# tp7/Sushi

Hardware: AMD Instinct MI355X
Metric: subtitle events/sec (matchTemplate+argmax) + max |shift err| vs cv2, 1/2/4/8 GPU (higher is better)
Workload: dtype f32; 1 GPU; BASELINE configs[2] (the north_star target's configuration): 3000 events, 120-min 12000 Hz float32 src/dst, +-120 s window (P=2880001 positions, patterns U[1,5] s), explicit centres; the whole job every step; global_events=3000, sample_type=float32, hard_events=0, events_with_a_planted_answer=3000, method=TM_SQDIFF_NORMED+argmin (what wav.py:185-186 does; see SURVEY F1), kernel_variant=2

## Files before the change

include/sushi_hip.h:

```cpp
#ifndef SUSHI_HIP_H
#define SUSHI_HIP_H

#include <stddef.h>
#include <stdint.h>

#ifdef __cplusplus
extern "C" {
#endif

#define SUSHI_HIP_ABI_VERSION 13

#if defined(__GNUC__)
#define SUSHI_HIP_API __attribute__((visibility("default")))
#else
#define SUSHI_HIP_API
#endif

#define SUSHI_HIP_OK 0
#define SUSHI_HIP_EINVAL (-1)
#define SUSHI_HIP_EALIGN (-2)
#define SUSHI_HIP_ELAUNCH (-3)
#define SUSHI_HIP_ENOSPACE (-4)
#define SUSHI_HIP_ENODEV (-5)
#define SUSHI_HIP_ENOMEM (-6)
#define SUSHI_HIP_EINTERNAL (-7)

#define SUSHI_HIP_U8 0
#define SUSHI_HIP_F32 1

#define SUSHI_HIP_PATH_FFT 0
#define SUSHI_HIP_PATH_DIRECT 1

#define SUSHI_HIP_METHOD_SQDIFF_NORMED 0
#define SUSHI_HIP_METHOD_CCOEFF_NORMED 1

SUSHI_HIP_API int sushi_hip_abi_version(void);
SUSHI_HIP_API const char* sushi_hip_strerror(int code);

SUSHI_HIP_API int sushi_hip_device_ok(void);
SUSHI_HIP_API int sushi_hip_device_prepare(void);

typedef struct SushiHipStream SushiHipStream;

SUSHI_HIP_API int sushi_hip_fft_size(void);
SUSHI_HIP_API int sushi_hip_fft_block(void);
SUSHI_HIP_API int sushi_hip_fft_slot_of_bin(int bin);
SUSHI_HIP_API int sushi_hip_fft_low_slot_of_bin(int bin);
SUSHI_HIP_API double sushi_hip_centre(int dtype);
SUSHI_HIP_API size_t sushi_hip_stream_bytes(int64_t n, int dtype, int searchable);
SUSHI_HIP_API size_t sushi_hip_stream_spectra_bytes(int64_t n);
SUSHI_HIP_API int sushi_hip_stream_create(const void* raw_dev, int dtype, int64_t n, int searchable,
                                          void* mem_dev, size_t mem_bytes, void* hip_stream, SushiHipStream** out);
SUSHI_HIP_API int sushi_hip_stream_add_spectra(SushiHipStream* stream, void* mem_dev, size_t mem_bytes, void* hip_stream);
#define SUSHI_HIP_VIEW_XC 0
#define SUSHI_HIP_VIEW_S1 1
#define SUSHI_HIP_VIEW_S2 2
#define SUSHI_HIP_VIEW_UREL 3
#define SUSHI_HIP_VIEW_BASE 4
#define SUSHI_HIP_VIEW_SPECTRA 5
#define SUSHI_HIP_VIEW_USREL 6
#define SUSHI_HIP_VIEW_BASE1 7
#define SUSHI_HIP_VIEW_COARSE 8
#define SUSHI_HIP_VIEW_SPECTRA_LOW 9
#define SUSHI_HIP_VIEW_ZNORM_REST 10
SUSHI_HIP_API int sushi_hip_stream_view(const SushiHipStream* stream, int which, const void** ptr_dev, size_t* bytes);
SUSHI_HIP_API void sushi_hip_stream_destroy(SushiHipStream* stream);

typedef struct SushiHipRequest {
    int64_t tmpl_off;
    int64_t win_start;
    int32_t tmpl_len;
    int32_t n_pos;
} SushiHipRequest;

typedef struct SushiHipBatchInfo {
    int32_t n_search;
    int32_t path;
    int32_t variant;
    int32_t sub_batches;
    int64_t direct_tiles;
    int64_t fft_pairs;
    int64_t fft_segments;
    uint64_t workspace_bytes;
    uint64_t mem_bytes;
    double flops;
    double algorithmic_bytes;
    int32_t lanes;
    int32_t reserved;
} SushiHipBatchInfo;

typedef struct SushiHipBatchDiag {
    int32_t flagged;
    int32_t all_positions;
    int64_t tiles_dense;
    int64_t tiles_sparse;
    int64_t candidates;
    float max_bound_ratio;
    float max_bound_ratio_noncandidate;
    int64_t audited;
    int64_t pairs_transformed;
    int64_t excluded_audited;
    float max_slb_ratio_excluded;
    int32_t slb_violations;
    int32_t band;
    int32_t suspended;
    int32_t band_votes[2];
    int64_t second_look_audited;
} SushiHipBatchDiag;

typedef struct SushiHipBatch SushiHipBatch;

SUSHI_HIP_API size_t sushi_hip_batch_bytes(const SushiHipRequest* req_host, int n, int path, int variant,
                                           size_t workspace_cap_bytes);
SUSHI_HIP_API int sushi_hip_batch_create(const SushiHipStream* dst, const SushiHipStream* src,
                                         const SushiHipRequest* req_host, int n, int path, int variant,
                                         size_t workspace_cap_bytes, void* mem_dev, size_t mem_bytes,
                                         void* hip_stream, SushiHipBatch** out);
SUSHI_HIP_API int sushi_hip_batch_reset(SushiHipBatch* batch, const SushiHipRequest* req_host, int n, void* hip_stream);
SUSHI_HIP_API int sushi_hip_batch_info(const SushiHipBatch* batch, SushiHipBatchInfo* info);
SUSHI_HIP_API int sushi_hip_batch_set_method(SushiHipBatch* batch, int method);
#define SUSHI_HIP_EXCLUDE_AUTO 0
#define SUSHI_HIP_EXCLUDE_ALWAYS 1
#define SUSHI_HIP_EXCLUDE_NEVER 2
#define SUSHI_HIP_EXCLUDE_BAND 3
#define SUSHI_HIP_EXCLUDE_WHOLE 4
SUSHI_HIP_API int sushi_hip_batch_set_exclusion(SushiHipBatch* batch, int mode);
#define SUSHI_HIP_BOUND_WORST_CASE 0
#define SUSHI_HIP_BOUND_STATISTICAL 1
SUSHI_HIP_API int sushi_hip_batch_set_bound_model(SushiHipBatch* batch, int model);
SUSHI_HIP_API int sushi_hip_batch_set_packed_output(SushiHipBatch* batch, int32_t* out_packed_dev);
SUSHI_HIP_API int sushi_hip_batch_set_early_output(SushiHipBatch* batch, int32_t* early);
SUSHI_HIP_API int sushi_hip_batch_run(SushiHipBatch* batch, double delta, int32_t* out_idx_dev, float* out_score_dev,
                                      void* hip_stream);
SUSHI_HIP_API int sushi_hip_batch_diagnostics(SushiHipBatch* batch, SushiHipBatchDiag* diag, float* ranking_err_host,
                                              int32_t* flagged_host);
SUSHI_HIP_API int sushi_hip_batch_pair_bounds(SushiHipBatch* batch, float* slb_host, float* acc_host, int64_t* n_pairs);
#define SUSHI_HIP_WS_TSPEC 0
#define SUSHI_HIP_WS_Y 1
#define SUSHI_HIP_WS_TSPEC_LOW 2
#define SUSHI_HIP_WS_Y_LOW 3
#define SUSHI_HIP_WS_TNORM_REST 4
#define SUSHI_HIP_WS_TSPEC_HALF 5
SUSHI_HIP_API int sushi_hip_batch_workspace_view(SushiHipBatch* batch, int which, void** ptr_dev, size_t* bytes);
SUSHI_HIP_API void sushi_hip_batch_destroy(SushiHipBatch* batch);

typedef struct SushiHipHit {
    int32_t index;
    float score;
} SushiHipHit;
SUSHI_HIP_API int sushi_hip_batch_run_threshold(SushiHipBatch* batch, double threshold, int32_t capacity,
                                                SushiHipHit* out_hits_dev, int64_t* out_counts_dev, void* hip_stream);

#define SUSHI_HIP_BEST_MAX_K 32
SUSHI_HIP_API int sushi_hip_batch_run_best(SushiHipBatch* batch, int32_t k, int32_t min_separation, const double* threshold,
                                           SushiHipHit* out_hits_dev, int32_t* out_counts_dev, void* hip_stream);

SUSHI_HIP_API int sushi_hip_fft_layout(int64_t win_start, int32_t n_pos, int32_t tmpl_len,
                                       int32_t* n_pairs, int32_t* n_seg);

SUSHI_HIP_API size_t sushi_hip_curve_bytes(const SushiHipRequest* req_host, int n);
SUSHI_HIP_API int sushi_hip_match_curves(const SushiHipStream* dst, const SushiHipStream* src,
                                         const SushiHipRequest* req_host, int n, int method,
                                         void* mem_dev, size_t mem_bytes, float* out_dev, void* hip_stream);

typedef struct SushiHipRetimeSegment {
    int64_t in_start;
    int64_t out_off;
    int64_t out_len;
    int32_t num, den;
} SushiHipRetimeSegment;
SUSHI_HIP_API size_t sushi_hip_retime_bytes(int n_seg);
SUSHI_HIP_API int sushi_hip_retime(const void* in_dev, int dtype, int64_t n_in,
                                   const SushiHipRetimeSegment* seg_host, int n_seg,
                                   void* out_dev, int64_t n_out,
                                   void* mem_dev, size_t mem_bytes, void* hip_stream);

SUSHI_HIP_API int sushi_hip_envelope(const void* in_dev, int dtype, int64_t n_in, int64_t in_start,
                                     int32_t hop, int32_t span, void* out_dev, int64_t out_len, void* hip_stream);

SUSHI_HIP_API int sushi_hip_filter(const void* in_dev, int dtype, int64_t n_in, int64_t in_start,
                                   const double* taps_dev, int32_t n_taps, void* out_dev, int64_t out_len, void* hip_stream);

SUSHI_HIP_API int sushi_hip_level(const void* in_dev, int dtype, int64_t n_in, int64_t in_start,
                                  int32_t window, double floor, double peak, void* out_dev, int64_t out_len, void* hip_stream);

typedef struct SushiHipJointRow {
    int64_t curve_off;
    double weight;
} SushiHipJointRow;
typedef struct SushiHipJointGroup {
    int32_t first_row;
    int32_t n_rows;
    int32_t n_shift;
    int32_t reserved;
} SushiHipJointGroup;
SUSHI_HIP_API size_t sushi_hip_joint_bytes(int n_groups, int n_rows);
SUSHI_HIP_API int sushi_hip_joint_reduce(const float* curves_dev, int64_t n_curve,
                                         const SushiHipJointRow* rows_host, int n_rows,
                                         const SushiHipJointGroup* groups_host, int n_groups, int method,
                                         void* mem_dev, size_t mem_bytes,
                                         int32_t* out_idx_dev, float* out_score_dev,
                                         float* out_row_score_dev, int32_t* out_row_idx_dev, float* out_row_best_dev,
                                         float* out_joint_dev, void* hip_stream);

SUSHI_HIP_API size_t sushi_hip_path_bytes(int n_rows, int32_t n_shift);
SUSHI_HIP_API int64_t sushi_hip_path_stay_words(int32_t n_shift);
SUSHI_HIP_API int sushi_hip_path_forward(const float* curves_dev, int64_t n_curve,
                                         const SushiHipJointRow* rows_host, int n_rows, int32_t n_shift,
                                         int method, double penalty, int row0, int n_total,
                                         double* D_dev, unsigned long long* stay_dev,
                                         double* row_min_dev, int32_t* row_arg_dev,
                                         int32_t* row_own_index_dev, float* row_own_score_dev,
                                         void* mem_dev, size_t mem_bytes, void* hip_stream);
SUSHI_HIP_API int sushi_hip_path_backtrack(const unsigned long long* stay_dev, const int32_t* row_arg_dev, int n_total,
                                           int32_t n_shift, int32_t* out_shift_dev, void* hip_stream);

SUSHI_HIP_API size_t sushi_hip_drift_bytes(int n_rows, int n_drifts);
SUSHI_HIP_API int sushi_hip_drift_reduce(const float* curves_dev, int64_t n_curve,
                                         const SushiHipJointRow* rows_host, int n_rows, int32_t n_shift,
                                         const int32_t* offsets_host, int n_drifts, int method,
                                         void* mem_dev, size_t mem_bytes,
                                         int32_t* out_best_dev, float* out_score_dev, float* out_row_score_dev,
                                         int32_t* out_drift_idx_dev, float* out_drift_score_dev,
                                         float* out_lines_dev, void* hip_stream);

#define SUSHI_HIP_TRACK_MAX_REACH 1024
#define SUSHI_HIP_TRACK_JUMP (-32768)
SUSHI_HIP_API size_t sushi_hip_track_bytes(int n_rows, int32_t n_shift);
SUSHI_HIP_API int sushi_hip_track_forward(const float* curves_dev, int64_t n_curve,
                                          const SushiHipJointRow* rows_host, const int32_t* reach_host, int n_rows, int32_t n_shift,
                                          int method, double penalty, double step_cost, int row0, int n_total,
                                          double* D_dev, int16_t* move_dev,
                                          double* row_min_dev, int32_t* row_arg_dev,
                                          int32_t* row_own_index_dev, float* row_own_score_dev,
                                          void* mem_dev, size_t mem_bytes, void* hip_stream);
SUSHI_HIP_API int sushi_hip_track_backtrack(const int16_t* move_dev, const int32_t* row_arg_dev, int n_total,
                                            int32_t n_shift, int32_t* out_shift_dev, void* hip_stream);

SUSHI_HIP_API int sushi_hip_track_forward_keep(const float* curves_dev, int64_t n_curve,
                                               const SushiHipJointRow* rows_host, const int32_t* reach_host, int n_rows, int32_t n_shift,
                                               int method, double penalty, double step_cost, int row0, int n_total,
                                               double* D_all_dev, int16_t* move_dev,
                                               double* row_min_dev, int32_t* row_arg_dev,
                                               int32_t* row_own_index_dev, float* row_own_score_dev,
                                               void* mem_dev, size_t mem_bytes, void* hip_stream);
SUSHI_HIP_API size_t sushi_hip_track_margins_bytes(int n_rows, int32_t n_shift);
SUSHI_HIP_API int sushi_hip_track_margins(const float* curves_dev, int64_t n_curve,
                                          const SushiHipJointRow* rows_host, const int32_t* reach_host, const int32_t* guard_host,
                                          int n_rows, int32_t n_shift, int method, double penalty, double step_cost,
                                          int row0, int n_total,
                                          const double* D_all_dev, const int32_t* shift_dev, double* C_dev, double* c_min_dev,
                                          double* through_dev, double* best_dev, int32_t* best_arg_dev,
                                          double* alt_dev, int32_t* alt_arg_dev, double* M_dev,
                                          void* mem_dev, size_t mem_bytes, void* hip_stream);

#define SUSHI_HIP_TRACK_BACK_ANY (-1)
SUSHI_HIP_API size_t sushi_hip_track_order_bytes(int n_rows, int32_t n_shift);
SUSHI_HIP_API int sushi_hip_track_forward_ordered(const float* curves_dev, int64_t n_curve,
                                                  const SushiHipJointRow* rows_host, const int32_t* reach_host,
                                                  const int32_t* back_host, int n_rows, int32_t n_shift,
                                                  int method, const double* penalty_host, double step_cost, int row0, int n_total,
                                                  double* D_dev, int16_t* move_dev,
                                                  double* P_dev, int32_t* from_dev, int32_t* back_dev,
                                                  double* row_min_dev, int32_t* row_arg_dev,
                                                  int32_t* row_own_index_dev, float* row_own_score_dev,
                                                  void* mem_dev, size_t mem_bytes, void* hip_stream);
SUSHI_HIP_API int sushi_hip_track_backtrack_ordered(const int16_t* move_dev, const int32_t* from_dev, const int32_t* back_dev,
                                                    const int32_t* row_arg_dev, int n_total, int32_t n_shift,
                                                    int32_t* out_shift_dev, void* hip_stream);

SUSHI_HIP_API int sushi_hip_track_forward_ordered_keep(const float* curves_dev, int64_t n_curve,
                                                       const SushiHipJointRow* rows_host, const int32_t* reach_host,
                                                       const int32_t* back_host, int n_rows, int32_t n_shift,
                                                       int method, const double* penalty_host, double step_cost, int row0, int n_total,
                                                       double* D_all_dev, int16_t* move_dev,
                                                       double* P_dev, int32_t* from_dev, int32_t* back_dev,
                                                       double* row_min_dev, int32_t* row_arg_dev,
                                                       int32_t* row_own_index_dev, float* row_own_score_dev,
                                                       void* mem_dev, size_t mem_bytes, void* hip_stream);
SUSHI_HIP_API size_t sushi_hip_track_order_margins_bytes(int n_rows, int32_t n_shift);
SUSHI_HIP_API int sushi_hip_track_order_margins(const float* curves_dev, int64_t n_curve,
                                                const SushiHipJointRow* rows_host, const int32_t* reach_host,
                                                const int32_t* back_host, const int32_t* guard_host,
                                                int n_rows, int32_t n_shift, int method, const double* penalty_host, double step_cost,
                                                int row0, int n_total,
                                                const double* D_all_dev, const int32_t* shift_dev, double* C_dev, double* S_dev,
                                                double* c_min_dev, double* through_dev, double* best_dev, int32_t* best_arg_dev,
                                                double* alt_dev, int32_t* alt_arg_dev, double* M_dev,
                                                void* mem_dev, size_t mem_bytes, void* hip_stream);

#define SUSHI_HIP_TRACK_WIDE_MAX_REACH 32767
SUSHI_HIP_API size_t sushi_hip_track_wide_bytes(int n_rows, int32_t n_shift);
SUSHI_HIP_API size_t sushi_hip_track_margins_wide_bytes(int n_rows, int32_t n_shift);
SUSHI_HIP_API int sushi_hip_track_forward_wide(const float* curves_dev, int64_t n_curve,
                                               const SushiHipJointRow* rows_host, const int32_t* reach_host, int n_rows, int32_t n_shift,
// ... 109 lines not shown
```

sushi_amd/_native.py:

```python
import ctypes
import os
import re

import numpy as np

from .common import SushiError

_HERE = os.path.dirname(os.path.abspath(__file__))
LIB_PATH = os.environ.get("SUSHI_HIP_LIB") or os.path.join(_HERE, "lib", "libsushi_hip.so")
HEADER_PATH = os.path.join(os.path.dirname(_HERE), "include", "sushi_hip.h")

U8, F32 = 0, 1
PATH_FFT, PATH_DIRECT = 0, 1
METHOD_SQDIFF_NORMED, METHOD_CCOEFF_NORMED = 0, 1
MIX_MAX_CHANNELS, MIX_MAX_OUTPUTS = 32, 8
PCM_FORMATS = {"u8": 1, "s16": 2, "s24": 3, "s32": 4, "f32": 5, "f64": 6}
PCM_WIDTHS = {"u8": 1, "s16": 2, "s24": 3, "s32": 4, "f32": 4, "f64": 8}
BEST_MAX_K = 32
TRACK_MAX_REACH, TRACK_JUMP = 1024, -32768
TRACK_WIDE_MAX_REACH = 32767
TRACK_BACK_ANY = -1
METHODS = {"sqdiff_normed": METHOD_SQDIFF_NORMED, "ccoeff_normed": METHOD_CCOEFF_NORMED}
VIEW_XC, VIEW_S1, VIEW_S2, VIEW_UREL, VIEW_BASE, VIEW_SPECTRA, VIEW_USREL, VIEW_BASE1, VIEW_COARSE, VIEW_SPECTRA_LOW, \
    VIEW_ZNORM_REST = range(11)

ABI_VERSION = 13
ENOSPACE = -4
NSTAGES = 6
STAGE_NAMES = ("tspec", "mac", "ifft", "refine", "finish", "bound")
STAGE_KERNELS = {"tspec": "tspec_real_kernel|tspec_kernel", "mac": "mac_kernel", "ifft": "mac_list_kernel+mac_rows_kernel+ifft_kernel", "refine": "refine_kernel",
                 "finish": "collect_kernel+exact_tiles_kernel+unpack_keys_kernel", "bound": "bound_low_kernel|bound_kernel"}
EXCLUSION = {"auto": 0, "always": 1, "never": 2, "band": 3, "whole": 4}
WS_TSPEC, WS_Y, WS_TSPEC_LOW, WS_Y_LOW, WS_TNORM_REST, WS_TSPEC_HALF = range(6)
BOUND_MODEL = {"worst_case": 0, "statistical": 1}
STAGE_KERNEL_SETS = {"tspec": ("tspec_real_kernel", "tspec_kernel"), "mac": ("mac_kernel", "mac_long_kernel"),
                     "ifft": ("ifft_kernel", "ifft_list_kernel", "pilot_kernel", "survivor_kernel", "mac_list_kernel", "mac_rows_kernel",
                              "bound_low_exact_kernel", "slb_list_kernel", "survivor2_kernel"),
                     "refine": ("refine_kernel",),
                     "finish": ("collect_kernel", "exact_tiles_kernel"), "bound": ("bound_kernel", "bound_low_kernel", "slb_kernel")}

REQUEST_DTYPE = np.dtype([("tmpl_off", "<i8"), ("win_start", "<i8"), ("tmpl_len", "<i4"), ("n_pos", "<i4")], align=True)
assert REQUEST_DTYPE.itemsize == 24
HIT_DTYPE = np.dtype([("index", "<i4"), ("score", "<f4")], align=True)
assert HIT_DTYPE.itemsize == 8
RETIME_SEGMENT_DTYPE = np.dtype([("in_start", "<i8"), ("out_off", "<i8"), ("out_len", "<i8"), ("num", "<i4"), ("den", "<i4")], align=True)
assert RETIME_SEGMENT_DTYPE.itemsize == 32
JOINT_ROW_DTYPE = np.dtype([("curve_off", "<i8"), ("weight", "<f8")], align=True)
assert JOINT_ROW_DTYPE.itemsize == 16
JOINT_GROUP_DTYPE = np.dtype([("first_row", "<i4"), ("n_rows", "<i4"), ("n_shift", "<i4"), ("reserved", "<i4")], align=True)
assert JOINT_GROUP_DTYPE.itemsize == 16
ROWS_ROW_DTYPE = np.dtype([("out_off", "<i8"), ("in_off", "<i8"), ("n_pos", "<i4"), ("reserved", "<i4")], align=True)
assert ROWS_ROW_DTYPE.itemsize == 24
ROWS_OVERFLOW, ROWS_BAD_HITS = 1, 2


class BatchInfo(ctypes.Structure):
    _fields_ = [("n_search", ctypes.c_int32), ("path", ctypes.c_int32), ("variant", ctypes.c_int32),
                ("sub_batches", ctypes.c_int32), ("direct_tiles", ctypes.c_int64), ("fft_pairs", ctypes.c_int64),
                ("fft_segments", ctypes.c_int64), ("workspace_bytes", ctypes.c_uint64), ("mem_bytes", ctypes.c_uint64),
                ("flops", ctypes.c_double), ("algorithmic_bytes", ctypes.c_double), ("lanes", ctypes.c_int32),
                ("reserved", ctypes.c_int32)]


class BatchDiag(ctypes.Structure):
    _fields_ = [("flagged", ctypes.c_int32), ("all_positions", ctypes.c_int32), ("tiles_dense", ctypes.c_int64),
                ("tiles_sparse", ctypes.c_int64), ("candidates", ctypes.c_int64), ("max_bound_ratio", ctypes.c_float),
                ("max_bound_ratio_noncandidate", ctypes.c_float), ("audited", ctypes.c_int64),
                ("pairs_transformed", ctypes.c_int64), ("excluded_audited", ctypes.c_int64),
                ("max_slb_ratio_excluded", ctypes.c_float), ("slb_violations", ctypes.c_int32), ("band", ctypes.c_int32),
                ("suspended", ctypes.c_int32), ("band_votes", ctypes.c_int32 * 2), ("second_look_audited", ctypes.c_int64)]


_lib = None


class NativeError(SushiError):
    pass


def declared_symbols():
    with open(HEADER_PATH) as f:
        text = f.read()
    return sorted(set(re.findall(r"SUSHI_HIP_API\s+[\w\s\*]+?\b(sushi_hip_\w+)\s*\(", text)))


def lib():
    global _lib
    if _lib is not None:
        return _lib
    if not os.path.exists(LIB_PATH):
        raise NativeError("libsushi_hip.so is not built (%s); run `python -m sushi_amd.build` -- "
                          "there is no CPU fallback for the matching path" % LIB_PATH)
    import torch
    L = ctypes.CDLL(LIB_PATH)
    vp, i64, ci, dbl, sz = ctypes.c_void_p, ctypes.c_int64, ctypes.c_int, ctypes.c_double, ctypes.c_size_t
    i32, u32, cf = ctypes.c_int32, ctypes.c_uint32, ctypes.c_float
    pvp = ctypes.POINTER(vp)
    L.sushi_hip_abi_version.restype = ci
    L.sushi_hip_strerror.restype = ctypes.c_char_p
    L.sushi_hip_strerror.argtypes = [ci]
    L.sushi_hip_device_ok.restype = ci
    L.sushi_hip_device_prepare.restype = ci
    L.sushi_hip_fft_size.restype = ci
    L.sushi_hip_fft_block.restype = ci
    L.sushi_hip_fft_slot_of_bin.restype = ci
    L.sushi_hip_fft_slot_of_bin.argtypes = [ci]
    L.sushi_hip_fft_low_slot_of_bin.restype = ci
    L.sushi_hip_fft_low_slot_of_bin.argtypes = [ci]
    L.sushi_hip_centre.restype = dbl
    L.sushi_hip_centre.argtypes = [ci]
    L.sushi_hip_stream_bytes.restype = sz
    L.sushi_hip_stream_bytes.argtypes = [i64, ci, ci]
    L.sushi_hip_stream_spectra_bytes.restype = sz
    L.sushi_hip_stream_spectra_bytes.argtypes = [i64]
    L.sushi_hip_stream_create.restype = ci
    L.sushi_hip_stream_create.argtypes = [vp, ci, i64, ci, vp, sz, vp, pvp]
    L.sushi_hip_stream_add_spectra.restype = ci
    L.sushi_hip_stream_add_spectra.argtypes = [vp, vp, sz, vp]
    L.sushi_hip_stream_view.restype = ci
    L.sushi_hip_stream_view.argtypes = [vp, ci, pvp, ctypes.POINTER(sz)]
    L.sushi_hip_stream_destroy.restype = None
    L.sushi_hip_stream_destroy.argtypes = [vp]
    L.sushi_hip_batch_bytes.restype = sz
    L.sushi_hip_batch_bytes.argtypes = [vp, ci, ci, ci, sz]
    L.sushi_hip_batch_create.restype = ci
    L.sushi_hip_batch_create.argtypes = [vp, vp, vp, ci, ci, ci, sz, vp, sz, vp, pvp]
    L.sushi_hip_batch_reset.restype = ci
    L.sushi_hip_batch_reset.argtypes = [vp, vp, ci, vp]
    L.sushi_hip_batch_info.restype = ci
    L.sushi_hip_batch_info.argtypes = [vp, ctypes.POINTER(BatchInfo)]
    L.sushi_hip_batch_set_method.restype = ci
    L.sushi_hip_batch_set_method.argtypes = [vp, ci]
    L.sushi_hip_batch_run.restype = ci
    L.sushi_hip_batch_run.argtypes = [vp, dbl, vp, vp, vp]
    L.sushi_hip_batch_run_threshold.restype = ci
    L.sushi_hip_batch_run_threshold.argtypes = [vp, dbl, i32, vp, vp, vp]
    L.sushi_hip_batch_run_best.restype = ci
    L.sushi_hip_batch_run_best.argtypes = [vp, i32, i32, ctypes.POINTER(dbl), vp, vp, vp]
    L.sushi_hip_batch_diagnostics.restype = ci
    L.sushi_hip_batch_diagnostics.argtypes = [vp, ctypes.POINTER(BatchDiag), vp, vp]
    L.sushi_hip_batch_set_packed_output.restype = ci
    L.sushi_hip_batch_set_packed_output.argtypes = [vp, vp]
    L.sushi_hip_batch_set_early_output.restype = ci
    L.sushi_hip_batch_set_early_output.argtypes = [vp, vp]
    L.sushi_hip_batch_set_exclusion.restype = ci
    L.sushi_hip_batch_set_exclusion.argtypes = [vp, ci]
    L.sushi_hip_batch_set_bound_model.restype = ci
    L.sushi_hip_batch_set_bound_model.argtypes = [vp, ci]
    L.sushi_hip_batch_pair_bounds.restype = ci
    L.sushi_hip_batch_pair_bounds.argtypes = [vp, vp, vp, ctypes.POINTER(i64)]
    L.sushi_hip_batch_workspace_view.restype = ci
    L.sushi_hip_batch_workspace_view.argtypes = [vp, ci, pvp, ctypes.POINTER(sz)]
    L.sushi_hip_batch_destroy.restype = None
    L.sushi_hip_batch_destroy.argtypes = [vp]
    L.sushi_hip_fft_layout.restype = ci
    L.sushi_hip_fft_layout.argtypes = [i64, i32, i32, ctypes.POINTER(i32), ctypes.POINTER(i32)]
    L.sushi_hip_curve_bytes.restype = sz
    L.sushi_hip_curve_bytes.argtypes = [vp, ci]
    L.sushi_hip_match_curves.restype = ci
    L.sushi_hip_match_curves.argtypes = [vp, vp, vp, ci, ci, vp, sz, vp, vp]
    L.sushi_hip_retime_bytes.restype = sz
    L.sushi_hip_retime_bytes.argtypes = [ci]
    L.sushi_hip_retime.restype = ci
    L.sushi_hip_retime.argtypes = [vp, ci, i64, vp, ci, vp, i64, vp, sz, vp]
    L.sushi_hip_envelope.restype = ci
    L.sushi_hip_envelope.argtypes = [vp, ci, i64, i64, i32, i32, vp, i64, vp]
    L.sushi_hip_filter.restype = ci
    L.sushi_hip_filter.argtypes = [vp, ci, i64, i64, vp, i32, vp, i64, vp]
    L.sushi_hip_level.restype = ci
    L.sushi_hip_level.argtypes = [vp, ci, i64, i64, i32, dbl, dbl, vp, i64, vp]
    L.sushi_hip_joint_bytes.restype = sz
    L.sushi_hip_joint_bytes.argtypes = [ci, ci]
    L.sushi_hip_joint_reduce.restype = ci
    L.sushi_hip_joint_reduce.argtypes = [vp, i64, vp, ci, vp, ci, ci, vp, sz, vp, vp, vp, vp, vp, vp, vp]
    L.sushi_hip_drift_bytes.restype = sz
    L.sushi_hip_drift_bytes.argtypes = [ci, ci]
    L.sushi_hip_drift_reduce.restype = ci
    L.sushi_hip_drift_reduce.argtypes = [vp, i64, vp, ci, i32, vp, ci, ci, vp, sz, vp, vp, vp, vp, vp, vp, vp]
    L.sushi_hip_path_bytes.restype = sz
    L.sushi_hip_path_bytes.argtypes = [ci, i32]
    L.sushi_hip_path_stay_words.restype = i64
    L.sushi_hip_path_stay_words.argtypes = [i32]
    L.sushi_hip_path_forward.restype = ci
    L.sushi_hip_path_forward.argtypes = [vp, i64, vp, ci, i32, ci, dbl, ci, ci, vp, vp, vp, vp, vp, vp, vp, sz, vp]
    L.sushi_hip_path_backtrack.restype = ci
    L.sushi_hip_path_backtrack.argtypes = [vp, vp, ci, i32, vp, vp]
    L.sushi_hip_track_bytes.restype = sz
    L.sushi_hip_track_bytes.argtypes = [ci, i32]
    L.sushi_hip_track_forward.restype = ci
    L.sushi_hip_track_forward.argtypes = [vp, i64, vp, vp, ci, i32, ci, dbl, dbl, ci, ci, vp, vp, vp, vp, vp, vp, vp, sz, vp]
    L.sushi_hip_track_backtrack.restype = ci
    L.sushi_hip_track_backtrack.argtypes = [vp, vp, ci, i32, vp, vp]
    L.sushi_hip_track_forward_keep.restype = ci
    L.sushi_hip_track_forward_keep.argtypes = L.sushi_hip_track_forward.argtypes
    L.sushi_hip_track_margins_bytes.restype = sz
    L.sushi_hip_track_margins_bytes.argtypes = [ci, i32]
    L.sushi_hip_track_margins.restype = ci
    L.sushi_hip_track_margins.argtypes = [vp, i64, vp, vp, vp, ci, i32, ci, dbl, dbl, ci, ci, vp, vp, vp, vp, vp, vp, vp, vp, vp, vp, vp,
                                          sz, vp]
    L.sushi_hip_track_wide_bytes.restype = sz
    L.sushi_hip_track_wide_bytes.argtypes = [ci, i32]
    L.sushi_hip_track_margins_wide_bytes.restype = sz
    L.sushi_hip_track_margins_wide_bytes.argtypes = [ci, i32]
    L.sushi_hip_track_forward_wide.restype = ci
    L.sushi_hip_track_forward_wide.argtypes = L.sushi_hip_track_forward.argtypes
    L.sushi_hip_track_forward_wide_keep.restype = ci
    L.sushi_hip_track_forward_wide_keep.argtypes = L.sushi_hip_track_forward.argtypes
    L.sushi_hip_track_margins_wide.restype = ci
    L.sushi_hip_track_margins_wide.argtypes = L.sushi_hip_track_margins.argtypes
    L.sushi_hip_track_order_bytes.restype = sz
    L.sushi_hip_track_order_bytes.argtypes = [ci, i32]
    L.sushi_hip_track_forward_ordered.restype = ci
    L.sushi_hip_track_forward_ordered.argtypes = [vp, i64, vp, vp, vp, ci, i32, ci, vp, dbl, ci, ci, vp, vp, vp, vp, vp, vp, vp, vp, vp,
                                                  vp, sz, vp]
    L.sushi_hip_track_backtrack_ordered.restype = ci
    L.sushi_hip_track_backtrack_ordered.argtypes = [vp, vp, vp, vp, ci, i32, vp, vp]
    L.sushi_hip_track_forward_ordered_keep.restype = ci
    L.sushi_hip_track_forward_ordered_keep.argtypes = L.sushi_hip_track_forward_ordered.argtypes
    L.sushi_hip_track_order_margins_bytes.restype = sz
    L.sushi_hip_track_order_margins_bytes.argtypes = [ci, i32]
    L.sushi_hip_track_order_margins.restype = ci
    L.sushi_hip_track_order_margins.argtypes = [vp, i64, vp, vp, vp, vp, ci, i32, ci, vp, dbl, ci, ci, vp, vp, vp, vp, vp, vp, vp, vp, vp,
                                                vp, vp, vp, sz, vp]
    L.sushi_hip_track_order_wide_bytes.restype = sz
    L.sushi_hip_track_order_wide_bytes.argtypes = [ci, i32]
    L.sushi_hip_track_order_margins_wide_bytes.restype = sz
    L.sushi_hip_track_order_margins_wide_bytes.argtypes = [ci, i32]
    L.sushi_hip_track_forward_ordered_wide.restype = ci
    L.sushi_hip_track_forward_ordered_wide.argtypes = L.sushi_hip_track_forward_ordered.argtypes
    L.sushi_hip_track_forward_ordered_wide_keep.restype = ci
    L.sushi_hip_track_forward_ordered_wide_keep.argtypes = L.sushi_hip_track_forward_ordered.argtypes
    L.sushi_hip_track_order_margins_wide.restype = ci
    L.sushi_hip_track_order_margins_wide.argtypes = L.sushi_hip_track_order_margins.argtypes
    L.sushi_hip_rows_tile.restype = ci
    L.sushi_hip_rows_bytes.restype = sz
    L.sushi_hip_rows_bytes.argtypes = [ci]
    L.sushi_hip_rows_from_hits.restype = ci
    L.sushi_hip_rows_from_hits.argtypes = [vp, vp, ci, i32, vp, cf, vp, i64, vp, vp, sz, vp]
    L.sushi_hip_rows_clamp.restype = ci
    L.sushi_hip_rows_clamp.argtypes = [vp, i64, vp, i64, vp, ci, ci, cf, vp, sz, vp]
    L.sushi_hip_load_decode.restype = ci
    L.sushi_hip_load_decode.argtypes = [vp, i64, i32, i32, vp, vp]
    L.sushi_hip_load_decode_mix.restype = ci
    L.sushi_hip_load_decode_mix.argtypes = [vp, i64, i32, i32, vp, i32, vp, i64, vp]
    L.sushi_hip_load_decode_format.restype = ci
    L.sushi_hip_load_decode_format.argtypes = [vp, i64, i32, i32, vp, vp]
    L.sushi_hip_load_decode_mix_format.restype = ci
    L.sushi_hip_load_decode_mix_format.argtypes = [vp, i64, i32, i32, vp, i32, vp, i64, vp]
    L.sushi_hip_load_resample.restype = ci
    L.sushi_hip_load_resample.argtypes = [vp, i64, i32, i32, dbl, i64, i32, i32, dbl, i64, i64, vp, vp]
    L.sushi_hip_load_resample_fir.restype = ci
    L.sushi_hip_load_resample_fir.argtypes = [vp, i64, i32, i32, vp, i32, i64, i64, i64, vp, vp]
    L.sushi_hip_load_histogram.restype = ci
    L.sushi_hip_load_histogram.argtypes = [vp, i64, ci, u32, u32, ci, vp, vp]
    L.sushi_hip_load_normalise.restype = ci
    L.sushi_hip_load_normalise.argtypes = [vp, i64, cf, cf, cf, vp, vp]
    L.sushi_hip_profile_begin.restype = ci
    L.sushi_hip_profile_end.restype = ci
    L.sushi_hip_profile_end.argtypes = [vp, ci, ctypes.POINTER(ci)]
    if L.sushi_hip_abi_version() != ABI_VERSION:
        raise NativeError("libsushi_hip.so ABI version mismatch")
    _lib = L
    return L


def check(rc, what):
    if rc != 0:
        msg = lib().sushi_hip_strerror(rc).decode()
        raise NativeError("%s failed: %s (%d)" % (what, msg, rc))


def fft_layout(win_start, n_pos, tmpl_len):
    a, b = ctypes.c_int32(0), ctypes.c_int32(0)
    check(lib().sushi_hip_fft_layout(int(win_start), int(n_pos), int(tmpl_len), ctypes.byref(a), ctypes.byref(b)),
          "sushi_hip_fft_layout")
    return a.value, b.value


def profile_begin():
    check(lib().sushi_hip_profile_begin(), "sushi_hip_profile_begin")


def profile_end(max_calls):
    buf = np.zeros((max(1, max_calls), NSTAGES), np.float32)
    n = ctypes.c_int(0)
    check(lib().sushi_hip_profile_end(buf.ctypes.data, int(max_calls), ctypes.byref(n)), "sushi_hip_profile_end")
    return buf[:n.value]
```

sushi_amd/csrc/fft_core.hpp:

```cpp
#ifndef SUSHI_FFT_CORE_HPP
#define SUSHI_FFT_CORE_HPP

#ifdef __HIPCC__
#define SUSHI_HD __device__ __forceinline__
#define SUSHI_HHD __host__ __device__ inline
#else
#define SUSHI_HD inline
#define SUSHI_HHD inline
#endif

namespace sushi_fft {

constexpr int PER = 16;
constexpr int TWIDDLE_N = 16384;

template <int LOGN> struct Plan;
template <> struct Plan<13> {
    static constexpr int N = 8192, NT = 512, R3 = 8;
};
template <> struct Plan<14> {
    static constexpr int N = 16384, NT = 1024, R3 = 16;
};
constexpr int R1 = 8, R2 = 8, R4 = 16;

// ... 491 lines not shown
}
typedef _Float16 h2 __attribute__((ext_vector_type(2)));
__device__ __forceinline__ h2 h_rot(const h2 a) { return h2{-a.y, a.x}; }
__device__ __forceinline__ h2 h_cmul(const h2 a, const h2 w) { return a * w.xx + h_rot(a) * w.yy; }
__device__ __forceinline__ h2 h_splat(const float c) { return h2{(_Float16)c, (_Float16)c}; }
__device__ __forceinline__ void h_bfly_root32(const h2 e, const h2 o, const int q, h2& lo, h2& hi) {
    const float C[9] = {1.0f, 0.98078528040323044913f, 0.92387953251128673848f, 0.83146961230254523708f, 0.70710678118654752440f,
                        0.55557023301960222474f, 0.38268343236508978178f, 0.19509032201612826785f, 0.0f};
    switch (q) {
        case 0: lo = e + o; hi = e - o; return;
        case 8: lo = e + h_rot(o); hi = e - h_rot(o); return;
        case 4: { const h2 p = o + h_rot(o); lo = p * h_splat(C[4]) + e; hi = e - p * h_splat(C[4]); return; }
        case 12: { const h2 p = h_rot(o) - o; lo = p * h_splat(C[4]) + e; hi = e - p * h_splat(C[4]); return; }
        default: {
            const float c = q <= 8 ? C[q] : -C[16 - q], sn = q <= 8 ? C[8 - q] : C[q - 8];
            lo = h_rot(o) * h_splat(sn) + (o * h_splat(c) + e);
            hi = e * h_splat(2.0f) - lo;
        }
    }
}
template <int R>
struct DftH {
    static __device__ __forceinline__ void run(h2* v) {
        h2 e[R / 2], o[R / 2];
#pragma unroll
        for (int u = 0; u < R / 2; ++u) { e[u] = v[2 * u]; o[u] = v[2 * u + 1]; }
        DftH<R / 2>::run(e);
        DftH<R / 2>::run(o);
#pragma unroll
        for (int t = 0; t < R / 2; ++t) h_bfly_root32(e[t], o[t], t * (32 / R), v[t], v[t + R / 2]);
    }
};
template <>
struct DftH<1> {
    static __device__ __forceinline__ void run(h2*) {}
};
struct HTwiddles { h2 p2[16]; h2 z1[4], z2[4], z3[4]; };
__device__ __forceinline__ h2 h_round(const cpx c) { return h2{(_Float16)c.x, (_Float16)c.y}; }
__device__ __forceinline__ HTwiddles load_htwiddles(const int lane, const cpx* __restrict__ tw) {
    HTwiddles t;
    const int e1 = lane & 15;
#pragma unroll
    for (int d = 0; d < 16; ++d) t.p2[d] = h_round(cconj(tw[((e1 * d) & 255) * (TWIDDLE_N / 256)]));
    const cpx q3 = cconj(tw[((lane & 15) + 64 * (lane >> 4)) * (TWIDDLE_N / 1024)]);
#pragma unroll
    for (int e = 0; e < 4; ++e) {
        const cpx z = cmul(q3, cconj(tw[e * (TWIDDLE_N / 64)]));
        const cpx z2 = cmul(z, z);
        t.z1[e] = h_round(z); t.z2[e] = h_round(z2); t.z3[e] = h_round(cmul(z2, z));
    }
    return t;
}
__device__ __forceinline__ unsigned h_abs2(const h2 a) {
    return __builtin_bit_cast(unsigned, __builtin_amdgcn_fdot2(a, a, 0.f, false));
}
__device__ __forceinline__ unsigned h_max_bits(const unsigned a, const unsigned b) { return a > b ? a : b; }
struct MfmaBh { half8 r, i; };
__device__ __forceinline__ MfmaBh load_mfma_bh(const int lane, const uint4v* __restrict__ table) {
    MfmaBh b;
    b.r = __builtin_bit_cast(half8, table[lane]);
    b.i = __builtin_bit_cast(half8, table[64 + lane]);
    return b;
}
__device__ __forceinline__ void fft_wave_half_front(const uint4v (&yl)[4], h2* v, const HTwiddles& tw, const MfmaBh& b, unsigned& max_in2,
                                                    h2* pass1_out = nullptr, h2* pass2_out = nullptr, h2* swapped_out = nullptr) {
    unsigned mi = 0u;
#pragma unroll
    for (int g = 0; g < 4; ++g) {
        unsigned rr01 = __builtin_amdgcn_perm(yl[g][1], yl[g][0], 0x05040100u), rr23 = __builtin_amdgcn_perm(yl[g][3], yl[g][2], 0x05040100u);
        unsigned ii01 = __builtin_amdgcn_perm(yl[g][1], yl[g][0], 0x07060302u), ii23 = __builtin_amdgcn_perm(yl[g][3], yl[g][2], 0x07060302u);
        { const auto r = __builtin_amdgcn_permlane32_swap(rr01, ii01, false, false); rr01 = r[0]; ii01 = r[1]; }
        { const auto r = __builtin_amdgcn_permlane32_swap(rr23, ii23, false, false); rr23 = r[0]; ii23 = r[1]; }
        const uint4v aw = {rr01, rr23, ii01, ii23};
        const half8 a = __builtin_bit_cast(half8, aw);
        const float4v z = {0.f, 0.f, 0.f, 0.f};
        const float4v dr = __builtin_amdgcn_mfma_f32_16x16x32_f16(a, b.r, z, 0, 0, 0);
        const float4v di = __builtin_amdgcn_mfma_f32_16x16x32_f16(a, b.i, z, 0, 0, 0);
#pragma unroll
        for (int i = 0; i < 4; ++i) {
            unsigned packed = __builtin_bit_cast(unsigned, h2{(_Float16)dr[i], (_Float16)di[i]});
            asm volatile("" : "+v"(packed));
            v[4 * g + i] = __builtin_bit_cast(h2, packed);
            mi = h_max_bits(mi, h_abs2(v[4 * g + i]));
        }
    }
    max_in2 = mi;
    if (pass1_out) {
#pragma unroll
        for (int t = 0; t < 16; ++t) pass1_out[t] = v[t];
    }
#pragma unroll
    for (int t = 1; t < 16; ++t) v[t] = h_cmul(v[t], tw.p2[t]);
    DftH<16>::run(v);
    if (pass2_out) {
#pragma unroll
        for (int t = 0; t < 16; ++t) pass2_out[t] = v[t];
    }
    auto swap32 = [](h2& x, h2& y) {
        const auto r = __builtin_amdgcn_permlane32_swap(__builtin_bit_cast(unsigned, x), __builtin_bit_cast(unsigned, y), false, false);
        unsigned ra = r[0], rb = r[1];
        asm volatile("" : "+v"(ra), "+v"(rb));
        x = __builtin_bit_cast(h2, ra); y = __builtin_bit_cast(h2, rb);
    };
    auto swap16 = [](h2& x, h2& y) {
        const auto r = __builtin_amdgcn_permlane16_swap(__builtin_bit_cast(unsigned, x), __builtin_bit_cast(unsigned, y), false, false);
        unsigned ra = r[0], rb = r[1];
        asm volatile("" : "+v"(ra), "+v"(rb));
        x = __builtin_bit_cast(h2, ra); y = __builtin_bit_cast(h2, rb);
    };
#pragma unroll
    for (int r = 0; r < 8; ++r) swap32(v[r], v[r + 8]);
#pragma unroll
    for (int r = 0; r < 16; ++r)
        if ((r & 4) == 0) swap16(v[r], v[r + 4]);
    if (swapped_out) {
#pragma unroll
        for (int t = 0; t < 16; ++t) swapped_out[t] = v[t];
    }
#pragma unroll
    for (int e = 0; e < 4; ++e) {
        h2 q[4] = {v[e], h_cmul(v[4 + e], tw.z1[e]), h_cmul(v[8 + e], tw.z2[e]), h_cmul(v[12 + e], tw.z3[e])};
        DftH<4>::run(q);
        v[e] = q[0]; v[4 + e] = q[1]; v[8 + e] = q[2]; v[12 + e] = q[3];
    }
}
#endif

constexpr int LB_HW = WN / 8;
constexpr int LB_BINS = 2 * LB_HW;
constexpr int LB_ENTRIES = LB_BINS / 4;
constexpr int LB_GROUPS = 8;
SUSHI_HHD int lslot_of_thread(int tid) {
    const int g = tid & 7, t = tid >> 3;
    const int kq = t >> 6, g4 = (t >> 4) & 3, mm = ((t & 3) << 2) | ((t >> 2) & 3);
    return (g * 4 + g4) * 32 + 16 * kq + mm;
}
SUSHI_HHD int lb_d1(int kq, int j) { return kq + (j == 0 ? 0 : (j == 1 ? 2 : (j == 2 ? 12 : 14))); }
SUSHI_HHD int lb_bin_of(int entry, int j) {
    const int g = entry >> 7, g4 = (entry >> 5) & 3, l = entry & 31, kq = l >> 4, mm = l & 15;
    const int d2 = 4 * g4 + (mm & 3), d3 = mm >> 2;
    const int m = 64 * lb_d1(kq, j) + 4 * d2 + d3;
    const int k = g + 8 * m;
    return k < WN / 8 ? k : k + WN / 2;
}
SUSHI_HHD int lslot_of_bin(int f) {
    if (f < 0 || f >= WN || (f >= LB_HW && f < WN - LB_HW)) return -1;
    const int k = f < LB_HW ? f : f - WN / 2;
    const int g = k & 7, m = k >> 3;
    const int d1 = m >> 6, d2 = (m >> 2) & 15, d3 = m & 3;
    const int kq = d1 & 1, b = d1 - kq;
    const int j = b == 0 ? 0 : (b == 2 ? 1 : (b == 12 ? 2 : 3));
    return (((g * 4 + (d2 >> 2)) * 32 + 16 * kq + ((d3 << 2) | (d2 & 3))) << 2) + j;
}
SUSHI_HHD double dft16_low_operand(int form, int l, int j) {
    const int kq = l >> 4, n = l & 15, part = kq >> 1, d1 = lb_d1(kq & 1, j);
    const double PI = 3.14159265358979323846;
    const double wr = __builtin_cos(2.0 * PI * (double)((n * d1) & 15) / 16.0), wi = __builtin_sin(2.0 * PI * (double)((n * d1) & 15) / 16.0);
    return form == 0 ? (part == 0 ? wr : -wi) : (part == 0 ? wi : wr);
}

#ifdef __HIPCC__
typedef _Float16 half4 __attribute__((ext_vector_type(4)));
typedef unsigned uint2v __attribute__((ext_vector_type(2)));
struct MfmaBl { half4 r, i; };
__device__ __forceinline__ MfmaBl load_mfma_bl(const int lane, const uint2v* __restrict__ table) {
    MfmaBl b;
    b.r = __builtin_bit_cast(half4, table[lane]);
    b.i = __builtin_bit_cast(half4, table[64 + lane]);
    return b;
}
__device__ __forceinline__ void fft_wave_half_tail(h2* v, const HTwiddles& tw) {
#pragma unroll
    for (int t = 1; t < 16; ++t) v[t] = h_cmul(v[t], tw.p2[t]);
    DftH<16>::run(v);
    auto swap32 = [](h2& x, h2& y) {
        const auto r = __builtin_amdgcn_permlane32_swap(__builtin_bit_cast(unsigned, x), __builtin_bit_cast(unsigned, y), false, false);
        unsigned ra = r[0], rb = r[1];
        asm volatile("" : "+v"(ra), "+v"(rb));
        x = __builtin_bit_cast(h2, ra); y = __builtin_bit_cast(h2, rb);
    };
    auto swap16 = [](h2& x, h2& y) {
        const auto r = __builtin_amdgcn_permlane16_swap(__builtin_bit_cast(unsigned, x), __builtin_bit_cast(unsigned, y), false, false);
        unsigned ra = r[0], rb = r[1];
        asm volatile("" : "+v"(ra), "+v"(rb));
        x = __builtin_bit_cast(h2, ra); y = __builtin_bit_cast(h2, rb);
    };
#pragma unroll
    for (int r = 0; r < 8; ++r) swap32(v[r], v[r + 8]);
#pragma unroll
    for (int r = 0; r < 16; ++r)
        if ((r & 4) == 0) swap16(v[r], v[r + 4]);
#pragma unroll
    for (int e = 0; e < 4; ++e) {
        h2 q[4] = {v[e], h_cmul(v[4 + e], tw.z1[e]), h_cmul(v[8 + e], tw.z2[e]), h_cmul(v[12 + e], tw.z3[e])};
        DftH<4>::run(q);
        v[e] = q[0]; v[4 + e] = q[1]; v[8 + e] = q[2]; v[12 + e] = q[3];
    }
}
__device__ __forceinline__ void fft_wave_half_front_low(const uint4v (&yl)[4], h2* v, const HTwiddles& tw, const MfmaBl& b, unsigned& max_in2,
                                                        h2* pass1_out = nullptr) {
    unsigned mi = 0u;
#pragma unroll
    for (int g = 0; g < 4; ++g) {
        unsigned rr01 = __builtin_amdgcn_perm(yl[g][1], yl[g][0], 0x05040100u), rr23 = __builtin_amdgcn_perm(yl[g][3], yl[g][2], 0x05040100u);
        unsigned ii01 = __builtin_amdgcn_perm(yl[g][1], yl[g][0], 0x07060302u), ii23 = __builtin_amdgcn_perm(yl[g][3], yl[g][2], 0x07060302u);
        { const auto r = __builtin_amdgcn_permlane32_swap(rr01, ii01, false, false); rr01 = r[0]; ii01 = r[1]; }
        { const auto r = __builtin_amdgcn_permlane32_swap(rr23, ii23, false, false); rr23 = r[0]; ii23 = r[1]; }
        const uint2v aw = {rr01, rr23};
        const half4 a = __builtin_bit_cast(half4, aw);
        const float4v z = {0.f, 0.f, 0.f, 0.f};
        const float4v dr = __builtin_amdgcn_mfma_f32_16x16x16f16(a, b.r, z, 0, 0, 0);
        const float4v di = __builtin_amdgcn_mfma_f32_16x16x16f16(a, b.i, z, 0, 0, 0);
#pragma unroll
        for (int i = 0; i < 4; ++i) {
            unsigned packed = __builtin_bit_cast(unsigned, h2{(_Float16)dr[i], (_Float16)di[i]});
            asm volatile("" : "+v"(packed));
            v[4 * g + i] = __builtin_bit_cast(h2, packed);
            mi = h_max_bits(mi, h_abs2(v[4 * g + i]));
        }
    }
    max_in2 = mi;
    if (pass1_out) {
#pragma unroll
        for (int t = 0; t < 16; ++t) pass1_out[t] = v[t];
    }
    fft_wave_half_tail(v, tw);
}
#endif

}
#endif
```

sushi_amd/csrc/run_policy.hpp:

```cpp
#ifndef SUSHI_RUN_POLICY_HPP
#define SUSHI_RUN_POLICY_HPP

#include <stdint.h>
#include <string.h>

#include <algorithm>

#include "sushi_geometry.hpp"

#ifndef SUSHI_HHD
#ifdef __HIPCC__
#define SUSHI_HHD __host__ __device__ inline
#else
#define SUSHI_HHD inline
#endif
#endif

namespace sushi {

enum RunKind { RUN_ARGMIN, RUN_THRESHOLD, RUN_BEST };

struct Learnt {
    int band = -1;
    int band_decided_method = -1;
    int band_votes[2] = {0, 0};
    int suspended = 0;
    unsigned suspended_at = 0;
    unsigned long long last_transformed = 0;
    void forget() { *this = Learnt(); }
};

struct LastRun {
    RunKind kind = RUN_ARGMIN;
    int band = -1;
    bool whole_cut = false;
    bool suspended = false;
    int64_t direct_pairs = 0;
    bool ran = false;
};

constexpr double SUSPEND_LEFT_SHARE = 0.75;
constexpr unsigned LOOK_AGAIN_MASK = 63u;
constexpr int64_t EXCLUDE_FROM_PAIRS = 3000, EXCLUDE_PAIRS_PER_SEARCH = 2;
constexpr double BAND_VOTE_SHARE = 0.75;
constexpr int64_t DIRECT_SLOTS_MIN = 4096, DIRECT_USUAL_PART = 8;
constexpr int64_t DIRECT_FIRST_RUN_PART = 2;

inline void absorb_counts(Learnt& l, int exclusion, unsigned run_seq, unsigned long long transformed, unsigned long long audited,
                          int64_t plan_pairs) {
    const unsigned long long left = transformed - audited;
    l.last_transformed = transformed;
    if (exclusion == SUSHI_HIP_EXCLUDE_AUTO) {
        if ((double)left > SUSPEND_LEFT_SHARE * (double)plan_pairs) { if (!l.suspended) l.suspended_at = run_seq; l.suspended = 1; }
        else l.suspended = 0;
    }
}

inline bool run_suspended(const Learnt& l, int exclusion, unsigned run_seq) {
    return exclusion == SUSHI_HIP_EXCLUDE_AUTO && l.suspended && ((run_seq - l.suspended_at) & LOOK_AGAIN_MASK) != LOOK_AGAIN_MASK;
}

inline bool whole_rows_throughout(const Learnt& l, int exclusion, int method, bool suspended) {
    return suspended || exclusion == SUSHI_HIP_EXCLUDE_NEVER || exclusion == SUSHI_HIP_EXCLUDE_WHOLE ||
           ((exclusion == SUSHI_HIP_EXCLUDE_AUTO || exclusion == SUSHI_HIP_EXCLUDE_ALWAYS) && l.band == 0 && l.band_decided_method == method);
}
inline bool takes_whole_cut(bool whole_rows, bool whole_cut_exists) { return whole_rows && whole_cut_exists; }
inline int run_lanes(bool whole_rows, int plan_lanes) { return whole_rows ? 1 : plan_lanes; }

inline bool sub_excludes(int exclusion, bool suspended, int64_t pairs, int n_sub) {
    return exclusion == SUSHI_HIP_EXCLUDE_ALWAYS || exclusion == SUSHI_HIP_EXCLUDE_BAND || exclusion == SUSHI_HIP_EXCLUDE_WHOLE ||
           (exclusion == SUSHI_HIP_EXCLUDE_AUTO && !suspended && pairs > EXCLUDE_FROM_PAIRS + EXCLUDE_PAIRS_PER_SEARCH * (int64_t)n_sub);
}

inline bool listed_run_excludes(int exclusion) { return exclusion != SUSHI_HIP_EXCLUDE_NEVER; }

inline bool form_chosen(int exclusion) { return exclusion == SUSHI_HIP_EXCLUDE_BAND || exclusion == SUSHI_HIP_EXCLUDE_WHOLE; }
inline bool vote_due(const Learnt& l, int exclusion, int method) {
    return !form_chosen(exclusion) && (l.band < 0 || l.band_decided_method != method);
}
inline void decide_form(Learnt& l, int method, int looked_at, int with_room) {
    l.band_votes[0] = looked_at; l.band_votes[1] = with_room;
    l.band = l.band_votes[0] > 0 && (double)l.band_votes[1] >= BAND_VOTE_SHARE * (double)l.band_votes[0] ? 1 : 0;
    l.band_decided_method = method;
}
inline int exclusion_form(const Learnt& l, int exclusion) {
    return !form_chosen(exclusion) ? l.band : exclusion == SUSHI_HIP_EXCLUDE_BAND ? 1 : 0;
}

inline int64_t direct_slots(unsigned long long last_transformed, int64_t pairs, int64_t plan_pairs) {
    int64_t direct64 = std::min<int64_t>(pairs, std::max<int64_t>(DIRECT_SLOTS_MIN, pairs / DIRECT_USUAL_PART));
    if ((double)last_transformed * (double)pairs > (double)direct64 * (double)plan_pairs) direct64 = pairs;
    else if (last_transformed == 0) direct64 = std::min<int64_t>(pairs, std::max<int64_t>(DIRECT_SLOTS_MIN, pairs / DIRECT_FIRST_RUN_PART));
    return direct64;
}

enum { PILOT_ROWS_BY_SEARCH = 0, PILOT_ROWS_LIST = 1 };
inline int pilot_rows_route(const char* setting) {
    if (!setting || !*setting || !strcmp(setting, "search")) return PILOT_ROWS_BY_SEARCH;
    return !strcmp(setting, "list") ? PILOT_ROWS_LIST : -1;
}
inline bool pilot_rows_by_search(int route) { return route != PILOT_ROWS_LIST; }

enum { REST_ROWS_BY_ITEM = 0, REST_ROWS_BY_SEARCH = 1 };
inline int rest_rows_route(const char* setting) {
    if (!setting || !*setting || !strcmp(setting, "items")) return REST_ROWS_BY_ITEM;
    return !strcmp(setting, "search") ? REST_ROWS_BY_SEARCH : -1;
}
inline bool rest_rows_by_item(int route) { return route != REST_ROWS_BY_SEARCH; }

#ifndef SUSHI_REST_ITEM_PAIRS
#define SUSHI_REST_ITEM_PAIRS 4
#endif
constexpr int REST_ITEM_PAIRS = SUSHI_REST_ITEM_PAIRS;
static_assert(REST_ITEM_PAIRS >= 1, "an item holds a pair");
SUSHI_HHD bool rest_pair_to_form(int listed, int i, int audit) { return listed != 0 && i != audit; }
SUSHI_HHD unsigned long long rest_item_starts(unsigned long long form, int before, int per_item) {
    unsigned long long starts = 0;
    int rank = before;
    for (unsigned long long m = form; m; m &= m - 1, ++rank)
        if (rank % per_item == 0) starts |= m & (~m + 1);
    return starts;
}
SUSHI_HHD unsigned long long rest_item_take(unsigned long long form, int room) {
    unsigned long long take = 0;
    for (unsigned long long m = form; m && room > 0; m &= m - 1, --room) take |= m & (~m + 1);
    return take;
}

enum { TSPEC_REAL = 0, TSPEC_COMPLEX = 1 };
inline int tspec_route(const char* setting) {
    if (!setting || !*setting || !strcmp(setting, "real")) return TSPEC_REAL;
    return !strcmp(setting, "complex") ? TSPEC_COMPLEX : -1;
}
inline bool tspec_real(int route) { return route != TSPEC_COMPLEX; }
inline bool tspec_half_rows(int route) { return tspec_real(route); }

inline void begin_run(LastRun& last, RunKind kind) {
    last = LastRun();
    last.kind = kind; last.ran = true;
}

inline void report_last_run(const LastRun& last, const Learnt& l, const RunCounters& c, SushiHipBatchDiag* diag) {
    const bool argmin = last.kind == RUN_ARGMIN;
    diag->pairs_transformed = (int64_t)c.pairs_transformed + last.direct_pairs;
    diag->band = last.band;
    diag->suspended = argmin && last.suspended ? 1 : 0;
    diag->band_votes[0] = argmin ? l.band_votes[0] : 0; diag->band_votes[1] = argmin ? l.band_votes[1] : 0;
    diag->second_look_audited = argmin ? (int64_t)c.second_look_audited : 0;
}

}
#endif
```

sushi_amd/csrc/sushi_fft.hip:

```cpp

#include <hip/hip_runtime.h>
#include <stdint.h>
#include <float.h>
#include <limits.h>
#include <stdio.h>
#include <stdlib.h>
#include <string.h>

#include <algorithm>
#include <cmath>
#include <memory>
#include <mutex>
#include <new>
#include <string>
#include <type_traits>
#include <vector>

#include "../../include/sushi_hip.h"
#include "sushi_common.hpp"
#include "sushi_internal.hpp"
#include "fft_core.hpp"
#include "mac_core.hpp"
#include "plan_core.hpp"
#include "batch_core.hpp"
#include "run_policy.hpp"

namespace {

using namespace sushi;
using sushi_fft::cpx;

constexpr int FN = FFT_N;
constexpr int FT = sushi_fft::Plan<FFT_LOGN>::NT;
constexpr int FH = FFT_H;
constexpr int HPT = FH / FT;
constexpr int RPB = FFT_SEG / FT;
static_assert(FH % FT == 0 && FFT_SEG % FT == 0 && HPT == FFT_VB * RPB, "position layout");
static_assert(HPT <= sushi_fft::PER, "a thread's valid outputs are a prefix of its transform outputs");
constexpr int LDS_FLOATS = sushi_fft::lds_floats<FFT_LOGN>();

#include "sushi_fft_store.inc"
#include "sushi_fft_spectra.inc"
#include "sushi_fft_mac.inc"
#include "sushi_fft_ifft.inc"
#include "sushi_fft_bound.inc"
#include "sushi_fft_collect.inc"
#include "sushi_fft_threshold.inc"
#include "sushi_fft_best.inc"
#include "sushi_fft_plan.inc"

}

struct HostSlots {
    static constexpr int SLOTS = 1024, WORDS = 2;
    std::mutex mu;
    unsigned long long* base = nullptr;
    std::vector<int> free_list;
    unsigned long long* take() {
        std::lock_guard<std::mutex> g(mu);
        if (!base) {
            if (hipHostMalloc((void**)&base, (size_t)SLOTS * WORDS * sizeof(unsigned long long), hipHostMallocPortable) != hipSuccess) { base = nullptr; return nullptr; }
            for (int k = SLOTS - 1; k >= 0; --k) free_list.push_back(k);
        }
        if (free_list.empty()) return nullptr;
        const int k = free_list.back(); free_list.pop_back();
        return base + (size_t)k * WORDS;
    }
    void give(unsigned long long* p) {
        if (!p) return;
        std::lock_guard<std::mutex> g(mu);
        free_list.push_back((int)((p - base) / WORDS));
    }
};
static HostSlots g_host_slots;

struct LanePool {
    static constexpr int MAX_DEVICES = 16;
    std::mutex mu;
    hipStream_t st[MAX_DEVICES][MAX_LANES] = {};
    hipStream_t get(int lane) {
        int dev = 0;
        if (hipGetDevice(&dev) != hipSuccess || dev < 0 || dev >= MAX_DEVICES) return nullptr;
        std::lock_guard<std::mutex> g(mu);
        if (!st[dev][lane] && hipStreamCreateWithFlags(&st[dev][lane], hipStreamNonBlocking) != hipSuccess) st[dev][lane] = nullptr;
        return st[dev][lane];
    }
};
static LanePool g_lane_pool;

struct SushiHipBatch {
    const SushiHipStream* dst = nullptr;
    const SushiHipStream* src = nullptr;
    int n = 0, path = 0, variant = 0, method = SUSHI_HIP_METHOD_SQDIFF_NORMED, exclusion = SUSHI_HIP_EXCLUDE_AUTO;
    Learnt learnt;
    LastRun last;
    unsigned run_seq = 0;
    int audit_every = 2;
    int pilot_rows = PILOT_ROWS_BY_SEARCH;
    int rest_rows = REST_ROWS_BY_ITEM;
    int tspec = TSPEC_REAL;
    int bound_model = SUSHI_HIP_BOUND_WORST_CASE;
    BoundFault fault;
    unsigned long long* host_stats = nullptr;
    hipEvent_t stats_ready = nullptr;
    bool stats_pending = false;
    int32_t* packed_out = nullptr;
    int32_t* early_out = nullptr;
    BatchPlanState states[2];
    BatchPlanState *now = &states[0], *spare = &states[1];
    bool planned = false;
    size_t mem_bytes = 0, ws_cap = 0;
    char* mem = nullptr;
    hipStream_t last_stream = nullptr;
    hipEvent_t uploaded = nullptr;
    hipStream_t lane_stream[MAX_LANES] = {};
    hipEvent_t lane_done[MAX_LANES] = {};
    hipEvent_t fork = nullptr;
    void* tspec_whole = nullptr;
    size_t tspec_whole_bytes = 0;
    void forget_learnt() { learnt.forget(); last = LastRun(); }
    ~SushiHipBatch() {
        for (int l = 1; l < MAX_LANES; ++l) {
            if (lane_stream[l]) (void)hipStreamSynchronize(lane_stream[l]);
            if (lane_done[l]) (void)hipEventDestroy(lane_done[l]);
        }
        if (fork) (void)hipEventDestroy(fork);
        if (uploaded) { (void)hipEventSynchronize(uploaded); (void)hipEventDestroy(uploaded); }
        if (stats_pending && stats_ready) (void)hipEventSynchronize(stats_ready);
        if (stats_ready) (void)hipEventDestroy(stats_ready);
        g_host_slots.give(host_stats);
        if (tspec_whole) (void)hipFree(tspec_whole);
    }
};

static SubView last_sub(const SushiHipBatch* b) {
    const std::vector<SubBatch>& subs = b->last.whole_cut ? b->now->plan.subs_whole : b->now->plan.subs;
    return SubView(b->mem, b->now->lay, b->now->plan.ws_lane, subs.back(), subs.size() - 1);
}

struct RunCtx {
    SushiHipBatch* b;
    const SushiHipStream *dst, *src;
    StreamRefs r;
    const SearchDesc* searches;
    unsigned long long *keys, *gkeys;
    int *flags, *flag_list, *viol;
    RunCounters* counters;
    double delta;
    int method, lanes = 1;
    unsigned run_seq = 0;
    ProfCall* pc = nullptr;
    bool suspended = false, cand_filled = false, excluded_any = false;
    RunCtx(SushiHipBatch* bb, double d) : b(bb), dst(bb->dst), src(bb->src), delta(d), method(bb->method) {
        r = StreamRefs{dst->xc, dst->s1, dst->s2, dst->n, src->xc, src->s1, src->s2, src->n, sushi_hip_centre(dst->dtype), dst->raw, src->raw,
                       dst->dtype};
        searches = (const SearchDesc*)(b->mem + b->now->lay.desc); keys = (unsigned long long*)(b->mem + b->now->lay.keys); gkeys = keys + b->n;
        flags = (int*)(b->mem + b->now->lay.flags); flag_list = (int*)(b->mem + b->now->lay.flag_list); viol = (int*)(b->mem + b->now->lay.viol);
        counters = (RunCounters*)(b->mem + b->now->lay.counters);
    }
};

struct Lanes {
    SushiHipBatch* b;
    hipStream_t st[MAX_LANES];
    int forked = 1;
    Lanes(SushiHipBatch* bb, hipStream_t st0) : b(bb) { for (hipStream_t& s : st) s = st0; }
    ~Lanes() { (void)join(); }
    int fork(int lanes) {
        if (lanes < 2) return SUSHI_HIP_OK;
        if ((!b->fork && hipEventCreateWithFlags(&b->fork, hipEventDisableTiming) != hipSuccess) || hipEventRecord(b->fork, st[0]) != hipSuccess)
            return SUSHI_HIP_ELAUNCH;
        for (int l = 1; l < lanes; ++l) {
            if (!b->lane_stream[l] && !(b->lane_stream[l] = g_lane_pool.get(l))) return SUSHI_HIP_ELAUNCH;
            if (!b->lane_done[l] && hipEventCreateWithFlags(&b->lane_done[l], hipEventDisableTiming) != hipSuccess) return SUSHI_HIP_ELAUNCH;
            if (hipStreamWaitEvent(b->lane_stream[l], b->fork, 0) != hipSuccess) return SUSHI_HIP_ELAUNCH;
            st[l] = b->lane_stream[l];
            forked = l + 1;
        }
        return SUSHI_HIP_OK;
    }
    int join() {
        int rc = SUSHI_HIP_OK;
        for (int l = 1; l < forked; ++l)
            if (hipEventRecord(b->lane_done[l], st[l]) != hipSuccess || hipStreamWaitEvent(st[0], b->lane_done[l], 0) != hipSuccess) rc = SUSHI_HIP_ELAUNCH;
        forked = 1;
        return rc;
    }
};

struct RunForm { bool suspended; const std::vector<SubBatch>* subs; int lanes; };
static int run_form(SushiHipBatch* b, unsigned run_seq, hipStream_t st0, RunForm* f) {
    if (b->stats_pending && hipEventQuery(b->stats_ready) == hipSuccess) {
        b->stats_pending = false;
        absorb_counts(b->learnt, b->exclusion, run_seq, b->host_stats[0], b->host_stats[1], b->now->plan.pairs);
    }
    f->suspended = run_suspended(b->learnt, b->exclusion, run_seq);
    const bool whole_rows = whole_rows_throughout(b->learnt, b->exclusion, b->method, f->suspended);
    if (whole_rows && b->now->plan.whole_pending) {
        if (complete_whole_cut(b->now->descs, b->now->plan)) {
            for (const UploadSpan& u : whole_cut_upload(b->now->plan, b->now->lay))
                if (hipMemcpyAsync(b->mem + u.dev_off, u.host, u.bytes, hipMemcpyHostToDevice, st0) != hipSuccess) return SUSHI_HIP_ELAUNCH;
            if (hipEventRecord(b->uploaded, st0) != hipSuccess) return SUSHI_HIP_ELAUNCH;
        } else {
            b->now->plan.whole_pending = false;
        }
    }
    const bool whole_cut = takes_whole_cut(whole_rows, !b->now->plan.subs_whole.empty());
    f->subs = whole_cut ? &b->now->plan.subs_whole : &b->now->plan.subs;
    f->lanes = run_lanes(whole_rows, b->now->plan.lanes);
    b->last.suspended = f->suspended; b->last.whole_cut = whole_cut;
    return SUSHI_HIP_OK;
}

static void fill_add(FillArgs& fa, void* p, size_t bytes, uint32_t v) { fa.p[fa.n] = (uint32_t*)p; fa.words[fa.n] = (uint32_t)(bytes / 4); fa.value[fa.n] = v; ++fa.n; }
static int begin_run(SushiHipBatch* b, const hipStream_t st0, const RunKind kind) {
    b->last_stream = st0;
    begin_run(b->last, kind);
    return hipStreamWaitEvent(st0, b->uploaded, 0) == hipSuccess ? SUSHI_HIP_OK : SUSHI_HIP_ELAUNCH;
}
template <class PerSub>
static int run_sub_batches(RunCtx& c, const hipStream_t st0, const RunKind kind, FillArgs fa, PerSub&& per_sub) {
    SushiHipBatch* b = c.b;
    int rc = begin_run(b, st0, kind);
    if (rc != SUSHI_HIP_OK) return rc;
    const MemSpan zeros = run_fill_span(b->now->lay);
    fill_add(fa, b->mem + zeros.off, zeros.bytes, 0u);
    if (launch_fill(fa, st0) != SUSHI_HIP_OK) return SUSHI_HIP_ELAUNCH;
    c.run_seq = b->run_seq++;
    RunForm form{false, &b->now->plan.subs, b->now->plan.lanes};
    if (kind == RUN_ARGMIN && (rc = run_form(b, c.run_seq, st0, &form)) != SUSHI_HIP_OK) return rc;
    c.suspended = form.suspended; c.lanes = form.lanes;
    Lanes lanes(b, st0);
    if ((rc = lanes.fork(form.lanes)) != SUSHI_HIP_OK) return rc;
    for (size_t si = 0; si < form.subs->size(); ++si) {
        const SubBatch& sb = (*form.subs)[si];
        if ((rc = per_sub(SubView(b->mem, b->now->lay, b->now->plan.ws_lane, sb, si), lanes.st[sb.lane])) != SUSHI_HIP_OK) return rc;
    }
    return lanes.join();
}

static int stage_tspec(const RunCtx& c, const SubView& v, hipStream_t st) {
    hipEvent_t t0 = prof_begin(c.pc, st);
    TspecArgs ta;
    ta.src_raw = c.src->raw; ta.searches = c.searches + v.sb.a0; ta.n_sub = v.n_sub; ta.sub_first_seg = v.sb.first_seg;
    ta.tspec = v.tspec; ta.sub_first_pair = v.sb.first_pair; ta.pairmap = v.pairmap; ta.tconst = v.tconst;
    ta.src_s1 = c.src->s1; ta.src_s2 = c.src->s2; ta.centre = c.r.centre; ta.dst_stats = c.dst->stats; ta.method = c.method;
    ta.tspec_low = v.tspec_low; ta.tnorm_rest = v.tnorm_rest;
    const bool real = tspec_real(c.b->tspec);
    if (launch_dtype(c.src->dtype, [&](auto t) {
            typedef std::remove_pointer_t<decltype(t)> S;
            if (real) hipLaunchKernelGGL(tspec_real_kernel<S>, dim3((unsigned)v.sb.segs), dim3(RT), 0, st, ta);
            else hipLaunchKernelGGL(tspec_kernel<S>, dim3((unsigned)v.sb.segs), dim3(FT), 0, st, ta); }) != SUSHI_HIP_OK)
        return SUSHI_HIP_ELAUNCH;
    prof_end(c.pc, t0, SUSHI_HIP_STAGE_TSPEC, st);
    return SUSHI_HIP_OK;
}

static BoundArgs bound_args(const RunCtx& c, const SubView& v) {
    const SushiHipStream* dst = c.dst;
    BoundArgs ba;
    memset(&ba, 0, sizeof(ba));
    ba.dst_stats = dst->stats; ba.searches = c.searches + v.sb.a0; ba.sub_first_pair = v.sb.first_pair; ba.first_search = v.sb.a0; ba.dst_len = dst->n;
    ba.pairmap = v.pairmap; ba.tconst = v.tconst; ba.ubase = dst->base; ba.sbase = dst->base1; ba.nb = dst->blocks;
    ba.coarse = dst->coarse; ba.nc = dst->nc; ba.slb = v.slb; ba.n_sub = v.n_sub; ba.n_pairs = (int)v.sb.pairs; ba.plist = v.plist;
    ba.slist = v.slist; ba.scount = v.n_slist; ba.order = v.order; ba.gkeys = c.gkeys; ba.pair_lb = v.pair_lb; ba.counters = c.counters; ba.acc = v.acc;
    ba.sub_first_seg = v.sb.first_seg; ba.tnorm_rest = v.tnorm_rest; ba.znorm_rest = dst->znorm_rest; ba.norm_stride = dst->norm_stride;
    ba.band_votes = v.votes; ba.audit_mark = v.audit_mark; ba.audit_seq = c.run_seq; ba.audit_every = c.b->audit_every;
    ba.worst_case = c.b->bound_model == SUSHI_HIP_BOUND_WORST_CASE ? 1 : 0;
    ba.half_err = ba.worst_case ? 0.6f : 0.29f;
    return ba;
}

static int launch_slb(const RunCtx& c, const SubView& v, const BoundArgs& x, hipStream_t st) {
    return launch_method(c.method, [&](auto m) {
        hipLaunchKernelGGL(slb_kernel<decltype(m)::value>, dim3((unsigned)((v.sb.pairs + 3) / 4)), dim3(256), 0, st, x); });
}

static int launch_bound_fault(const RunCtx& c, const SubView& v, hipStream_t st) {
    BoundFaultArgs fa;
    fa.searches = c.searches + v.sb.a0; fa.pairmap = v.pairmap; fa.slb = v.slb; fa.first_search = v.sb.a0;
    fa.sub_first_pair = v.sb.first_pair; fa.n_pairs = (int)v.sb.pairs; fa.f = c.b->fault;
    hipLaunchKernelGGL(bound_fault_kernel, dim3((unsigned)((v.sb.pairs + 255) / 256)), dim3(256), 0, st, fa);
    return launch_ok();
}

static int decide_band(const RunCtx& c, const SubView& v, hipStream_t st, int* band) {
    SushiHipBatch* b = c.b;
    if (vote_due(b->learnt, b->exclusion, b->method)) {
        int slots[VOTE_SLOTS * VOTE_STRIDE];
        if (hipMemsetAsync(v.votes, 0, sizeof(slots), st) != hipSuccess) return SUSHI_HIP_ELAUNCH;
        BoundArgs bp = bound_args(c, v);
        bp.band = 2;
        if (launch_slb(c, v, bp, st) != SUSHI_HIP_OK) return SUSHI_HIP_ELAUNCH;
        if (hipMemcpyAsync(slots, v.votes, sizeof(slots), hipMemcpyDeviceToHost, st) != hipSuccess || hipStreamSynchronize(st) != hipSuccess)
            return SUSHI_HIP_ELAUNCH;
        int looked_at = 0, with_room = 0;
        for (int k = 0; k < VOTE_SLOTS; ++k) { looked_at += slots[k * VOTE_STRIDE]; with_room += slots[k * VOTE_STRIDE + 1]; }
        decide_form(b->learnt, b->method, looked_at, with_room);
    }
    *band = b->last.band = exclusion_form(b->learnt, b->exclusion);
    return SUSHI_HIP_OK;
}

static int launch_mac(const RunCtx& c, const SubView& v, hipStream_t st, const bool low, const int* enable, const int32_t* items_of_the_launch) {
    const SubBatch& sb = v.sb;
    MacArgs ma;
    ma.spec_blocks = c.dst->blocks; ma.searches = c.searches + sb.a0; ma.tconst = v.tconst; ma.sub_first_seg = sb.first_seg;
    ma.sub_first_pair = sb.first_pair; ma.dummy = v.dummy; ma.enable = enable;
    if (low) { ma.spec = (const uint4*)c.dst->spec_low; ma.tspec = v.tspec_low; ma.y = v.ylow; }
    else { ma.spec = (const uint4*)c.dst->spec; ma.tspec = (const uint4*)v.tspec; ma.y = v.y; }
    ma.tspec_half = !low && tspec_half_rows(c.b->tspec) ? 1 : 0;
    for (int kern = 0; kern < 2; ++kern) {
        if (sb.item_count[kern] == 0) continue;
        ma.items = items_of_the_launch + (size_t)(sb.item_first[kern] - sb.item_first[0]) * (1 + MAC_SPW);
        ma.n_items = sb.item_count[kern];
        const int chunks = (low ? LROWE : ROWE) / MAC_BW;
        ma.chunk_group = std::min(sb.chunk_group[kern], chunks / 8);
        const dim3 grid((unsigned)chunks * (unsigned)ma.n_items);
        auto go = [&](auto row) {
            if (kern == 0) hipLaunchKernelGGL(mac_kernel<decltype(row)::value>, grid, dim3(MAC_THREADS), 0, st, ma);
            else hipLaunchKernelGGL(mac_long_kernel<decltype(row)::value>, grid, dim3(MAC_THREADS), 0, st, ma);
        };
        if (low) go(std::integral_constant<int, LROWE>()); else go(std::integral_constant<int, ROWE>());
        if (launch_ok() != SUSHI_HIP_OK) return SUSHI_HIP_ELAUNCH;
    }
    return SUSHI_HIP_OK;
}

static int launch_mac_list(const RunCtx& c, const SubView& v, hipStream_t st, const int* list, const int* count, int n_list,
                           const int* dense_search, int long_only) {
    MacListArgs la;
    la.dense_search = dense_search; la.long_only = long_only;
    la.spec = (const uint4*)c.dst->spec; la.spec_blocks = c.dst->blocks; la.tspec = (const uint4*)v.tspec; la.tspec_half = tspec_half_rows(c.b->tspec) ? 1 : 0; la.y = v.y;
    la.searches = c.searches + v.sb.a0; la.tconst = v.tconst; la.pairmap = v.pairmap; la.list = list; la.count = count;
    la.n_list = n_list; la.sub_first_seg = v.sb.first_seg; la.sub_first_pair = v.sb.first_pair;
    const int64_t want = (int64_t)n_list * MACL_PARTS;
    hipLaunchKernelGGL(mac_list_kernel, dim3((unsigned)std::min<int64_t>(want, 256 * 32)), dim3(MACL_THREADS), 0, st, la);
    return launch_ok();
}

static int launch_mac_rows(const RunCtx& c, const SubView& v, hipStream_t st, const BoundArgs& ba, const int mode) {
    const SubBatch& sb = v.sb;
    MacRowsArgs ra;
    ra.spec = (const uint4*)c.dst->spec; ra.spec_blocks = c.dst->blocks; ra.tspec = (const uint4*)v.tspec; ra.tspec_half = tspec_half_rows(c.b->tspec) ? 1 : 0; ra.y = v.y;
    ra.searches = c.searches + sb.a0; ra.tconst = v.tconst; ra.mark = ba.audit_mark; ra.n_sub = v.n_sub;
    ra.sub_first_seg = sb.first_seg; ra.sub_first_pair = sb.first_pair; ra.dense_search = v.dense_search;
    ra.plist = ba.plist; ra.first_search = ba.first_search; ra.audit_seq = ba.audit_seq; ra.audit_every = ba.audit_every;
    ra.items = v.slist; ra.item_count = v.n_rest_items; ra.pairmap = v.pairmap; ra.n_pairs = (int)sb.pairs;
    const int64_t rows_want = (int64_t)(mode == ROWS_ITEMS ? sb.pairs : v.n_sub) * (mode == ROWS_FIRST && ra.tspec_half ? MACL_PARTS / 2 : MACL_PARTS);
    const dim3 grid0((unsigned)std::min<int64_t>(rows_want, 256 * 32)), grid1((unsigned)std::min<int64_t>(rows_want, 256 * 16));
    auto go = [&](auto m) {
        if (sb.item_count[0] > 0) hipLaunchKernelGGL((mac_rows_kernel<0, decltype(m)::value>), grid0, dim3(MACL_THREADS), 0, st, ra);
        if (sb.item_count[1] > 0) hipLaunchKernelGGL((mac_rows_kernel<1, decltype(m)::value>), grid1, dim3(MACL_THREADS), 0, st, ra);
    };
    if (mode == ROWS_FIRST) go(std::integral_constant<int, ROWS_FIRST>());
    else if (mode == ROWS_REST) go(std::integral_constant<int, ROWS_REST>());
    else if (mode == ROWS_ITEMS) go(std::integral_constant<int, ROWS_ITEMS>());
    else go(std::integral_constant<int, ROWS_MARKED>());
    return launch_ok();
}

static int launch_ifft(const RunCtx& c, const IfftArgs& x, unsigned grid, hipStream_t st) {
    const bool strided = x.count && !x.list_direct;
    return launch_method(c.method, [&](auto m) {
        if (strided) hipLaunchKernelGGL(ifft_list_kernel<decltype(m)::value>, dim3(grid), dim3(FT), 0, st, x);
        else hipLaunchKernelGGL(ifft_kernel<decltype(m)::value>, dim3(grid), dim3(FT), 0, st, x);
    });
}

static int bound_pairs(const RunCtx& c, const SubView& v, hipStream_t st, const int band, BoundArgs& ba) {
    const SubBatch& sb = v.sb;
    ba = bound_args(c, v);
    ba.band = band;
    ba.y = band ? (const uint2*)v.ylow : (const uint2*)v.y;
    if (!band && hipMemsetAsync(ba.acc, 0, (size_t)sb.pairs * 2 * sizeof(float), st) != hipSuccess) return SUSHI_HIP_ELAUNCH;
    const int per_pair = band ? 1 : 16;
    const int64_t want = (sb.pairs * per_pair + BOUND_THREADS / 64 - 1) / (BOUND_THREADS / 64);
    const unsigned grid = (unsigned)std::min<int64_t>(want, 256 * (band ? 3 * (c.lanes > 1 ? 2 : 4) : 4));
    auto go = [&](auto energies) {
        if (band) hipLaunchKernelGGL(bound_low_kernel<decltype(energies)::value>, dim3(grid), dim3(BOUND_THREADS), 0, st, ba);
        else hipLaunchKernelGGL(bound_kernel<decltype(energies)::value>, dim3(grid), dim3(BOUND_THREADS), 0, st, ba);
    };
    if (ba.worst_case) go(std::false_type()); else go(std::true_type());
    if (launch_ok() != SUSHI_HIP_OK || launch_slb(c, v, ba, st) != SUSHI_HIP_OK) return SUSHI_HIP_ELAUNCH;
    if (c.b->fault.period > 0) return launch_bound_fault(c, v, st);
    return SUSHI_HIP_OK;
}

static int second_look(const RunCtx& c, const SubView& v, hipStream_t st, BoundArgs& ba) {
    ba.list = ba.slist; ba.list_count = ba.scount;
    ba.list2 = v.slist2; ba.list2_count = v.n_slist2;
    hipLaunchKernelGGL(bound_low_exact_kernel, dim3(256 * 4), dim3(BLE_T), 0, st, ba);
    if (launch_ok() != SUSHI_HIP_OK) return SUSHI_HIP_ELAUNCH;
    if (launch_method(c.method, [&](auto m) { hipLaunchKernelGGL(slb_list_kernel<decltype(m)::value>, dim3(256 * 2), dim3(256), 0, st, ba); }) !=
        SUSHI_HIP_OK)
        return SUSHI_HIP_ELAUNCH;
    if (c.b->fault.period > 0 && launch_bound_fault(c, v, st) != SUSHI_HIP_OK) return SUSHI_HIP_ELAUNCH;
    hipLaunchKernelGGL(survivor2_kernel, dim3(256), dim3(256), 0, st, ba);
    return launch_ok();
}

static int exclude_pairs(const RunCtx& c, const SubView& v, hipStream_t st, const int band, IfftArgs& ip, hipEvent_t& t0) {
    const SubBatch& sb = v.sb;
    BoundArgs ba;
    if (bound_pairs(c, v, st, band, ba) != SUSHI_HIP_OK) return SUSHI_HIP_ELAUNCH;
    prof_end(c.pc, t0, SUSHI_HIP_STAGE_BOUND, st);
    t0 = prof_begin(c.pc, st);
    hipLaunchKernelGGL(pilot_kernel, dim3((unsigned)v.n_sub), dim3(64), 0, st, ba);
    if (launch_ok() != SUSHI_HIP_OK) return SUSHI_HIP_ELAUNCH;
    ip.slb = ba.slb; ip.audit_mark = nullptr;
    ip.order = ba.plist; ip.count = nullptr;
    const bool by_search = pilot_rows_by_search(c.b->pilot_rows);
    if (band && by_search && launch_mac_rows(c, v, st, ba, ROWS_FIRST) != SUSHI_HIP_OK) return SUSHI_HIP_ELAUNCH;
    if (band && launch_mac_list(c, v, st, ba.plist, nullptr, v.n_sub, nullptr, by_search ? 1 : 0) != SUSHI_HIP_OK) return SUSHI_HIP_ELAUNCH;
    if (launch_ifft(c, ip, (unsigned)v.n_sub, st) != SUSHI_HIP_OK) return SUSHI_HIP_ELAUNCH;
    hipLaunchKernelGGL(survivor_kernel, dim3((unsigned)((sb.pairs + 255) / 256)), dim3(256), 0, st, ba);
    if (launch_ok() != SUSHI_HIP_OK) return SUSHI_HIP_ELAUNCH;
    ip.order = ba.slist; ip.count = ba.scount; ip.audit_mark = ba.audit_mark;
    if (!band) return SUSHI_HIP_OK;
    if (second_look(c, v, st, ba) != SUSHI_HIP_OK) return SUSHI_HIP_ELAUNCH;
    ip.order = ba.list2; ip.count = ba.list2_count;
    const bool by_item = by_search && rest_rows_by_item(c.b->rest_rows);
    hipLaunchKernelGGL(dense_search_kernel, dim3((unsigned)v.n_sub), dim3(64), 0, st, ba, v.dense_search, v.n_dense_listed,
                       by_item ? v.slist : nullptr, v.n_rest_items);
    const size_t second = (size_t)(sb.item_first[1] - sb.item_first[0]) * (1 + MAC_SPW);
    hipLaunchKernelGGL(dense_repack_kernel, dim3(2), dim3(REPACK_THREADS), 0, st, v.items, sb.item_count[0], v.items + second,
                       sb.item_count[1], v.dense_search, v.n_sub, v.ditems, v.ditems + second, v.n_dense_listed, (int)(sb.pairs / 8),
                       v.any_dense);
    if (launch_ok() != SUSHI_HIP_OK) return SUSHI_HIP_ELAUNCH;
    if (launch_mac_rows(c, v, st, ba, by_item ? ROWS_ITEMS : by_search ? ROWS_REST : ROWS_MARKED) != SUSHI_HIP_OK) return SUSHI_HIP_ELAUNCH;
    if (sb.long_patterns && launch_mac_list(c, v, st, ba.list2, ba.list2_count, (int)sb.pairs, v.dense_search, 1) != SUSHI_HIP_OK) return SUSHI_HIP_ELAUNCH;
    return launch_mac(c, v, st, false, v.any_dense, v.ditems);
}

static int transform_listed(const RunCtx& c, const SubView& v, hipStream_t st, IfftArgs ip) {
    const SubBatch& sb = v.sb;
    const SushiHipBatch* b = c.b;
    const unsigned direct = (unsigned)direct_slots(b->learnt.last_transformed, sb.pairs, b->now->plan.pairs);
    ip.list_first = 0; ip.list_direct = 1;
    if (launch_ifft(c, ip, direct, st) != SUSHI_HIP_OK) return SUSHI_HIP_ELAUNCH;
    if ((int64_t)direct >= sb.pairs) return SUSHI_HIP_OK;
    ip.list_first = (int)direct; ip.list_direct = 0;
    return launch_ifft(c, ip, (unsigned)std::min<int64_t>(sb.pairs - direct, 1024), st);
}

static int stage_refine(const RunCtx& c, const SubView& v, hipStream_t st) {
    hipEvent_t t0 = prof_begin(c.pc, st);
    RefineParams rp;
    rp.r = c.r; rp.searches = c.searches; rp.first_search = v.sb.a0; rp.n_sub = v.n_sub; rp.sub_first_pair = v.sb.first_pair;
    rp.cand = v.cand; rp.pair_lb = v.pair_lb; rp.gkeys = c.gkeys; rp.keys = c.keys; rp.flags = c.flags; rp.flag_list = c.flag_list + v.sb.a0;
    rp.sub = v.sub; rp.counters = c.counters; rp.delta = (float)c.delta; rp.method = c.method; rp.citems = v.citems; rp.n_citems = v.n_citems;
    rp.viol = c.viol; rp.early = reinterpret_cast<int4*>(c.b->early_out);
    const int rc = launch_refine(rp, st);
    if (rc == SUSHI_HIP_OK) prof_end(c.pc, t0, SUSHI_HIP_STAGE_REFINE, st);
    return rc;
}

static int stage_collect(const RunCtx& c, const SubView& v, hipStream_t st, IfftArgs ia) {
    hipEvent_t t0 = prof_begin(c.pc, st);
    ia.citems = v.citems; ia.n_citems = v.n_citems;
    if (launch_method(c.method, [&](auto m) { hipLaunchKernelGGL(collect_kernel<decltype(m)::value>, dim3(COLLECT_GRID), dim3(FT), 0, st, ia); }) !=
        SUSHI_HIP_OK)
        return SUSHI_HIP_ELAUNCH;
    TileParams tp;
    tp.r = c.r; tp.searches = c.searches; tp.tiles = v.tiles; tp.cand = v.candbuf; tp.keys = c.keys; tp.counters = c.counters; tp.sub = v.sub; tp.method = c.method;
    const int rc = launch_tiles(tp, st);
    if (rc == SUSHI_HIP_OK) prof_end(c.pc, t0, SUSHI_HIP_STAGE_FINISH, st);
    return rc;
}

static int run_sub(RunCtx& c, const SubView& v, hipStream_t st) {
    SushiHipBatch* b = c.b;
    const SubBatch& sb = v.sb;
    int rc = stage_tspec(c, v, st);
    if (rc != SUSHI_HIP_OK) return rc;
    const bool exclude = sub_excludes(b->exclusion, c.suspended, sb.pairs, v.n_sub);
    c.excluded_any = c.excluded_any || exclude;
    int band = 0;
    if (exclude && (rc = decide_band(c, v, st, &band)) != SUSHI_HIP_OK) return rc;
    hipEvent_t t0 = prof_begin(c.pc, st);
    if (launch_mac(c, v, st, band != 0, nullptr, v.items) != SUSHI_HIP_OK) return SUSHI_HIP_ELAUNCH;
    prof_end(c.pc, t0, SUSHI_HIP_STAGE_MAC, st);
    t0 = prof_begin(c.pc, st);
    if (!c.cand_filled && hipMemsetAsync(v.cand, 0xff, cand_rows_bytes(sb.pairs), st) != hipSuccess)
        return SUSHI_HIP_ELAUNCH;
    IfftArgs ia;
    memset(&ia, 0, sizeof(ia));
    ia.y = (const uint2*)v.y; ia.dst_stats = c.dst->stats; ia.searches = c.searches + sb.a0; ia.n_sub = v.n_sub; ia.first_search = sb.a0;
    ia.sub_first_pair = sb.first_pair; ia.dst_len = c.dst->n; ia.delta = (float)c.delta; ia.cand = v.cand; ia.pair_lb = v.pair_lb; ia.gkeys = c.gkeys;
    ia.pairmap = v.pairmap; ia.tconst = v.tconst; ia.order = v.order; ia.urel = c.dst->urel; ia.nb = c.dst->blocks; ia.ubase = c.dst->base;
    ia.usrel = c.dst->usrel; ia.sbase = c.dst->base1; ia.flags = c.flags; ia.flag_list = c.flag_list + sb.a0; ia.sub = v.sub;
    ia.tiles = v.tiles; ia.candbuf = v.candbuf; ia.cand_cap = (int)cand_capacity(sb.pairs); ia.counters = c.counters; ia.viol = c.viol;
    if (!exclude) {
        if (launch_ifft(c, ia, (unsigned)sb.pairs, st) != SUSHI_HIP_OK) return SUSHI_HIP_ELAUNCH;
        b->last.direct_pairs += sb.pairs;
    } else {
        IfftArgs ip = ia;
        if ((rc = exclude_pairs(c, v, st, band, ip, t0)) != SUSHI_HIP_OK || (rc = transform_listed(c, v, st, ip)) != SUSHI_HIP_OK) return rc;
    }
    prof_end(c.pc, t0, SUSHI_HIP_STAGE_IFFT, st);
    if ((rc = stage_refine(c, v, st)) != SUSHI_HIP_OK) return rc;
    return stage_collect(c, v, st, ia);
}

static ListedPairs listed_pairs(const RunCtx& c, const SubView& v) {
    ListedPairs lp;
    lp.r = c.r; lp.searches = c.searches + v.sb.a0; lp.pairmap = v.pairmap; lp.sub_first_pair = v.sb.first_pair; lp.first_search = v.sb.a0;
    lp.list = v.order; lp.list_count = nullptr; lp.list_max = (int)v.sb.pairs; lp.rows = (uint32_t*)v.y; lp.method = c.method;
    return lp;
}

static void pair_run_args(const RunCtx& c, const SubView& v, PairRunArgs& a) {
    a.searches = c.searches + v.sb.a0; a.first_search = v.sb.a0; a.sub_first_pair = v.sb.first_pair; a.n_sub = v.n_sub; a.n_pairs = (int)v.sb.pairs;
    a.pairmap = v.pairmap; a.rows = (const uint32_t*)v.y; a.slb = v.slb; a.audit_mark = v.audit_mark; a.viol = c.viol;
    a.counters = c.counters; a.method = c.method;
}

static int mac_and_bound(const RunCtx& c, const SubView& v, hipStream_t st, int* band, BoundArgs& ba) {
    const int rc = decide_band(c, v, st, band);
    if (rc != SUSHI_HIP_OK) return rc;
    if (launch_mac(c, v, st, *band != 0, nullptr, v.items) != SUSHI_HIP_OK) return SUSHI_HIP_ELAUNCH;
    return bound_pairs(c, v, st, *band, ba);
}

struct ThresholdRun { double threshold; unsigned long long ukey; int32_t capacity; SushiHipHit* hits; int64_t* counts; };

static int run_sub_threshold(RunCtx& c, const SubView& v, hipStream_t st, const ThresholdRun& tr) {
    SushiHipBatch* b = c.b;
    const SubBatch& sb = v.sb;
    const bool exclude = listed_run_excludes(b->exclusion);
    ThresholdTileParams tp;
    tp.lp = listed_pairs(c, v);
    tp.threshold = tr.threshold; tp.pass = 0; tp.hits = tr.hits; tp.capacity = tr.capacity;
    ThrArgs ta;
    memset(&ta, 0, sizeof(ta));
    pair_run_args(c, v, ta);
    ta.rows_w = (uint32_t*)v.y; ta.counts_out = tr.counts;
    if (!exclude) ta.audit_mark = nullptr;
    int rc = stage_tspec(c, v, st);
    if (rc != SUSHI_HIP_OK) return rc;
    if (exclude) {
        hipLaunchKernelGGL(thr_seed_kernel, dim3((unsigned)((v.n_sub + 255) / 256)), dim3(256), 0, st, c.gkeys + sb.a0, v.n_sub, tr.ukey, v.plist);
        if (launch_ok() != SUSHI_HIP_OK) return SUSHI_HIP_ELAUNCH;
        int band = 0;
        BoundArgs ba;
        if ((rc = mac_and_bound(c, v, st, &band, ba)) != SUSHI_HIP_OK) return rc;
        hipLaunchKernelGGL(survivor_kernel, dim3((unsigned)((sb.pairs + 255) / 256)), dim3(256), 0, st, ba);
        if (launch_ok() != SUSHI_HIP_OK) return SUSHI_HIP_ELAUNCH;
        tp.lp.list = ba.slist; tp.lp.list_count = ba.scount;
        if (band) {
            if (second_look(c, v, st, ba) != SUSHI_HIP_OK) return SUSHI_HIP_ELAUNCH;
            tp.lp.list = ba.list2; tp.lp.list_count = ba.list2_count;
        }
        ta.list = tp.lp.list; ta.list_count = tp.lp.list_count;
        ta.list3 = band ? v.slist : v.slist2; ta.list3_count = v.n_list3;
    } else {
        b->last.direct_pairs += sb.pairs;
    }
    if (launch_threshold_tiles(tp, st) != SUSHI_HIP_OK) return SUSHI_HIP_ELAUNCH;
    ThresholdTileParams t3 = tp;
    if (exclude) {
        hipLaunchKernelGGL(thr_check_kernel, dim3((unsigned)std::min<int64_t>((sb.pairs + 255) / 256, 256)), dim3(256), 0, st, ta);
        hipLaunchKernelGGL(thr_extend_kernel, dim3((unsigned)((sb.pairs + 255) / 256)), dim3(256), 0, st, ta);
        if (launch_ok() != SUSHI_HIP_OK) return SUSHI_HIP_ELAUNCH;
        t3.lp.list = ta.list3; t3.lp.list_count = ta.list3_count;
        if (launch_threshold_tiles(t3, st) != SUSHI_HIP_OK) return SUSHI_HIP_ELAUNCH;
    }
    hipLaunchKernelGGL(thr_scan_kernel, dim3((unsigned)v.n_sub), dim3(256), 0, st, ta);
    if (launch_ok() != SUSHI_HIP_OK) return SUSHI_HIP_ELAUNCH;
    if (tr.capacity == 0) return SUSHI_HIP_OK;
    tp.pass = 1; t3.pass = 1;
    if (launch_threshold_tiles(tp, st) != SUSHI_HIP_OK) return SUSHI_HIP_ELAUNCH;
    if (exclude && launch_threshold_tiles(t3, st) != SUSHI_HIP_OK) return SUSHI_HIP_ELAUNCH;
    return SUSHI_HIP_OK;
}

struct BestRun { int k, min_separation, has_threshold; double threshold; unsigned long long tkey; SushiHipHit* hits; int32_t* counts; };

static int run_sub_best(RunCtx& c, const SubView& v, hipStream_t st, const BestRun& br) {
    SushiHipBatch* b = c.b;
    const SubBatch& sb = v.sb;
    const bool exclude = listed_run_excludes(b->exclusion);
    BestParams bp;
    memset(&bp, 0, sizeof(bp));
    bp.lp = listed_pairs(c, v);
    bp.n_sub = v.n_sub; bp.has_threshold = br.has_threshold; bp.threshold = br.threshold; bp.tkey = br.tkey; bp.k = br.k;
    bp.min_separation = br.min_separation; bp.gkeys = c.gkeys; bp.hits = br.hits; bp.counts = br.counts;
    int rc = stage_tspec(c, v, st);
    if (rc != SUSHI_HIP_OK) return rc;
    if (!exclude) {
        b->last.direct_pairs += sb.pairs;
        if (launch_best_tiles(bp, st) != SUSHI_HIP_OK) return SUSHI_HIP_ELAUNCH;
        return launch_best_select(bp, st);
    }
    int band = 0;
    BoundArgs ba;
    if ((rc = mac_and_bound(c, v, st, &band, ba)) != SUSHI_HIP_OK) return rc;
    BestArgs a;
    memset(&a, 0, sizeof(a));
    pair_run_args(c, v, a);
    a.k = br.k; a.order = v.order; a.gkeys = c.gkeys; a.tkey = br.tkey; a.list = v.slist; a.list_count = v.n_slist; a.flags = c.flags;
    a.need = c.flag_list; a.audit_seq = c.run_seq; a.audit_every = b->audit_every;
    bp.audit_mark = v.audit_mark; bp.stamp_flags = c.flags; bp.reset0 = v.n_slist; bp.reset1 = v.n_slist2;
    const unsigned per_pair = (unsigned)((sb.pairs + 255) / 256);
    auto evaluate = [&](const int* list, const int* count) {
        bp.lp.list = list; bp.lp.list_count = count;
        return launch_best_tiles(bp, st);
    };
    int stamp = 1;
    a.stamp = bp.stamp = stamp;
    hipLaunchKernelGGL(best_seed_kernel, dim3((unsigned)v.n_sub), dim3(256), 0, st, a);
    if (launch_ok() != SUSHI_HIP_OK) return SUSHI_HIP_ELAUNCH;
    const bool seed_look = band && br.has_threshold;
    if (seed_look && second_look(c, v, st, ba) != SUSHI_HIP_OK) return SUSHI_HIP_ELAUNCH;
    if (evaluate(seed_look ? v.slist2 : v.slist, seed_look ? v.n_slist2 : v.n_slist) != SUSHI_HIP_OK || launch_best_select(bp, st) != SUSHI_HIP_OK) return SUSHI_HIP_ELAUNCH;
    for (int round = 0; round < BEST_ROUNDS; ++round) {
        a.stamp = bp.stamp = ++stamp;
        hipLaunchKernelGGL(best_survivor_kernel, dim3(per_pair), dim3(256), 0, st, a);
        if (launch_ok() != SUSHI_HIP_OK) return SUSHI_HIP_ELAUNCH;
        if (band && second_look(c, v, st, ba) != SUSHI_HIP_OK) return SUSHI_HIP_ELAUNCH;
        if (evaluate(band ? v.slist2 : v.slist, band ? v.n_slist2 : v.n_slist) != SUSHI_HIP_OK || launch_best_select(bp, st) != SUSHI_HIP_OK) return SUSHI_HIP_ELAUNCH;
    }
    a.stamp = bp.stamp = ++stamp;
    hipLaunchKernelGGL(best_final_kernel, dim3(per_pair), dim3(256), 0, st, a);
    if (launch_ok() != SUSHI_HIP_OK || evaluate(v.slist, v.n_slist) != SUSHI_HIP_OK) return SUSHI_HIP_ELAUNCH;
    hipLaunchKernelGGL(best_check_kernel, dim3(per_pair), dim3(256), 0, st, a);
    a.list = v.slist2; a.list_count = v.n_slist2;
    hipLaunchKernelGGL(best_extend_kernel, dim3(per_pair), dim3(256), 0, st, a);
    if (launch_ok() != SUSHI_HIP_OK || evaluate(v.slist2, v.n_slist2) != SUSHI_HIP_OK) return SUSHI_HIP_ELAUNCH;
    return launch_best_select(bp, st);
}

static thread_local PlanCache g_plan_cache;

static int variant_of(int path, int variant, const SushiHipRequest* req, int n) {
    int tiles[DIRECT_CHOICES];
    for (int v = 0; v < DIRECT_CHOICES; ++v) tiles[v] = direct_variant_tile(v);
    return resolve_variant(path, variant, req, n, direct_variant_count(), tiles);
}

extern "C" {

int sushi_hip_device_prepare(void) {
    for (int l = 1; l < MAX_LANES; ++l)
        if (!g_lane_pool.get(l)) return SUSHI_HIP_ELAUNCH;
    unsigned long long* p = g_host_slots.take();
    if (!p) return SUSHI_HIP_ENOMEM;
    g_host_slots.give(p);
    return SUSHI_HIP_OK;
}

int sushi_hip_fft_size(void) { return FN; }

int sushi_hip_fft_block(void) { return FFT_SEG; }

int sushi_hip_fft_slot_of_bin(int bin) { return (bin < 0 || bin >= FN) ? -1 : sushi_fft::mslot_of_bin(bin); }

int sushi_hip_fft_low_slot_of_bin(int bin) { return sushi_fft::lslot_of_bin(bin); }

size_t sushi_hip_stream_spectra_bytes(int64_t n) { return n <= 0 ? 0 : spectra_layout(n).total; }

int sushi_hip_fft_layout(int64_t win_start, int32_t n_pos, int32_t tmpl_len, int32_t* n_pairs, int32_t* n_seg) {
    if (win_start < 0 || n_pos < 1 || tmpl_len < 1 || !n_pairs || !n_seg) return SUSHI_HIP_EINVAL;
    const FftLayout l = fft_layout(win_start, n_pos, tmpl_len);
    *n_pairs = l.n_pairs;
    *n_seg = l.n_seg;
    return SUSHI_HIP_OK;
}

int sushi_hip_stream_add_spectra(SushiHipStream* s, void* mem_dev, size_t mem_bytes, void* hip_stream) {
    if (!s || !mem_dev) return SUSHI_HIP_EINVAL;
    if ((uintptr_t)mem_dev & 255) return SUSHI_HIP_EALIGN;
    const size_t need = sushi_hip_stream_spectra_bytes(s->n);
    if (mem_bytes < need) return SUSHI_HIP_ENOSPACE;
    if (s->blocks >= 0x7fffffff) return SUSHI_HIP_EINVAL;
    SushiHipStream with = *s;
    fill_spectra(with, mem_dev, stream_layout(s->n, 0));
    if (launch_dtype(s->dtype, [&](auto t) {
            using T = std::remove_pointer_t<decltype(t)>;
            hipLaunchKernelGGL(spectra_kernel<T>, dim3((unsigned)s->blocks + 1), dim3(FT), 0, (hipStream_t)hip_stream, (const T*)s->raw, s->n,
                               (uint32_t*)with.spec, (const double*)s->stats, (uint4*)with.spec_low, with.znorm_rest, with.norm_stride); }) != SUSHI_HIP_OK)
        return SUSHI_HIP_ELAUNCH;
    *s = with;
    return SUSHI_HIP_OK;
}

size_t sushi_hip_batch_bytes(const SushiHipRequest* req_host, int n, int path, int variant, size_t workspace_cap_bytes) { return c_boundary([&]() -> size_t {
    if (!req_host || n <= 0 || (path != SUSHI_HIP_PATH_FFT && path != SUSHI_HIP_PATH_DIRECT)) return 0;
    if ((variant = variant_of(path, variant, req_host, n)) < 0) return 0;
    std::vector<SearchDesc> descs;
    int64_t tiles;
    if (make_descs(req_host, n, direct_variant_tile(variant), descs, &tiles) != SUSHI_HIP_OK) return 0;
    if (path == SUSHI_HIP_PATH_DIRECT) return batch_layout(n, path, 0, 0, 0, 0, 0).total;
    Plan plan;
    const char* lanes = getenv("SUSHI_HIP_LANES");
    if (make_plan(descs, workspace_cap_bytes, lanes, plan) != SUSHI_HIP_OK) return 0;
    const size_t total = batch_layout(n, path, plan.order.size(), plan.items.size(), plan.ws_bytes, plan.subs.size(), plan.segs).total;
    g_plan_cache.remember(req_host, n, workspace_cap_bytes, lanes, std::move(plan));
    return total;
}, 0, 0); }

static int plan_and_upload(SushiHipBatch* b, const SushiHipRequest* req_host, int n, hipStream_t st) {
    const BatchSpec spec{b->path, direct_variant_tile(b->variant), b->ws_cap, b->mem_bytes, b->dst->n, b->src->n, b->dst->dtype == SUSHI_HIP_F32 ? 4.0 : 1.0};
    const int rc = stage_batch(req_host, n, spec, getenv("SUSHI_HIP_LANES"), g_plan_cache, *b->spare);
    if (rc != SUSHI_HIP_OK) return rc;
    if (b->uploaded ? hipEventSynchronize(b->uploaded) != hipSuccess : hipEventCreateWithFlags(&b->uploaded, hipEventDisableTiming) != hipSuccess)
        return SUSHI_HIP_ELAUNCH;
    std::swap(b->now, b->spare);
    b->forget_learnt();
    b->planned = hipMemcpyAsync(b->mem + b->now->lay.desc, b->now->upload.data(), b->now->upload.size(), hipMemcpyHostToDevice, st) == hipSuccess &&
                 hipEventRecord(b->uploaded, st) == hipSuccess;
    return b->planned ? SUSHI_HIP_OK : SUSHI_HIP_ELAUNCH;
}

int sushi_hip_batch_create(const SushiHipStream* dst, const SushiHipStream* src, const SushiHipRequest* req_host, int n,
                           int path, int variant, size_t workspace_cap_bytes, void* mem_dev, size_t mem_bytes,
                           void* hip_stream, SushiHipBatch** out) { return c_boundary([&]() -> int {
    if (!dst || !src || !req_host || !mem_dev || !out || n <= 0) return SUSHI_HIP_EINVAL;
    if (path != SUSHI_HIP_PATH_FFT && path != SUSHI_HIP_PATH_DIRECT) return SUSHI_HIP_EINVAL;
    if (dst->dtype != src->dtype) return SUSHI_HIP_EINVAL;
    if ((uintptr_t)mem_dev & 255) return SUSHI_HIP_EALIGN;
    if (path == SUSHI_HIP_PATH_FFT && !dst->spec) return SUSHI_HIP_EINVAL;
    if ((variant = variant_of(path, variant, req_host, n)) < 0) return SUSHI_HIP_EINVAL;
    SushiHipBatch* b = new (std::nothrow) SushiHipBatch();
    if (!b) return SUSHI_HIP_ENOMEM;
    std::unique_ptr<SushiHipBatch> guard(b);
    b->dst = dst; b->src = src; b->n = n; b->path = path; b->variant = variant;
    b->mem = (char*)mem_dev; b->mem_bytes = mem_bytes; b->ws_cap = workspace_cap_bytes;
    const char* e = getenv("SUSHI_HIP_AUDIT_EVERY");
    if (e && *e) { const int v = atoi(e); b->audit_every = v < 0 ? 0 : v; }
    if ((b->pilot_rows = pilot_rows_route(getenv("SUSHI_HIP_PILOT_ROWS"))) < 0) return SUSHI_HIP_EINVAL;
    if ((b->rest_rows = rest_rows_route(getenv("SUSHI_HIP_REST_ROWS"))) < 0) return SUSHI_HIP_EINVAL;
    if ((b->tspec = tspec_route(getenv("SUSHI_HIP_TSPEC"))) < 0) return SUSHI_HIP_EINVAL;
    const char* m = getenv("SUSHI_HIP_BOUND_MODEL");
    if (m && !strcmp(m, "statistical")) b->bound_model = SUSHI_HIP_BOUND_STATISTICAL;
    const char* f = getenv("SUSHI_HIP_TEST_BOUND_FAULT");
    if (f && *f && !parse_bound_fault(f, &b->fault)) return SUSHI_HIP_EINVAL;
    const int rc = plan_and_upload(b, req_host, n, (hipStream_t)hip_stream);
    if (rc != SUSHI_HIP_OK) return rc;
    *out = guard.release();
    return SUSHI_HIP_OK;
}); }

int sushi_hip_batch_reset(SushiHipBatch* b, const SushiHipRequest* req_host, int n, void* hip_stream) { return c_boundary([&]() -> int {
    if (!b || !req_host || n != b->n) return SUSHI_HIP_EINVAL;
    if (b->stats_pending && b->stats_ready) { (void)hipEventSynchronize(b->stats_ready); b->stats_pending = false; }
    return plan_and_upload(b, req_host, n, (hipStream_t)hip_stream);
}); }

int sushi_hip_batch_info(const SushiHipBatch* b, SushiHipBatchInfo* info) {
    if (!b || !info) return SUSHI_HIP_EINVAL;
    memset(info, 0, sizeof(*info));
    info->n_search = b->n; info->path = b->path; info->variant = b->variant;
    info->sub_batches = b->path == SUSHI_HIP_PATH_FFT ? (int32_t)b->now->plan.subs.size() : 1;
    info->direct_tiles = b->now->n_tiles;
    info->fft_pairs = b->now->plan.pairs; info->fft_segments = b->now->plan.segs;
    info->workspace_bytes = b->now->plan.ws_bytes; info->mem_bytes = b->now->lay.total;
    info->flops = b->now->flops; info->algorithmic_bytes = b->now->algorithmic_bytes;
    info->lanes = b->path == SUSHI_HIP_PATH_FFT ? b->now->plan.lanes : 1;
    return SUSHI_HIP_OK;
}

void sushi_hip_batch_destroy(SushiHipBatch* b) { delete b; }

int sushi_hip_batch_set_method(SushiHipBatch* b, int method) {
    if (!b) return SUSHI_HIP_EINVAL;
    if (!method_known(method)) return SUSHI_HIP_EINVAL;
    b->method = method;
    return SUSHI_HIP_OK;
}

int sushi_hip_batch_set_packed_output(SushiHipBatch* b, int32_t* out_packed_dev) {
    if (!b) return SUSHI_HIP_EINVAL;
    if ((uintptr_t)out_packed_dev & 7) return SUSHI_HIP_EALIGN;
    b->packed_out = out_packed_dev;
    return SUSHI_HIP_OK;
}

int sushi_hip_batch_set_early_output(SushiHipBatch* b, int32_t* early) {
    if (!b) return SUSHI_HIP_EINVAL;
    if ((uintptr_t)early & 15) return SUSHI_HIP_EALIGN;
    b->early_out = early;
    return SUSHI_HIP_OK;
}

int sushi_hip_batch_set_exclusion(SushiHipBatch* b, int mode) {
    if (!b || mode < SUSHI_HIP_EXCLUDE_AUTO || mode > SUSHI_HIP_EXCLUDE_WHOLE) return SUSHI_HIP_EINVAL;
    b->exclusion = mode;
    return SUSHI_HIP_OK;
}

int sushi_hip_batch_set_bound_model(SushiHipBatch* b, int model) {
    if (!b || (model != SUSHI_HIP_BOUND_WORST_CASE && model != SUSHI_HIP_BOUND_STATISTICAL)) return SUSHI_HIP_EINVAL;
    b->bound_model = model;
    return SUSHI_HIP_OK;
}

int sushi_hip_batch_run(SushiHipBatch* b, double delta, int32_t* out_idx_dev, float* out_score_dev, void* hip_stream) { return c_boundary([&]() -> int {
    if (!b || !out_idx_dev || !out_score_dev || !b->planned) return SUSHI_HIP_EINVAL;
    const hipStream_t st0 = (hipStream_t)hip_stream;
    RunCtx c(b, delta);
    if (b->path == SUSHI_HIP_PATH_DIRECT) {
        if (begin_run(b, st0, RUN_ARGMIN) != SUSHI_HIP_OK) return SUSHI_HIP_ELAUNCH;
        return launch_direct(c.r, c.searches, b->n, (int)b->now->n_tiles, b->variant, b->method, c.keys, out_idx_dev, out_score_dev, b->packed_out, st0);
    }
    if (!(delta >= 3.8e-6) || delta > 1.0) return SUSHI_HIP_EINVAL;
    if (g_prof_on) { g_prof.emplace_back(); c.pc = &g_prof.back(); }
    FillArgs fa{};
    fill_add(fa, c.keys, (size_t)2 * b->n * sizeof(uint64_t), 0xffffffffu);
    if ((c.cand_filled = fills_candidate_rows(b->now->plan))) {
        const SubView v0(b->mem, b->now->lay, b->now->plan.ws_lane, b->now->plan.subs[0], 0);
        fill_add(fa, v0.cand, cand_rows_bytes(v0.sb.pairs), 0xffffffffu);
    }
    int rc = run_sub_batches(c, st0, RUN_ARGMIN, fa, [&](const SubView& v, hipStream_t st) { return run_sub(c, v, st); });
    if (rc != SUSHI_HIP_OK) return rc;
    hipEvent_t t0 = prof_begin(c.pc, st0);
    rc = launch_unpack(c.keys, b->n, b->method, out_idx_dev, out_score_dev, b->packed_out, st0);
    prof_end(c.pc, t0, SUSHI_HIP_STAGE_FINISH, st0);
    if (rc == SUSHI_HIP_OK && c.excluded_any && !b->stats_pending) {
        if (!b->host_stats) b->host_stats = g_host_slots.take();
        if (b->host_stats && !b->stats_ready && hipEventCreateWithFlags(&b->stats_ready, hipEventDisableTiming) != hipSuccess) b->stats_ready = nullptr;
        if (b->host_stats && b->stats_ready &&
            hipMemcpyAsync(b->host_stats, &c.counters->pairs_transformed, 2 * sizeof(unsigned long long), hipMemcpyDeviceToHost, st0) == hipSuccess &&
            hipEventRecord(b->stats_ready, st0) == hipSuccess)
            b->stats_pending = true;
    }
    return rc;
}); }

int sushi_hip_batch_run_threshold(SushiHipBatch* b, double threshold, int32_t capacity, SushiHipHit* out_hits_dev, int64_t* out_counts_dev,
                                  void* hip_stream) { return c_boundary([&]() -> int {
    if (!b || !out_hits_dev || !out_counts_dev || capacity < 0 || !std::isfinite(threshold) || b->path != SUSHI_HIP_PATH_FFT || !b->planned)
        return SUSHI_HIP_EINVAL;
    if (((uintptr_t)out_hits_dev & 3) || ((uintptr_t)out_counts_dev & 7)) return SUSHI_HIP_EALIGN;
    const ThresholdRun tr{threshold, ranking_key(b->method, threshold, false), capacity, out_hits_dev, out_counts_dev};
    RunCtx c(b, 0.0);
    return run_sub_batches(c, (hipStream_t)hip_stream, RUN_THRESHOLD, FillArgs{},
                           [&](const SubView& v, hipStream_t st) { return run_sub_threshold(c, v, st, tr); });
}); }

int sushi_hip_batch_run_best(SushiHipBatch* b, int32_t k, int32_t min_separation, const double* threshold, SushiHipHit* out_hits_dev,
                             int32_t* out_counts_dev, void* hip_stream) { return c_boundary([&]() -> int {
    if (!b || !out_hits_dev || !out_counts_dev || k < 1 || k > SUSHI_HIP_BEST_MAX_K || min_separation < 0 ||
        (threshold && !std::isfinite(*threshold)) || b->path != SUSHI_HIP_PATH_FFT || !b->planned)
        return SUSHI_HIP_EINVAL;
    if (((uintptr_t)out_hits_dev & 3) || ((uintptr_t)out_counts_dev & 3)) return SUSHI_HIP_EALIGN;
    const BestRun br{k, min_separation, threshold ? 1 : 0, threshold ? *threshold : 0.0,
                     threshold ? ranking_key(b->method, *threshold, true) : NO_KEY, out_hits_dev, out_counts_dev};
    RunCtx c(b, 0.0);
    return run_sub_batches(c, (hipStream_t)hip_stream, RUN_BEST, FillArgs{},
                           [&](const SubView& v, hipStream_t st) { return run_sub_best(c, v, st, br); });
}); }

int sushi_hip_batch_diagnostics(SushiHipBatch* b, SushiHipBatchDiag* diag, float* ranking_err_host, int32_t* flagged_host) { return c_boundary([&]() -> int {
    if (!b || !diag) return SUSHI_HIP_EINVAL;
    memset(diag, 0, sizeof(*diag));
    if (!b->last.ran || b->path != SUSHI_HIP_PATH_FFT) {
        if (ranking_err_host) memset(ranking_err_host, 0, (size_t)b->n * sizeof(float));
        if (flagged_host) memset(flagged_host, 0, (size_t)b->n * sizeof(int32_t));
        return SUSHI_HIP_OK;
    }
    if (hipStreamSynchronize(b->last_stream) != hipSuccess) return SUSHI_HIP_ELAUNCH;
    RunCounters c;
    if (hipMemcpy(&c, b->mem + b->now->lay.counters, sizeof(c), hipMemcpyDeviceToHost) != hipSuccess) return SUSHI_HIP_ELAUNCH;
    diag->flagged = c.n_flagged; diag->all_positions = c.n_all_positions;
    diag->tiles_dense = (int64_t)c.tiles_dense; diag->tiles_sparse = (int64_t)c.tiles_sparse;
    diag->candidates = (int64_t)c.candidates;
    memcpy(&diag->max_bound_ratio, &c.max_ratio_bits, sizeof(float));
    memcpy(&diag->max_bound_ratio_noncandidate, &c.max_ratio_audit_bits, sizeof(float));
    diag->audited = (int64_t)c.audited;
    diag->excluded_audited = (int64_t)c.excluded_audited;
    memcpy(&diag->max_slb_ratio_excluded, &c.max_slb_ratio_bits, sizeof(float));
    diag->slb_violations = c.slb_violations;
    report_last_run(b->last, b->learnt, c, diag);
    if (b->last.kind != RUN_ARGMIN) {
        if (ranking_err_host) memset(ranking_err_host, 0, (size_t)b->n * sizeof(float));
        if (flagged_host) memset(flagged_host, 0, (size_t)b->n * sizeof(int32_t));
        if (b->last.kind == RUN_BEST && flagged_host &&
            hipMemcpy(flagged_host, b->mem + b->now->lay.flags, (size_t)b->n * sizeof(int32_t), hipMemcpyDeviceToHost) != hipSuccess)
            return SUSHI_HIP_ELAUNCH;
        return SUSHI_HIP_OK;
    }
    std::vector<int32_t> fl((size_t)b->n);
    if (hipMemcpy(fl.data(), b->mem + b->now->lay.flags, (size_t)b->n * sizeof(int32_t), hipMemcpyDeviceToHost) != hipSuccess)
        return SUSHI_HIP_ELAUNCH;
    if (flagged_host) memcpy(flagged_host, fl.data(), (size_t)b->n * sizeof(int32_t));
    if (ranking_err_host) {
        std::vector<unsigned long long> g((size_t)b->n);
        if (hipMemcpy(g.data(), b->mem + b->now->lay.keys + (size_t)b->n * sizeof(unsigned long long),
                      (size_t)b->n * sizeof(unsigned long long), hipMemcpyDeviceToHost) != hipSuccess)
            return SUSHI_HIP_ELAUNCH;
        for (int k = 0; k < b->n; ++k) {
            const uint32_t bits = fl[k] ? 0u : (uint32_t)(g[k] & 0xffffffffull);
            memcpy(&ranking_err_host[k], &bits, sizeof(float));
        }
    }
    return SUSHI_HIP_OK;
}); }

int sushi_hip_batch_pair_bounds(SushiHipBatch* b, float* slb_host, float* acc_host, int64_t* n_pairs) { return c_boundary([&]() -> int {
    if (!b || !n_pairs) return SUSHI_HIP_EINVAL;
    if (!b->last.ran || b->path != SUSHI_HIP_PATH_FFT || b->now->plan.subs.empty()) { *n_pairs = 0; return SUSHI_HIP_OK; }
    if (hipStreamSynchronize(b->last_stream) != hipSuccess) return SUSHI_HIP_ELAUNCH;
    const SubView v = last_sub(b);
    const int64_t cap = *n_pairs;
    *n_pairs = v.sb.pairs;
    if (cap < v.sb.pairs) return SUSHI_HIP_ENOSPACE;
    if (slb_host && hipMemcpy(slb_host, v.slb, (size_t)v.sb.pairs * sizeof(float), hipMemcpyDeviceToHost) != hipSuccess) return SUSHI_HIP_ELAUNCH;
    if (acc_host && hipMemcpy(acc_host, v.acc, (size_t)v.sb.pairs * 2 * sizeof(float), hipMemcpyDeviceToHost) != hipSuccess) return SUSHI_HIP_ELAUNCH;
    return SUSHI_HIP_OK;
}); }

int sushi_hip_batch_workspace_view(SushiHipBatch* b, int which, void** ptr_dev, size_t* bytes) {
    if (!b || !ptr_dev || !bytes) return SUSHI_HIP_EINVAL;
    *ptr_dev = nullptr; *bytes = 0;
    if (!b->last.ran || b->path != SUSHI_HIP_PATH_FFT || b->now->plan.subs.empty()) return SUSHI_HIP_OK;
    if (hipStreamSynchronize(b->last_stream) != hipSuccess) return SUSHI_HIP_ELAUNCH;
    const SubView v = last_sub(b);
    switch (which) {
        case SUSHI_HIP_WS_TSPEC: {
            const size_t need = (size_t)v.sb.segs * ROW_BYTES;
            if (!tspec_half_rows(b->tspec)) { *ptr_dev = v.tspec; *bytes = need; break; }
            if (b->tspec_whole_bytes < need) {
                if (b->tspec_whole) (void)hipFree(b->tspec_whole);
                b->tspec_whole = nullptr; b->tspec_whole_bytes = 0;
                if (hipMalloc(&b->tspec_whole, need) != hipSuccess) { b->tspec_whole = nullptr; return SUSHI_HIP_ENOMEM; }
                b->tspec_whole_bytes = need;
            }
            const long long n_entries = (long long)v.sb.segs * ROWE;
            hipLaunchKernelGGL(tspec_expand_kernel, dim3((unsigned)std::min<long long>((n_entries + 255) / 256, 256 * 32)), dim3(256), 0, b->last_stream,
                               (const uint4*)v.tspec, (uint4*)b->tspec_whole, n_entries);
            if (launch_ok() != SUSHI_HIP_OK || hipStreamSynchronize(b->last_stream) != hipSuccess) return SUSHI_HIP_ELAUNCH;
            *ptr_dev = b->tspec_whole; *bytes = need;
            break;
        }
        case SUSHI_HIP_WS_TSPEC_HALF:
            if (!tspec_half_rows(b->tspec)) return SUSHI_HIP_EINVAL;
            *ptr_dev = v.tspec; *bytes = (size_t)v.sb.segs * HROW_BYTES;
            break;
        case SUSHI_HIP_WS_Y: *ptr_dev = v.y; *bytes = (size_t)v.sb.pairs * ROW_BYTES; break;
        case SUSHI_HIP_WS_TSPEC_LOW: *ptr_dev = v.tspec_low; *bytes = (size_t)v.sb.segs * LROW_BYTES; break;
        case SUSHI_HIP_WS_Y_LOW: *ptr_dev = v.ylow; *bytes = (size_t)v.sb.pairs * LROW_BYTES; break;
        case SUSHI_HIP_WS_TNORM_REST: *ptr_dev = v.tnorm_rest; *bytes = (size_t)v.sb.segs * sizeof(float); break;
        default: return SUSHI_HIP_EINVAL;
    }
    return SUSHI_HIP_OK;
}

int sushi_hip_profile_begin(void) {
    for (ProfCall& c : g_prof)
        for (ProfSpan& sp : c.spans) { (void)hipEventDestroy(sp.t0); (void)hipEventDestroy(sp.t1); }
    g_prof.clear();
    g_prof_on = true;
    return SUSHI_HIP_OK;
}

int sushi_hip_profile_end(float* stage_ms, int max_calls, int* n_calls) { return c_boundary([&]() -> int {
    g_prof_on = false;
    if (!stage_ms || !n_calls || max_calls < 0) return SUSHI_HIP_EINVAL;
    int out = 0;
    int rc = SUSHI_HIP_OK;
    for (ProfCall& c : g_prof) {
        if (out < max_calls && !c.spans.empty()) {
            float* row = stage_ms + (size_t)out * SUSHI_HIP_NSTAGES;
            for (int k = 0; k < SUSHI_HIP_NSTAGES; ++k) row[k] = 0.f;
            for (ProfSpan& sp : c.spans) {
                float ms = 0.f;
                if (hipEventSynchronize(sp.t1) != hipSuccess || hipEventElapsedTime(&ms, sp.t0, sp.t1) != hipSuccess) {
                    rc = SUSHI_HIP_ELAUNCH;
                    break;
                }
                if (sp.stage >= 0 && sp.stage < SUSHI_HIP_NSTAGES) row[sp.stage] += ms;
            }
            ++out;
        }
        for (ProfSpan& sp : c.spans) { (void)hipEventDestroy(sp.t0); (void)hipEventDestroy(sp.t1); }
    }
    g_prof.clear();
    *n_calls = out;
    return rc;
}); }

}
```

sushi_amd/csrc/sushi_fft_bound.inc:

```

struct BoundArgs {
    const uint2* y;
    const double* dst_stats;
    const SearchDesc* searches;
    int sub_first_pair;
    int first_search;
    int64_t dst_len;
    const int* pairmap;
    const TemplConsts* tconst;
    const double* ubase;
    const double* sbase;
    int64_t nb;
    const double* coarse;
    int64_t nc;
    float* slb;
    float* acc;
    int n_sub;
    int n_pairs;
    int* plist;
    int* slist;
    int* scount;
    const int* order;
    const unsigned long long* gkeys;
    float* pair_lb;
    RunCounters* counters;
    int band;
    int sub_first_seg;
    const float* tnorm_rest;
    const float* znorm_rest;
    int64_t norm_stride;
    int* band_votes;
    unsigned char* audit_mark;
    unsigned audit_seq;
    int audit_every;
    int worst_case;
    float half_err;
    const int* list;
    const int* list_count;
    int* list2;
    int* list2_count;
};

template <bool NEED_Q>
__global__ __launch_bounds__(256, 3)
void bound_low_kernel(BoundArgs a) {
    const int lane = threadIdx.x & 63;
    const int waves = gridDim.x * 4;
    const int gw = blockIdx.x * 4 + (threadIdx.x >> 6);
    const int64_t n_items = (int64_t)a.n_pairs * sushi_fft::LB_GROUPS;
    const sushi_fft::MfmaBl mb = sushi_fft::load_mfma_bl(lane, reinterpret_cast<const sushi_fft::uint2v*>(g_dft16_bl));
    const sushi_fft::HTwiddles tw = sushi_fft::load_htwiddles(lane, twiddles());
    const sushi_fft::uint4v* __restrict__ yh = reinterpret_cast<const sushi_fft::uint4v*>(a.y);
    auto load_item = [&](const int64_t it, sushi_fft::uint4v (&yl)[4]) {
#pragma unroll
        for (int u = 0; u < 4; ++u) yl[u] = yh[(size_t)it * (LROWE / sushi_fft::LB_GROUPS) + u * 32 + (lane & 31)];
    };
    if (gw >= a.n_pairs) return;
    sushi_fft::uint4v yl[4], yn[4];
    load_item((int64_t)gw * sushi_fft::LB_GROUPS, yl);
    for (int64_t pr = gw; pr < a.n_pairs; pr += waves) {
        float msum[sushi_fft::PER];
#pragma unroll
        for (int r = 0; r < sushi_fft::PER; ++r) msum[r] = 0.f;
        float q2 = 0.f, d2 = 0.f, dc_re = 0.f, dc_im = 0.f;
        for (int g = 0; g < sushi_fft::LB_GROUPS; ++g) {
            int64_t nx = pr * sushi_fft::LB_GROUPS + g + 1;
            if (g == sushi_fft::LB_GROUPS - 1) nx = pr + waves < a.n_pairs ? (pr + waves) * sushi_fft::LB_GROUPS : nx - 1;
            nx = nx < n_items ? nx : n_items - 1;
            load_item(nx, yn);
            __builtin_amdgcn_sched_barrier(0);
            typedef _Float16 h2 __attribute__((ext_vector_type(2)));
            if (NEED_Q) {
                float q = 0.f;
#pragma unroll
                for (int u = 0; u < 4; ++u) q = add_abs2_entry(yl[u], q);
                q2 += lane < 32 ? q : 0.f;
            }
            if (g == 0) {
                const h2 y0 = __builtin_bit_cast(h2, (unsigned)__builtin_amdgcn_readfirstlane((int)yl[0][0]));
                dc_re = (float)y0.x; dc_im = (float)y0.y;
                if ((lane & 31) == 0) yl[0][0] = 0u;
            }
            sushi_fft::h2 v[sushi_fft::PER];
            unsigned in2;
            sushi_fft::fft_wave_half_front_low(yl, v, tw, mb, in2);
            d2 += a.half_err * a.half_err * __uint_as_float(wave_max_u32(in2));
#pragma unroll
            for (int r = 0; r < sushi_fft::PER; ++r) msum[r] = __builtin_amdgcn_fdot2(v[r], v[r], msum[r], false);
#pragma unroll
            for (int u = 0; u < 4; ++u) yl[u] = yn[u];
        }
        unsigned m2 = 0u;
#pragma unroll
        for (int r = 0; r < sushi_fft::PER; ++r) m2 = sushi_fft::h_max_bits(m2, __float_as_uint(msum[r]));
        const unsigned wm = wave_max_u32(m2);
        const float qw = NEED_Q ? wave_sum_f32(q2) : 0.f;
        if (lane == 0) {
            float bw = 1.4142137f * 2.8284272f * (sqrtf(__uint_as_float(wm)) * 1.002f + sqrtf(d2)) * 1024.0f + fmaxf(dc_re, dc_im);
            if (wm >= 0x7f800000u || !(d2 < __builtin_inff())) bw = __builtin_inff();
            a.acc[2 * (size_t)pr] = bw;
            a.acc[2 * (size_t)pr + 1] = qw * 1.000001f;
        }
    }
}

constexpr int BOUND_THREADS = 256;
template <bool NEED_Q>
__global__ __launch_bounds__(BOUND_THREADS, 4)
void bound_kernel(BoundArgs a) {
    const int lane = threadIdx.x & 63;
    const int waves = gridDim.x * (BOUND_THREADS / 64);
    const int gw = blockIdx.x * (BOUND_THREADS / 64) + (threadIdx.x >> 6);
    const int64_t n_items = (int64_t)a.n_pairs * 16;
    const sushi_fft::MfmaBh mb = sushi_fft::load_mfma_bh(lane, reinterpret_cast<const sushi_fft::uint4v*>(g_dft16_bh));
    const sushi_fft::HTwiddles tw = sushi_fft::load_htwiddles(lane, twiddles());
    const sushi_fft::uint4v* __restrict__ yh = reinterpret_cast<const sushi_fft::uint4v*>(a.y);
    auto load_item = [&](const int64_t it, sushi_fft::uint4v (&yl)[4]) {
        const size_t pr = (size_t)(it >> 4);
        const int n1 = (int)(it & 15);
#pragma unroll
        for (int u = 0; u < 4; ++u) yl[u] = yh[pr * (FN / 4) + sushi_fft::wslot_uint4(n1 * 64 + lane, u)];
    };
    int64_t it = gw;
    if (it >= n_items) return;
    sushi_fft::uint4v yl[4], yn[4];
    load_item(it, yl);
    for (; it < n_items; it += waves) {
        const int64_t nx = it + waves < n_items ? it + waves : it;
        load_item(nx, yn);
        __builtin_amdgcn_sched_barrier(0);
        float q2 = 0.f;
        if (NEED_Q) {
#pragma unroll
            for (int u = 0; u < 4; ++u) q2 = add_abs2_entry(yl[u], q2);
        }
        sushi_fft::h2 v[sushi_fft::PER];
        unsigned in2;
        sushi_fft::fft_wave_half_front(yl, v, tw, mb, in2);
        unsigned m2 = 0u;
#pragma unroll
        for (int r = 0; r < sushi_fft::PER; ++r) m2 = sushi_fft::h_max_bits(m2, sushi_fft::h_abs2(v[r]));
        const unsigned wm = wave_max_u32(m2), wi = wave_max_u32(in2);
        const float qw = NEED_Q ? wave_sum_f32(q2) : 0.f;
        if (lane == 0) {
            const size_t pr = (size_t)(it >> 4);
            float bw = (sqrtf(__uint_as_float(wm)) * 1.002f + a.half_err * sqrtf(__uint_as_float(wi))) * 1024.0f;
            if (wm >= 0x7f800000u || wi >= 0x7f800000u) bw = __builtin_inff();
            atomicAdd(a.acc + 2 * pr, bw);
            if (NEED_Q) atomicMax(reinterpret_cast<unsigned*>(a.acc + 2 * pr + 1), __float_as_uint(qw));
        }
#pragma unroll
        for (int u = 0; u < 4; ++u) yl[u] = yn[u];
    }
}

template <int METHOD>
__device__ __forceinline__ void slb_one(const BoundArgs& a, const int pr, const int lane) {
    constexpr bool CC = METHOD == SUSHI_HIP_METHOD_CCOEFF_NORMED;
    const int k = __builtin_amdgcn_readfirstlane(a.pairmap[pr]);
    const SearchDesc sd = a.searches[k];
    const FftLayout lay = fft_layout(sd.win_start, sd.n_pos, sd.tmpl_len);
    const int64_t pairI = absolute_pair(lay, a.sub_first_pair, pr, sd);
    const int64_t qbase = pairI * FFT_STEP * (int64_t)FFT_SEG;
    const int M = sd.tmpl_len;
    const TemplConsts tc = a.tconst[k];
    const int64_t kA = pairI * FFT_STEP;
    const int n_seg = lay.n_seg;
    const int64_t n = a.dst_len;
    const double c = a.dst_stats[1];
    const float acc0 = a.acc[2 * (size_t)pr], acc1 = a.acc[2 * (size_t)pr + 1];
    const int64_t iA = kA < a.nb ? kA : a.nb, iB = kA + n_seg + 2 * FFT_VB < a.nb ? kA + n_seg + 2 * FFT_VB : a.nb;
    const double u0 = a.ubase[iA], u1 = a.ubase[iB], s0 = a.sbase[iA], s1 = a.sbase[iB];
    const int sl = lane < n_seg ? lane : 0;
    const int64_t jl = kA + sl < a.nb ? kA + sl : a.nb;
    float tn0 = a.tnorm_rest[(sd.first_seg - a.sub_first_seg) + sl];
    const float zn0 = a.znorm_rest[jl], an0 = a.znorm_rest[a.norm_stride + jl], bn0 = a.znorm_rest[2 * a.norm_stride + jl];
    constexpr int NSB = 2 * FH / COARSE_G;
    static_assert(NSB <= 128 && (FFT_STEP * FFT_SEG) % COARSE_G == 0, "a lane looks up two stretches");
    const int64_t plo = sd.win_start - qbase, phi = (int64_t)sd.n_pos + (sd.win_start - qbase);
    const double* __restrict__ c2 = a.coarse;
    const double* __restrict__ c1 = a.coarse + a.nc;
    auto clampi = [&](int64_t x) { return x < a.nc - 1 ? x : a.nc - 1; };
    bool use[2];
    int64_t js[2], je[2], jo0[2], jo1[2];
    double c2e[2], c2s[2], c1e[2], c1s[2], c2o1[2], c2o0[2], c1o1[2], c1o0[2];
#pragma unroll
    for (int t = 0; t < 2; ++t) {
        const int sb = lane + 64 * t;
        const int64_t p0 = (int64_t)sb * COARSE_G;
        use[t] = sb < NSB && p0 + COARSE_G > plo && p0 < phi;
        const int64_t j = qbase / COARSE_G + sb;
        js[t] = clampi(j + 1); je[t] = clampi(j + M / COARSE_G);
        c2e[t] = c2[je[t]]; c2s[t] = c2[js[t]];
        if (CC) {
            jo0[t] = clampi(j); jo1[t] = clampi(j + M / COARSE_G + 2);
            c1e[t] = c1[je[t]]; c1s[t] = c1[js[t]];
            c2o1[t] = c2[jo1[t]]; c2o0[t] = c2[jo0[t]]; c1o1[t] = c1[jo1[t]]; c1o0[t] = c1[jo0[t]];
        }
    }
    __builtin_amdgcn_sched_barrier(0);
    float wl = __builtin_inff();
#pragma unroll
    for (int t = 0; t < 2; ++t) {
        if (use[t]) {
            double e = 0.0;
            if (je[t] > js[t]) {
                if (CC) {
                    auto len = [&](int64_t lo, int64_t hi) {
                        const int64_t x0 = lo * COARSE_G < n ? lo * COARSE_G : n, x1 = hi * COARSE_G < n ? hi * COARSE_G : n;
                        return (double)(x1 - x0);
                    };
                    const double d_in = (c1e[t] - c1s[t]) - c * len(js[t], je[t]);
                    const double e_in = (c2e[t] - c2s[t]) - 2.0 * c * (c1e[t] - c1s[t]) + c * c * len(js[t], je[t]);
                    const double e_out = (c2o1[t] - c2o0[t]) - 2.0 * c * (c1o1[t] - c1o0[t]) + c * c * len(jo0[t], jo1[t]);
                    const double d_ub = fabs(d_in) + sqrt(2.0 * COARSE_G * fmax(e_out - e_in, 0.0)) * 1.000001 + 1e-6 * (fabs(d_in) + 1.0);
                    e = e_in * 0.999999 - d_ub * d_ub / (double)M - 1e-9 * (c2e[t] - c2s[t]);
                } else {
                    e = c2e[t] - c2s[t];
                }
            }
            wl = fminf(wl, fmaxf((float)e * 0.9999995f, 0.f));
        }
    }
    const float wlb = wave_min_f32(wl);
    float b_rest = 0.f;
    if (a.band) {
        const float t0n = lane < n_seg ? sqrtf(tn0) * 1.000002f : 0.f;
        float pz = t0n * zn0, pa = t0n * an0, pb = t0n * bn0;
        for (int s = lane + 64; s < n_seg; s += 64) {
            const int64_t jj = kA + s < a.nb ? kA + s : a.nb;
            const float t = sqrtf(a.tnorm_rest[(sd.first_seg - a.sub_first_seg) + s]) * 1.000002f;
            pz += t * a.znorm_rest[jj]; pa += t * a.znorm_rest[a.norm_stride + jj]; pb += t * a.znorm_rest[2 * a.norm_stride + jj];
        }
        pz = wave_sum_f32(pz); pa = wave_sum_f32(pa); pb = wave_sum_f32(pb);
        const int passes = (n_seg + MAC_SMAX_LONG - 1) / MAC_SMAX_LONG;
        b_rest = (fmaxf(pa, pb) + 1.5e-3f * pz) * tc.mac_scale * (1.0006f + 0.0005f * (float)passes) + 1e-3f;
    }
    if (lane == 0) {
        float B = acc0, qmax = acc1;
        if (a.band) {
            B = (a.band == 2 ? 0.f : B) + b_rest;
            qmax = ((a.band == 2 ? 0.f : qmax) + b_rest * b_rest) * (1.0f / (float)(FT / 64));
        }
        const int64_t s_lo = qbase < n ? qbase : n;
        const int64_t s_hi64 = (kA + n_seg + 2 * FFT_VB) * (int64_t)FFT_SEG;
        const int64_t s_hi = s_hi64 < n ? s_hi64 : n;
        const double e2 = (u1 - u0) - 2.0 * c * (s1 - s0) + c * c * (double)(s_hi - s_lo);
        const double zn_c = sqrt(fmax(e2, 0.0)) * 1.0000005, zn = sqrt(fmax(u1 - u0, 0.0)) * 1.0000005;
        const int mac_passes = (n_seg + MAC_SMAX_LONG - 1) / MAC_SMAX_LONG;
        const double sigma_y = sqrt((double)((float)(FT / 64) * qmax) * (7.9472862e-8 * (double)(2 + mac_passes)) + (double)FN * 1.2e-15) *
                               (double)tc.inv_scale;
        const double tn = CC ? (tc.inv_tnorm_c > 0.f ? 1.0 / (double)tc.inv_tnorm_c : 0.0) : (double)tc.tnorm;
        double ymax = (double)B * (double)tc.inv_scale + fabs((double)B) * (double)tc.inv_scale * 2e-5;
        if (a.worst_case) {
            const double c_wc = (double)(mac_passes + 2) * 4.8829e-4 * 1.001 + 4e-5;
            const double zn_wc = CC ? fmax(zn, zn_c) : zn_c;
            ymax += c_wc * 2.8284272 * tn * zn_wc
                  + 3.3e-10 * sqrt((double)n_seg) * tn * sqrt(fmax(a.dst_stats[0], 0.0)) + 5e-4 * (double)tc.inv_scale;
        } else {
            ymax += 5.9604645e-8 * (double)FFT_KE * (CC ? fmax(zn, zn_c) : zn_c) * tn + (double)Y_KQ * sigma_y;
        }
        float slb = -__builtin_inff();
        bool room = false;
        if (CC) {
            if (wlb > 0.f && wlb < __builtin_inff() && !tc.flat && tn > 0.0) {
                slb = (float)(1.0 - ymax / (tn * sqrt((double)wlb)) * 1.000001);
                room = slb > 0.55f;
            }
        } else {
            const double t0 = tc.tU - 2.0 * (double)tc.c_sum_t;
            const double a0 = t0 - 2.0 * ymax;
            if (wlb > 0.f && wlb < __builtin_inff() && a0 < (double)wlb && tc.tU > 0.0) {
                slb = (float)((a0 + (double)wlb) / (sqrt((double)wlb) * (double)tc.tnorm) * 0.999999);
                room = a0 + (double)wlb >= 0.55 * (t0 + (double)wlb);
            }
        }
        a.slb[pr] = slb;
        if (a.band == 2) {
            int* __restrict__ v = a.band_votes + (size_t)(pr & (VOTE_SLOTS - 1)) * VOTE_STRIDE;
            atomicAdd(v, 1);
            if (room) atomicAdd(v + 1, 1);
        }
    }
}
template <int METHOD>
__global__ __launch_bounds__(256)
void slb_kernel(BoundArgs a) {
    const int pr = __builtin_amdgcn_readfirstlane(blockIdx.x * 4 + (threadIdx.x >> 6));
    if (pr >= a.n_pairs) return;
    slb_one<METHOD>(a, pr, threadIdx.x & 63);
}
template <int METHOD>
__global__ __launch_bounds__(256)
void slb_list_kernel(BoundArgs a) {
    const int n = *a.list_count;
    if (n > a.n_pairs / 5) return;
    const int waves = gridDim.x * 4;
    for (int slot = blockIdx.x * 4 + (threadIdx.x >> 6); slot < n; slot += waves)
        slb_one<METHOD>(a, __builtin_amdgcn_readfirstlane(a.list[slot]), threadIdx.x & 63);
}

struct BoundFaultArgs {
    const SearchDesc* searches;
    const int* pairmap;
    float* slb;
    int first_search, sub_first_pair, n_pairs;
    BoundFault f;
};
__global__ __launch_bounds__(256)
void bound_fault_kernel(BoundFaultArgs a) {
    const int pr = blockIdx.x * 256 + threadIdx.x;
    if (pr >= a.n_pairs) return;
    const int k = a.pairmap[pr];
    if ((unsigned)(a.first_search + k) % (unsigned)a.f.period != (unsigned)a.f.phase) return;
    if (a.f.pair >= 0 && pair_of_search(a.sub_first_pair, pr, a.searches[k]) != a.f.pair) return;
    a.slb[pr] = __builtin_inff();
}

__global__ __launch_bounds__(64)
void pilot_kernel(BoundArgs a) {
    const int k = blockIdx.x, lane = threadIdx.x;
    const SearchDesc sd = a.searches[k];
    const FftLayout lay = fft_layout(sd.win_start, sd.n_pos, sd.tmpl_len);
    const int p0 = first_pair_in_sub(a.sub_first_pair, sd);
    unsigned long long best = NO_KEY;
    for (int i = lane; i < lay.n_pairs; i += 64) {
        const float s = a.slb[p0 + i];
        const unsigned long long key = ((unsigned long long)ordered_bits(__float_as_uint(s)) << 32) | (unsigned)i;
        best = key < best ? key : best;
    }
    best = wave_min_u64(best);
    if (lane == 0) {
        a.plist[k] = p0 + (int)(best & 0xffffffffull);
        if (k == 0) *a.scount = 0;
        atomicAdd(&a.counters->pairs_transformed, 1ull);
    }
}

__device__ __forceinline__ bool bound_excludes(const float* slb, const int pr, const unsigned long long gkey) {
    const float U = gkey == NO_KEY ? __builtin_inff() : key_score(gkey);
    return U < 0.9999f && slb[pr] > U * 1.000001f + 1e-7f;
}

template <class Args>
__device__ __forceinline__ bool audited_search(const Args& a, const int k) {
    return a.audit_every > 0 && ((unsigned)(a.first_search + k) + a.audit_seq) % (unsigned)a.audit_every == 0u;
}
template <class Args>
__device__ __forceinline__ int audit_pair_of(const Args& a, const SearchDesc& sd, const int k) {
    const FftLayout lay = fft_layout(sd.win_start, sd.n_pos, sd.tmpl_len);
    const unsigned h = ((unsigned)(a.first_search + k) * 2654435761u + a.audit_seq * 40503u) >> 9;
    return (int)(h % (unsigned)lay.n_pairs);
}
template <class Args>
__device__ __forceinline__ bool is_audit_pair(const Args& a, const int pr, const int k) {
    if (!audited_search(a, k)) return false;
    const SearchDesc sd = a.searches[k];
    return audit_pair_of(a, sd, k) == pair_of_search(a.sub_first_pair, pr, sd);
}

__device__ __forceinline__ void append_pairs(int* list, int* count, RunCounters* counters, const bool add, const int pr) {
    const unsigned long long m = __ballot(add);
    const int lane = threadIdx.x & 63;
    int base = 0;
    if (lane == 0 && m) {
        base = atomicAdd(count, __popcll(m));
        atomicAdd(&counters->pairs_transformed, (unsigned long long)__popcll(m));
    }
    base = __shfl(base, 0, 64);
    if (add) list[base + __popcll(m & ((1ull << lane) - 1ull))] = pr;
}

__global__ __launch_bounds__(256)
void survivor_kernel(BoundArgs a) {
    const int b = blockIdx.x * 256 + threadIdx.x;
    bool keep = false;
    int pr = 0;
    if (b < a.n_pairs) {
        pr = a.order[b];
        const int k = a.pairmap[pr];
        bool audit = false;
        if (a.plist[k] != pr) {
            const bool excluded = bound_excludes(a.slb, pr, a.gkeys[a.first_search + k]);
            if (excluded && audited_search(a, k)) {
                const SearchDesc sd = a.searches[k];
                audit = audit_pair_of(a, sd, k) == a.sub_first_pair + pr - sd.first_pair;
            }
            if (excluded && !audit) a.pair_lb[pr] = __builtin_inff();
            keep = !excluded || audit;
        }
        if (a.audit_mark) a.audit_mark[pr] = (audit ? MARK_AUDITED : 0) | (keep ? MARK_LISTED : 0);
    }
    append_pairs(a.slist, a.scount, a.counters, keep, pr);
}

enum { ROWS_MARKED = 0, ROWS_FIRST = 1, ROWS_REST = 2, ROWS_ITEMS = 3 };
struct MacRowsArgs {
    const uint4* spec;
    int64_t spec_blocks;
    const uint4* tspec;
    int tspec_half;
    uint4* y;
    const SearchDesc* searches;
    const TemplConsts* tconst;
    const unsigned char* mark;
    int n_sub;
    int sub_first_seg;
    int sub_first_pair;
    const int* dense_search;
    const int* plist;
    int first_search;
    unsigned audit_seq;
    int audit_every;
    const int* items;
    const int* item_count;
    const int* pairmap;
    int n_pairs;
};
template <int SMAX>
__device__ __forceinline__ void mac_row_of_pair(const MacRowsArgs& a, const FftLayout& lay, const sushi_mac::h8 (&tt)[SMAX],
                                                const uint4* __restrict__ zsp, const int p0, const int ip, const float sy, const int e,
                                                const int z_zero) {
    typedef _Float16 h2 __attribute__((ext_vector_type(2)));
    const long long I = lay.pair0 + ip;
    sushi_mac::acc4 acc = sushi_mac::zero_acc();
#pragma unroll
    for (int s6 = 0; s6 < SMAX; s6 += 6) {
        sushi_mac::h8 z[6];
#pragma unroll
        for (int t = 0; t < 6; ++t) {
            const long long jj = s6 + t < lay.n_seg ? FFT_STEP * I + s6 + t : (long long)z_zero;
            z[t] = as_h8(zsp[(size_t)(jj < z_zero ? jj : z_zero) * ROWE]);
        }
#pragma unroll
        for (int t = 0; t < 6; ++t) {
            const sushi_mac::zrow zr = {z[t], sushi_mac::rot_mi(z[t])};
            sushi_mac::mac4(acc, tt[s6 + t], zr);
        }
    }
    unsigned o[sushi_mac::BINS];
#pragma unroll
    for (int q = 0; q < sushi_mac::BINS; ++q) {
        const h2 h = {(_Float16)(acc.re[q] * sy), (_Float16)(acc.im[q] * sy)};
        o[q] = __builtin_bit_cast(unsigned, h);
    }
    a.y[(size_t)(p0 + ip) * ROWE + e] = uint4{o[0], o[1], o[2], o[3]};
}
template <int SMAX>
__device__ __forceinline__ void mac_rows_first_paired(const MacRowsArgs& a, const SearchDesc& sd, const FftLayout& lay, const int k,
                                                      const float sy, const int h, const int z_zero) {
    const uint4* __restrict__ hrow = a.tspec + (size_t)(sd.first_seg - a.sub_first_seg) * HROWE;
    const int e_own = sushi_fft::half_to_full(h), e_mir = sushi_fft::half_mirror_of(h);
    const int p0 = first_pair_in_sub(a.sub_first_pair, sd);
    const int audit = audited_search(a, k) ? audit_pair_of(a, sd, k) : -1;
    const int pilot = a.plist[k] - p0;
    const bool two = audit >= 0 && audit < lay.n_pairs && audit != pilot;
    sushi_mac::h8 tt[SMAX];
#pragma unroll
    for (int s = 0; s < SMAX; ++s) tt[s] = s < lay.n_seg ? as_h8(hrow[(size_t)s * HROWE + h]) : sushi_mac::zero_h8();
    mac_row_of_pair<SMAX>(a, lay, tt, a.spec + e_own, p0, pilot, sy, e_own, z_zero);
    if (two) mac_row_of_pair<SMAX>(a, lay, tt, a.spec + e_own, p0, audit, sy, e_own, z_zero);
    if ((h & ~16) == 0) {
        const int hx = sushi_fft::half_entry(1024, h >> 4);
#pragma unroll
        for (int s = 0; s < SMAX; ++s) tt[s] = s < lay.n_seg ? as_h8(hrow[(size_t)s * HROWE + hx]) : sushi_mac::zero_h8();
    }
#pragma unroll
    for (int s = 0; s < SMAX; ++s) tt[s] = as_h8(sushi_fft::real_conjrev(as_uint4(tt[s])));
    mac_row_of_pair<SMAX>(a, lay, tt, a.spec + e_mir, p0, pilot, sy, e_mir, z_zero);
    if (two) mac_row_of_pair<SMAX>(a, lay, tt, a.spec + e_mir, p0, audit, sy, e_mir, z_zero);
}
template <int SMAX, int MODE>
__device__ __forceinline__ void mac_rows_of_search(const MacRowsArgs& a, const SearchDesc& sd, const FftLayout& lay, const int k,
                                                   const float sy, const int e, unsigned long long (*masks)[4], const int z_zero) {
    if (MODE == ROWS_FIRST && a.tspec_half) { mac_rows_first_paired<SMAX>(a, sd, lay, k, sy, e, z_zero); return; }
    const TspecLane tsp = tspec_lane(a.tspec, a.tspec_half, (size_t)(sd.first_seg - a.sub_first_seg), e);
    const uint4* __restrict__ zsp = a.spec + e;
    const int p0 = first_pair_in_sub(a.sub_first_pair, sd);
    const int tid = threadIdx.x;
    int audit = -1;
    if (MODE != ROWS_MARKED && audited_search(a, k)) audit = audit_pair_of(a, sd, k);
    if (MODE == ROWS_REST) {
        bool any = false;
        for (int i = tid; i < lay.n_pairs; i += MACL_THREADS) any = any || (i != audit && (a.mark[p0 + i] & MARK_LISTED));
        if (!__syncthreads_or(any)) return;
    }
    sushi_mac::h8 tt[SMAX];
#pragma unroll
    for (int s = 0; s < SMAX; ++s) tt[s] = s < lay.n_seg ? as_h8(tspec_entry(tsp, (size_t)s)) : sushi_mac::zero_h8();
    if (MODE == ROWS_FIRST) {
        const int pilot = a.plist[k] - p0;
        mac_row_of_pair<SMAX>(a, lay, tt, zsp, p0, pilot, sy, e, z_zero);
        if (audit >= 0 && audit < lay.n_pairs && audit != pilot) mac_row_of_pair<SMAX>(a, lay, tt, zsp, p0, audit, sy, e, z_zero);
        return;
    }
    for (int base = 0; base < lay.n_pairs; base += MACL_THREADS) {
        __syncthreads();
        const int i = base + tid;
        const bool on = i < lay.n_pairs && (MODE == ROWS_MARKED || i != audit) && (a.mark[p0 + i] & MARK_LISTED);
        const unsigned long long bm = __ballot(on);
        if ((tid & 63) == 0) (*masks)[tid >> 6] = bm;
        __syncthreads();
        for (int w = 0; w < 4; ++w) {
            unsigned long long m = (*masks)[w];
            while (m) {
                const int bit = __builtin_ctzll(m);
                m &= m - 1;
                mac_row_of_pair<SMAX>(a, lay, tt, zsp, p0, base + 64 * w + bit, sy, e, z_zero);
            }
        }
    }
}
template <int SMAX>
__device__ __forceinline__ void mac_rows_of_item(const MacRowsArgs& a, const SearchDesc& sd, const FftLayout& lay, const int k,
                                                 const float sy, const int e, const int z_zero, const int first) {
    const TspecLane tsp = tspec_lane(a.tspec, a.tspec_half, (size_t)(sd.first_seg - a.sub_first_seg), e);
    const uint4* __restrict__ zsp = a.spec + e;
    const int p0 = first_pair_in_sub(a.sub_first_pair, sd);
    const int audit = audited_search(a, k) ? audit_pair_of(a, sd, k) : -1;
    sushi_mac::h8 tt[SMAX];
#pragma unroll
    for (int s = 0; s < SMAX; ++s) tt[s] = s < lay.n_seg ? as_h8(tspec_entry(tsp, (size_t)s)) : sushi_mac::zero_h8();
    int room = REST_ITEM_PAIRS;
    for (int base = first; base < lay.n_pairs && room > 0; base += 64) {
        const int i = base + (threadIdx.x & 63);
        const bool on = i < lay.n_pairs && rest_pair_to_form(a.mark[p0 + i] & MARK_LISTED, i, audit);
        unsigned long long m = rest_item_take(__ballot(on), room);
        room -= __popcll(m);
        while (m) {
            const int bit = __builtin_ctzll(m);
            m &= m - 1;
            mac_row_of_pair<SMAX>(a, lay, tt, zsp, p0, base + bit, sy, e, z_zero);
        }
    }
}
template <int LONG, int MODE>
__global__ __launch_bounds__(MACL_THREADS)
void mac_rows_kernel(MacRowsArgs a) {
    __shared__ unsigned long long masks[4];
    const int z_zero = (int)(a.spec_blocks < 0x7fffffff ? a.spec_blocks : 0x7fffffff);
    if (MODE == ROWS_ITEMS) {
        const int listed = *a.item_count;
        const int n_items = listed < a.n_pairs ? listed : a.n_pairs;
        for (long long it = blockIdx.x; it < (long long)n_items * MACL_PARTS; it += gridDim.x) {
            const int first = __builtin_amdgcn_readfirstlane(a.items[it / MACL_PARTS]);
            if ((unsigned)first >= (unsigned)a.n_pairs) continue;
            const int k = __builtin_amdgcn_readfirstlane(a.pairmap[first]);
            if ((unsigned)k >= (unsigned)a.n_sub || a.dense_search[k]) continue;
            const int e = (int)(it % MACL_PARTS) * MACL_THREADS + threadIdx.x;
            const SearchDesc sd = a.searches[k];
            const FftLayout lay = fft_layout(sd.win_start, sd.n_pos, sd.tmpl_len);
            const float sy = a.tconst[k].mac_scale;
            const int i0 = first - first_pair_in_sub(a.sub_first_pair, sd);
            if ((unsigned)i0 >= (unsigned)lay.n_pairs) continue;
            if (LONG) {
                if (lay.n_seg > MAC_SMAX_SHORT && lay.n_seg <= MAC_SMAX_LONG) mac_rows_of_item<MAC_SMAX_LONG>(a, sd, lay, k, sy, e, z_zero, i0);
            } else {
                if (lay.n_seg <= 6) mac_rows_of_item<6>(a, sd, lay, k, sy, e, z_zero, i0);
                else if (lay.n_seg <= 12) mac_rows_of_item<12>(a, sd, lay, k, sy, e, z_zero, i0);
                else if (lay.n_seg <= MAC_SMAX_SHORT) mac_rows_of_item<MAC_SMAX_SHORT>(a, sd, lay, k, sy, e, z_zero, i0);
            }
        }
        return;
    }
    const int parts = MODE == ROWS_FIRST && a.tspec_half ? MACL_PARTS / 2 : MACL_PARTS;
    for (long long it = blockIdx.x; it < (long long)a.n_sub * parts; it += gridDim.x) {
        const int k = (int)(it / parts);
        if (MODE != ROWS_FIRST && a.dense_search[k]) continue;
        const int e = (int)(it % parts) * MACL_THREADS + threadIdx.x;
        const SearchDesc sd = a.searches[k];
        const FftLayout lay = fft_layout(sd.win_start, sd.n_pos, sd.tmpl_len);
        const float sy = a.tconst[k].mac_scale;
        if (LONG) {
            if (lay.n_seg > MAC_SMAX_SHORT && lay.n_seg <= MAC_SMAX_LONG) mac_rows_of_search<MAC_SMAX_LONG, MODE>(a, sd, lay, k, sy, e, &masks, z_zero);
        } else {
            if (lay.n_seg <= 6) mac_rows_of_search<6, MODE>(a, sd, lay, k, sy, e, &masks, z_zero);
            else if (lay.n_seg <= 12) mac_rows_of_search<12, MODE>(a, sd, lay, k, sy, e, &masks, z_zero);
            else if (lay.n_seg <= MAC_SMAX_SHORT) mac_rows_of_search<MAC_SMAX_SHORT, MODE>(a, sd, lay, k, sy, e, &masks, z_zero);
        }
    }
}

constexpr int BLE_LOGN = 13;
constexpr int BLE_N = sushi_fft::Plan<BLE_LOGN>::N, BLE_T = sushi_fft::Plan<BLE_LOGN>::NT;
static_assert(BLE_N == FN / 2, "the low band sampled at every second position");
__global__ __launch_bounds__(BLE_T)
void bound_low_exact_kernel(BoundArgs a) {
    __shared__ __attribute__((aligned(16))) float lds[sushi_fft::lds_floats<BLE_LOGN>()];
    __shared__ unsigned red[BLE_T / 64];
    typedef _Float16 h2 __attribute__((ext_vector_type(2)));
    const int n = *a.list_count;
    if (n > a.n_pairs / 5) return;
    for (int slot = blockIdx.x; slot < n; slot += gridDim.x) {
        int tid = threadIdx.x;
        asm volatile("" : "+v"(tid));
        const sushi_fft::Twiddles tw = sushi_fft::load_twiddles<BLE_LOGN, 1>(tid, twiddles());
        const int pr = a.list[slot];
        const uint32_t* __restrict__ row = reinterpret_cast<const uint32_t*>(a.y) + (size_t)pr * (LROWE * 4);
        cpx v[sushi_fft::PER];
        float dc_re = 0.f, dc_im = 0.f;
#pragma unroll
        for (int r = 0; r < sushi_fft::PER; ++r) {
            const int kin = sushi_fft::in_index<BLE_LOGN>(tid, r);
            const bool in_band = kin < FN / 8 || kin >= 3 * FN / 8;
            const int ls = sushi_fft::lslot_of_bin(kin < FN / 8 ? kin : (in_band ? kin + FN / 2 : 0));
            const h2 h = __builtin_bit_cast(h2, in_band ? row[ls] : 0u);
            v[r] = cpx{(float)h.x, (float)h.y};
            if (kin == 0) { dc_re = v[r].x; dc_im = v[r].y; v[r] = cpx{0.f, 0.f}; }
        }
        sushi_fft::fft_split<BLE_LOGN, 1>(v, tid, lds, tw);
        float m2 = 0.f;
#pragma unroll
        for (int r = 0; r < sushi_fft::PER; ++r) m2 = fmaxf(m2, v[r].x * v[r].x + v[r].y * v[r].y);
        const unsigned wm = wave_max_u32(__float_as_uint(m2));
        __syncthreads();
        if ((tid & 63) == 0) red[tid >> 6] = wm;
        __syncthreads();
        if (tid == 0) {
            unsigned mm = 0u;
#pragma unroll
            for (int i = 0; i < BLE_T / 64; ++i) mm = red[i] > mm ? red[i] : mm;
            float bw = 1.4142137f * sqrtf(__uint_as_float(mm)) * 1.0007f + fmaxf(dc_re, dc_im);
            if (mm >= 0x7f800000u) bw = __builtin_inff();
            a.acc[2 * (size_t)pr] = fminf(a.acc[2 * (size_t)pr], bw);
        }
        __syncthreads();
    }
}
__global__ __launch_bounds__(256)
void survivor2_kernel(BoundArgs a) {
    const int n = *a.list_count;
    const bool second_look = n <= a.n_pairs / 5;
    for (int base = blockIdx.x * 256; base < n; base += gridDim.x * 256) {
        const int slot = base + threadIdx.x;
        bool keep = false;
        int pr = 0;
        if (slot < n) {
            pr = a.list[slot];
            keep = true;
            if (second_look && !(a.audit_mark[pr] & MARK_AUDITED)) {
                const int k = a.pairmap[pr];
                if (bound_excludes(a.slb, pr, a.gkeys[a.first_search + k])) {
                    const unsigned h = ((unsigned)(a.sub_first_pair + pr) * 2654435761u + a.audit_seq * 40503u) >> 11;
                    if (a.audit_every > 0 && h % (16u * (unsigned)a.audit_every) == 0u) {
                        a.audit_mark[pr] = MARK_AUDITED | MARK_LISTED | MARK_SECOND_LOOK;
                    } else {
                        keep = false;
                        a.pair_lb[pr] = __builtin_inff();
                        a.audit_mark[pr] = 0;
                    }
                }
            }
        }
        const unsigned long long m = __ballot(keep), act = __ballot(slot < n);
        const int lane = threadIdx.x & 63;
        const int dropped = __popcll(act) - __popcll(m);
        int b0 = 0;
        if (lane == 0 && m) b0 = atomicAdd(a.list2_count, __popcll(m));
        if (lane == 0 && dropped > 0)
            atomicAdd(&a.counters->pairs_transformed, (unsigned long long)0 - (unsigned long long)dropped);
        b0 = __shfl(b0, 0, 64);
        if (keep) a.list2[b0 + __popcll(m & ((1ull << lane) - 1ull))] = pr;
    }
}

__global__ __launch_bounds__(64)
void dense_search_kernel(BoundArgs a, int* __restrict__ dense_search, int* __restrict__ any, int* __restrict__ items,
                         int* __restrict__ item_count) {
    const int lane = threadIdx.x;
    const int k = blockIdx.x;
    const SearchDesc sd = a.searches[k];
    const FftLayout lay = fft_layout(sd.win_start, sd.n_pos, sd.tmpl_len);
    const int p0 = first_pair_in_sub(a.sub_first_pair, sd);
    const int audit = items && audited_search(a, k) ? audit_pair_of(a, sd, k) : -1;
    int listed = 0, formed = 0;
    for (int base = 0; base < lay.n_pairs; base += 64) {
        const int i = base + lane;
        const int on = i < lay.n_pairs ? (a.audit_mark[p0 + i] & MARK_LISTED) : 0;
        listed += on ? 1 : 0;
        if (items) {
            const unsigned long long form = __ballot(rest_pair_to_form(on, i, audit));
            const unsigned long long starts = rest_item_starts(form, formed, REST_ITEM_PAIRS);
            formed += __popcll(form);
            if (starts) {
                int slot = 0;
                if (lane == 0) slot = atomicAdd(item_count, __popcll(starts));
                slot = __shfl(slot, 0, 64) + __popcll(starts & ((1ull << lane) - 1ull));
                if (((starts >> lane) & 1ull) && slot < a.n_pairs) items[slot] = p0 + i;
            }
        }
    }
#pragma unroll
    for (int d = 32; d >= 1; d >>= 1) listed += __shfl_xor(listed, d, 64);
    if (lane == 0) {
        const int dense = listed * 5 > lay.n_pairs * 2 ? 1 : 0;
        dense_search[k] = dense;
        if (dense) atomicAdd(any, listed);
    }
}

constexpr int REPACK_THREADS = 1024;
__global__ __launch_bounds__(REPACK_THREADS)
void dense_repack_kernel(const int* __restrict__ items0, int n_items0, const int* __restrict__ items1, int n_items1,
                         int* __restrict__ dense_search, int n_search, int* __restrict__ out0, int* __restrict__ out1,
                         const int* __restrict__ listed_dense, int min_listed, int* __restrict__ any) {
    if (*listed_dense < min_listed) {
        if (blockIdx.x == 0) for (int k = threadIdx.x; k < n_search; k += REPACK_THREADS) dense_search[k] = 0;
        return;
    }
    if (threadIdx.x == 0) *any = 1;
    const int* __restrict__ items = blockIdx.x == 0 ? items0 : items1;
    const int n_items = blockIdx.x == 0 ? n_items0 : n_items1;
    int* __restrict__ out = blockIdx.x == 0 ? out0 : out1;
    if (n_items == 0) return;
    __shared__ int wave_tot[REPACK_THREADS / 64];
    __shared__ int carry_s, out_base_s;
    const int tid = threadIdx.x, lane = tid & 63, wave = tid >> 6;
    for (int e = tid; e < n_items * (1 + MAC_SPW); e += REPACK_THREADS) out[e] = -1;
    if (tid == 0) out_base_s = 0;
    __syncthreads();
    const int n_ent = n_items * MAC_SPW;
    for (int c = 0; c < MAC_CLASSES; ++c) {
        if (tid == 0) carry_s = 0;
        __syncthreads();
        for (int e0 = 0; e0 < n_ent; e0 += REPACK_THREADS) {
            const int e = e0 + tid;
            int member = -1;
            if (e < n_ent) {
                const int* __restrict__ item = items + (size_t)(e / MAC_SPW) * (1 + MAC_SPW);
                const int k = item[1 + e % MAC_SPW];
                if (item[0] == c && k >= 0 && dense_search[k] != 0) member = k;
            }
            const unsigned long long m = __ballot(member >= 0);
            if (lane == 0) wave_tot[wave] = __popcll(m);
            __syncthreads();
            int before = carry_s;
            for (int w = 0; w < wave; ++w) before += wave_tot[w];
            if (member >= 0) {
                const int pos = before + __popcll(m & ((1ull << lane) - 1ull));
                int* __restrict__ o = out + (size_t)(out_base_s + pos / MAC_SPW) * (1 + MAC_SPW);
                o[1 + pos % MAC_SPW] = member;
                if (pos % MAC_SPW == 0) o[0] = c;
            }
            __syncthreads();
            if (tid == 0) { int t = 0; for (int w = 0; w < REPACK_THREADS / 64; ++w) t += wave_tot[w]; carry_s += t; }
            __syncthreads();
        }
        if (tid == 0) out_base_s += (carry_s + MAC_SPW - 1) / MAC_SPW;
        __syncthreads();
    }
}
```

sushi_amd/csrc/sushi_geometry.hpp:

```cpp
#ifndef SUSHI_GEOMETRY_HPP
#define SUSHI_GEOMETRY_HPP

#include <stddef.h>
#include <stdint.h>

#include "../../include/sushi_hip.h"

#ifdef __HIPCC__
#define SUSHI_GEOM_HD __host__ __device__
#else
#define SUSHI_GEOM_HD
#endif

namespace sushi {

constexpr int FFT_LOGN = 14;
constexpr int FFT_N = 1 << FFT_LOGN;
constexpr int FFT_SEG = 4096;
constexpr int FFT_HOP = FFT_SEG;
constexpr int FFT_VB = FFT_N / FFT_SEG - 1;
constexpr int FFT_H = FFT_VB * FFT_SEG;
constexpr int FFT_STEP = 2 * FFT_VB;
constexpr int FFT_CAND = 8;
constexpr int FFT_AUDIT = 4;
constexpr int AUDIT_RUNS = 4;
constexpr int FFT_ROW = 32;
static_assert(FFT_CAND + 2 + AUDIT_RUNS * FFT_AUDIT <= FFT_ROW, "candidates, overflow marker, error bound, audit runs");
constexpr int TILE = 1024;
constexpr int TILES_PER_PAIR = 2 * FFT_H / TILE;
constexpr int COARSE_G = 256;

struct FftLayout { int64_t pair0; int n_pairs; int n_seg; };
SUSHI_GEOM_HD inline FftLayout fft_layout(int64_t win_start, int n_pos, int tmpl_len) {
    FftLayout l;
    l.pair0 = (win_start / FFT_SEG) / FFT_STEP;
    const int64_t pair_last = ((win_start + n_pos - 1) / FFT_SEG) / FFT_STEP;
    l.n_pairs = (int)(pair_last - l.pair0 + 1);
    l.n_seg = (tmpl_len + FFT_SEG - 1) / FFT_SEG;
    return l;
}

constexpr int MAC_CLASSES = 5;
constexpr int MAC_SHORT_CLASSES = 3;
SUSHI_GEOM_HD constexpr int mac_class_smax(int c) { return FFT_STEP * (c + 1); }
SUSHI_GEOM_HD inline int mac_class(int n_seg) {
    for (int c = 0; c < MAC_CLASSES - 1; ++c)
        if (n_seg <= mac_class_smax(c)) return c;
    return MAC_CLASSES - 1;
}

SUSHI_GEOM_HD inline bool method_known(int method) {
    return method == SUSHI_HIP_METHOD_SQDIFF_NORMED || method == SUSHI_HIP_METHOD_CCOEFF_NORMED;
}

inline size_t align_up(size_t x, size_t a) { return (x + a - 1) / a * a; }

constexpr int32_t REQUEST_MAX_TERM = 0x7fffffff - 65536;
inline bool request_fits(const SushiHipRequest& r, int64_t dst_n, int64_t src_n) {
    if (r.tmpl_len < 1 || r.n_pos < 1 || r.win_start < 0 || r.tmpl_off < 0) return false;
    if (r.n_pos > REQUEST_MAX_TERM || r.tmpl_len > REQUEST_MAX_TERM) return false;
    return r.tmpl_len <= src_n - r.tmpl_off && (int64_t)r.n_pos + r.tmpl_len - 1 <= dst_n - r.win_start;
}

struct SearchDesc {
    int64_t tmpl_off;
    int64_t win_start;
    int32_t tmpl_len;
    int32_t n_pos;
    int32_t first_tile;
    int32_t first_pair;
    int32_t first_seg;
    int32_t reserved;
};
static_assert(sizeof(SearchDesc) == 40, "SearchDesc layout");

constexpr int SPARSE_TILE_MAX = 256;
constexpr int SPARSE_UNIT = 64;
struct TileDesc {
    int32_t search;
    int32_t p0;
    int32_t off;
    int32_t cnt;
};

struct SubCounters {
    int32_t n_tiles;
    int32_t tile_next;
    int32_t n_cand;
    int32_t sub_flagged;
};

struct RunCounters {
    int32_t n_flagged;
    int32_t n_all_positions;
    unsigned long long tiles_dense, tiles_sparse, candidates;
    uint32_t max_ratio_bits;
    uint32_t max_ratio_audit_bits;
    unsigned long long audited;
    unsigned long long pairs_transformed;
    unsigned long long excluded_audited;
    uint32_t max_slb_ratio_bits;
    int32_t slb_violations;
    unsigned long long second_look_audited;
};

struct TemplConsts {
    double tU;
    float inv_tnorm;
    float tnorm;
    float tmean;
    float inv_tnorm_c;
    float inv_m;
    int flat;
    float c_sum_t;
    float inv_scale;
    float mac_scale;
};

constexpr int ROW_BYTES = FFT_N * 4;
constexpr int ROWE = FFT_N / 4;
constexpr int LROWE = FFT_N / 16;
constexpr int LROW_BYTES = LROWE * 16;
constexpr int HROWE = ROWE / 2 + 16;
constexpr int HROW_BYTES = HROWE * 16;
struct SpectraLayout { size_t low, norms, total; int64_t norm_stride; };
inline SpectraLayout spectra_layout(int64_t n) {
    const size_t rows = (size_t)((n + FFT_SEG - 1) / FFT_SEG + 1), norm_bytes = align_up(rows * sizeof(float), 256);
    SpectraLayout l;
    l.low = rows * ROW_BYTES; l.norms = l.low + rows * LROW_BYTES; l.total = l.norms + 3 * norm_bytes;
    l.norm_stride = (int64_t)(norm_bytes / sizeof(float));
    return l;
}

constexpr int MAC_SPW = 8;
constexpr int MAC_BPW = 64 / MAC_SPW;
constexpr int MAC_WAVES = 4;
constexpr int MAC_THREADS = MAC_WAVES * 64;
constexpr int MAC_BW = MAC_BPW * MAC_WAVES;
constexpr int MAC_DUMMY_LINES = 1024;
constexpr int MAC_CHUNKS = ROWE / MAC_BW;
static_assert(MAC_CHUNKS % 8 == 0, "every XCD owns the same number of bin chunks");

constexpr int VOTE_SLOTS = 64, VOTE_STRIDE = 32;

}
#endif
```

sushi_amd/device.py:

```python
import ctypes
import os
import threading
import time

import numpy as np
import torch

from . import _native
from .axis import method_code
from .common import SushiError
from .rowcheck import DTYPE_CODE as _DTYPE_CODE


def _require_gpu(device=None):
    if not torch.cuda.is_available():
        raise SushiError("sushi_amd needs a ROCm GPU (MI355X / gfx950): torch.cuda.is_available() is False "
                         "and there is no CPU fallback")
    return torch.device("cuda", torch.cuda.current_device()) if device is None else torch.device(device)


_warms = {}
_warm_lock = threading.Lock()


# ... 310 lines not shown
            return False
        _native.check(rc, "sushi_hip_batch_reset")
        self.requests = req
        self._read_info()
        return True

    def set_packed_output(self, packed):
        self._host_rec = None
        if self._early is not None:
            _native.check(_native.lib().sushi_hip_batch_set_early_output(self._handle, None), "sushi_hip_batch_set_early_output")
            self._early = self._early_np = None
        if packed is None:
            _native.check(_native.lib().sushi_hip_batch_set_packed_output(self._handle, None), "sushi_hip_batch_set_packed_output")
            self._packed = None
            return
        if packed.dtype != torch.int32 or not packed.is_cuda or not packed.is_contiguous() or packed.dim() != 2 or \
                packed.shape[1] != 2 or packed.shape[0] < self.n:
            raise SushiError("packed output: a contiguous int32 CUDA tensor [>= n, 2]")
        _native.check(_native.lib().sushi_hip_batch_set_packed_output(self._handle, packed.data_ptr()), "sushi_hip_batch_set_packed_output")
        self._packed = packed

    def set_method(self, method):
        _native.check(_native.lib().sushi_hip_batch_set_method(self._handle, method_code(method)), "sushi_hip_batch_set_method")
        self.method = method

    def set_bound_model(self, model):
        if model not in _native.BOUND_MODEL:
            raise SushiError("bound model must be one of %s" % sorted(_native.BOUND_MODEL))
        _native.check(_native.lib().sushi_hip_batch_set_bound_model(self._handle, _native.BOUND_MODEL[model]),
                      "sushi_hip_batch_set_bound_model")

    def run(self, hip_stream=None):
        st = _raw_stream(self.dst.device) if hip_stream is None else hip_stream
        if self._early_np is not None:
            self._early_np[:, 2] = 0
        rc = _native.lib().sushi_hip_batch_run(self._handle, self.delta, self.out_idx.data_ptr(),
                                               self.out_score.data_ptr(), st)
        _native.check(rc, "sushi_hip_batch_run")
        return self.out_idx, self.out_score

    def run_threshold(self, threshold, capacity, hip_stream=None):
        if self.path != "fft":
            raise SushiError("threshold runs need the FFT path")
        capacity = int(capacity)
        if capacity < 0:
            raise SushiError("capacity must be >= 0")
        threshold = float(threshold)
        if not np.isfinite(threshold):
            raise SushiError("threshold must be finite")
        dev = self.dst.device
        with torch.cuda.device(dev):
            hits = torch.empty((self.n, capacity, 2), dtype=torch.int32, device=dev)
            counts = torch.empty(self.n, dtype=torch.int64, device=dev)
            hp = hits.data_ptr() if hits.numel() else counts.data_ptr()
            st = _raw_stream(dev) if hip_stream is None else hip_stream
            rc = _native.lib().sushi_hip_batch_run_threshold(self._handle, threshold, capacity, hp, counts.data_ptr(), st)
            _native.check(rc, "sushi_hip_batch_run_threshold")
        return hits, counts

    def occurrences(self, threshold, capacity=None):
        cap = 4096 if capacity is None else int(capacity)
        hits, counts = self.run_threshold(threshold, cap)
        cnt = counts.cpu().numpy()
        need = int(cnt.max()) if cnt.size else 0
        if need > cap:
            hits, counts = self.run_threshold(threshold, need)
            cnt = counts.cpu().numpy()
            cap = need
        return _hit_lists(hits.cpu().numpy() if cap else np.zeros((self.n, 0, 2), np.int32), cnt)

    def run_best(self, k, min_separation=None, threshold=None, hip_stream=None):
        if self.path != "fft":
            raise SushiError("best-k runs need the FFT path")
        k = int(k)
        if not 1 <= k <= _native.BEST_MAX_K:
            raise SushiError("k must be in 1..%d" % _native.BEST_MAX_K)
        sep = 0 if min_separation is None else int(min_separation)
        if sep < 1 and min_separation is not None:
            raise SushiError("min_separation must be >= 1 (None: each request's tmpl_len)")
        thr = None
        if threshold is not None:
            threshold = float(threshold)
            if not np.isfinite(threshold):
                raise SushiError("threshold must be finite")
            thr = ctypes.byref(ctypes.c_double(threshold))
        dev = self.dst.device
        with torch.cuda.device(dev):
            hits = torch.empty((self.n, k, 2), dtype=torch.int32, device=dev)
            counts = torch.empty(self.n, dtype=torch.int32, device=dev)
            st = _raw_stream(dev) if hip_stream is None else hip_stream
            rc = _native.lib().sushi_hip_batch_run_best(self._handle, k, sep, thr, hits.data_ptr(), counts.data_ptr(), st)
            _native.check(rc, "sushi_hip_batch_run_best")
        return hits, counts

    def best(self, k, min_separation=None, threshold=None):
        hits, counts = self.run_best(k, min_separation, threshold)
        return _hit_lists(hits.cpu().numpy(), counts.cpu().numpy())

    def results(self):
        if self._early_np is not None:
            e = self._early_np
            t_end = time.perf_counter() + 2e-3
            while not e[:, 2].all():
                if time.perf_counter() > t_end:
                    break
            else:
                if not e[:, 3].any():
                    return e[:, 0].copy(), e[:, 1].copy().view(np.float32)
        if self._host_rec is not None:
            torch.cuda.current_stream(self.dst.device).synchronize()
            rec = self._host_rec.numpy()
            return rec[:, 0].copy(), rec[:, 1].copy().view(np.float32)
        if self._packed is not None:
            rec = self._packed[:self.n].cpu().numpy()
            return np.ascontiguousarray(rec[:, 0]), np.ascontiguousarray(rec[:, 1]).view(np.float32)
        return self.out_idx.cpu().numpy(), self.out_score.cpu().numpy()

    def diagnostics(self, per_search=False):
        d = _native.BatchDiag()
        err = np.zeros(self.n, np.float32) if per_search else None
        flg = np.zeros(self.n, np.int32) if per_search else None
        rc = _native.lib().sushi_hip_batch_diagnostics(self._handle, ctypes.byref(d),
                                                       err.ctypes.data if per_search else None,
                                                       flg.ctypes.data if per_search else None)
        _native.check(rc, "sushi_hip_batch_diagnostics")
        out = {k: getattr(d, k) for k, _ in _native.BatchDiag._fields_ if k != "reserved"}
        out["band_votes"] = [int(v) for v in d.band_votes]
        if per_search:
            out["ranking_err"], out["flagged_per_search"] = err, flg
        return out

    def pair_bounds(self):
        n = ctypes.c_int64(int(self.fft_pairs))
        slb = np.empty(int(self.fft_pairs), np.float32)
        acc = np.empty((int(self.fft_pairs), 2), np.float32)
        _native.check(_native.lib().sushi_hip_batch_pair_bounds(self._handle, slb.ctypes.data, acc.ctypes.data, ctypes.byref(n)),
                      "sushi_hip_batch_pair_bounds")
        return slb[:n.value], acc[:n.value]

    def workspace_view(self, which):
        ptr, nbytes = ctypes.c_void_p(), ctypes.c_size_t(0)
        _native.check(_native.lib().sushi_hip_batch_workspace_view(self._handle, int(which), ctypes.byref(ptr), ctypes.byref(nbytes)),
                      "sushi_hip_batch_workspace_view")
        if not ptr.value:
            return None
        off = ptr.value - self._mem.data_ptr()
        if 0 <= off and off + nbytes.value <= self._mem.numel():
            return self._mem[off:off + nbytes.value].view(torch.float16)
        class _Foreign:
            __cuda_array_interface__ = {"shape": (nbytes.value,), "typestr": "|u1", "data": (ptr.value, False), "version": 2}
        with torch.cuda.device(self._mem.device):
            return torch.as_tensor(_Foreign(), device=self._mem.device).clone().view(torch.float16)

    def ranking_errors(self):
        return self.diagnostics(per_search=True)["ranking_err"]

    def fallback_count(self):
        return int(self.diagnostics()["flagged"]) if self.path == "fft" else 0
```

Baseline: 409,200 events/s.

## Split SLB bound across 16-lane rows, pipeline second-look FFT, block-level list appends

Result: faster. 424,100 events/s (median of 6 runs) (+3.6%).

```diff
diff --git a/include/sushi_hip.h b/include/sushi_hip.h
--- a/include/sushi_hip.h
+++ b/include/sushi_hip.h
@@ -135,12 +135,19 @@
 SUSHI_HIP_API int sushi_hip_batch_diagnostics(SushiHipBatch* batch, SushiHipBatchDiag* diag, float* ranking_err_host,
                                               int32_t* flagged_host);
 SUSHI_HIP_API int sushi_hip_batch_pair_bounds(SushiHipBatch* batch, float* slb_host, float* acc_host, int64_t* n_pairs);
+SUSHI_HIP_API int sushi_hip_batch_bounds_again(SushiHipBatch* batch, int by_wave, int pass, float* slb_host, int32_t* votes_host,
+                                               int64_t* n_pairs);
 #define SUSHI_HIP_WS_TSPEC 0
 #define SUSHI_HIP_WS_Y 1
 #define SUSHI_HIP_WS_TSPEC_LOW 2
 #define SUSHI_HIP_WS_Y_LOW 3
 #define SUSHI_HIP_WS_TNORM_REST 4
 #define SUSHI_HIP_WS_TSPEC_HALF 5
+#define SUSHI_HIP_WS_SLIST 6
+#define SUSHI_HIP_WS_SLIST2 7
+#define SUSHI_HIP_WS_SCOUNT 8
+#define SUSHI_HIP_WS_MARKS 9
+#define SUSHI_HIP_WS_PAIR_LB 10
 SUSHI_HIP_API int sushi_hip_batch_workspace_view(SushiHipBatch* batch, int which, void** ptr_dev, size_t* bytes);
 SUSHI_HIP_API void sushi_hip_batch_destroy(SushiHipBatch* batch);
 
diff --git a/sushi_amd/_native.py b/sushi_amd/_native.py
--- a/sushi_amd/_native.py
+++ b/sushi_amd/_native.py
@@ -32,6 +32,7 @@
                  "finish": "collect_kernel+exact_tiles_kernel+unpack_keys_kernel", "bound": "bound_low_kernel|bound_kernel"}
 EXCLUSION = {"auto": 0, "always": 1, "never": 2, "band": 3, "whole": 4}
 WS_TSPEC, WS_Y, WS_TSPEC_LOW, WS_Y_LOW, WS_TNORM_REST, WS_TSPEC_HALF = range(6)
+WS_SLIST, WS_SLIST2, WS_SCOUNT, WS_MARKS, WS_PAIR_LB = range(6, 11)
 BOUND_MODEL = {"worst_case": 0, "statistical": 1}
 STAGE_KERNEL_SETS = {"tspec": ("tspec_real_kernel", "tspec_kernel"), "mac": ("mac_kernel", "mac_long_kernel"),
                      "ifft": ("ifft_kernel", "ifft_list_kernel", "pilot_kernel", "survivor_kernel", "mac_list_kernel", "mac_rows_kernel",
@@ -149,6 +150,9 @@
     L.sushi_hip_batch_set_bound_model.argtypes = [vp, ci]
     L.sushi_hip_batch_pair_bounds.restype = ci
     L.sushi_hip_batch_pair_bounds.argtypes = [vp, vp, vp, ctypes.POINTER(i64)]
+    if hasattr(L, "sushi_hip_batch_bounds_again"):
+        L.sushi_hip_batch_bounds_again.restype = ci
+        L.sushi_hip_batch_bounds_again.argtypes = [vp, ci, ci, vp, vp, ctypes.POINTER(i64)]
     L.sushi_hip_batch_workspace_view.restype = ci
     L.sushi_hip_batch_workspace_view.argtypes = [vp, ci, pvp, ctypes.POINTER(sz)]
     L.sushi_hip_batch_destroy.restype = None
diff --git a/sushi_amd/csrc/fft_core.hpp b/sushi_amd/csrc/fft_core.hpp
--- a/sushi_amd/csrc/fft_core.hpp
+++ b/sushi_amd/csrc/fft_core.hpp
@@ -667,6 +667,9 @@
     const int j = b == 0 ? 0 : (b == 2 ? 1 : (b == 12 ? 2 : 3));
     return (((g * 4 + (d2 >> 2)) * 32 + 16 * kq + ((d3 << 2) | (d2 & 3))) << 2) + j;
 }
+SUSHI_HHD constexpr bool sl_in_band(int r) { return (r & 7) < 2 || (r & 7) >= 6; }
+SUSHI_HHD constexpr int sl_sub(int r) { return (r & 7) < 2 ? (r & 7) : (r & 7) - 4; }
+SUSHI_HHD int sl_entry(int tid, int b) { return lslot_of_bin(2 * tid + b) >> 2; }
 SUSHI_HHD double dft16_low_operand(int form, int l, int j) {
     const int kq = l >> 4, n = l & 15, part = kq >> 1, d1 = lb_d1(kq & 1, j);
     const double PI = 3.14159265358979323846;
diff --git a/sushi_amd/csrc/run_policy.hpp b/sushi_amd/csrc/run_policy.hpp
--- a/sushi_amd/csrc/run_policy.hpp
+++ b/sushi_amd/csrc/run_policy.hpp
@@ -108,6 +108,20 @@
 }
 inline bool rest_rows_by_item(int route) { return route != REST_ROWS_BY_SEARCH; }
 
+enum { SLB_BY_GROUP = 0, SLB_BY_WAVE = 1 };
+inline int slb_route(const char* setting) {
+    if (!setting || !*setting || !strcmp(setting, "group")) return SLB_BY_GROUP;
+    return !strcmp(setting, "wave") ? SLB_BY_WAVE : -1;
+}
+inline bool slb_by_wave(int route) { return route == SLB_BY_WAVE; }
+
+enum { SECOND_LOOK_AHEAD = 0, SECOND_LOOK_PLAIN = 1 };
+inline int second_look_route(const char* setting) {
+    if (!setting || !*setting || !strcmp(setting, "ahead")) return SECOND_LOOK_AHEAD;
+    return !strcmp(setting, "plain") ? SECOND_LOOK_PLAIN : -1;
+}
+inline bool second_look_plain(int route) { return route == SECOND_LOOK_PLAIN; }
+
 #ifndef SUSHI_REST_ITEM_PAIRS
 #define SUSHI_REST_ITEM_PAIRS 4
 #endif
diff --git a/sushi_amd/csrc/sushi_fft.hip b/sushi_amd/csrc/sushi_fft.hip
--- a/sushi_amd/csrc/sushi_fft.hip
+++ b/sushi_amd/csrc/sushi_fft.hip
@@ -99,7 +99,11 @@
     int pilot_rows = PILOT_ROWS_BY_SEARCH;
     int rest_rows = REST_ROWS_BY_ITEM;
     int tspec = TSPEC_REAL;
+    int slb = SLB_BY_GROUP;
+    int second_look = SECOND_LOOK_AHEAD;
     int bound_model = SUSHI_HIP_BOUND_WORST_CASE;
+    BoundArgs last_bounds;
+    int last_bounds_method = -1;
     BoundFault fault;
     unsigned long long* host_stats = nullptr;
     hipEvent_t stats_ready = nullptr;
@@ -272,8 +276,10 @@
 }
 
 static int launch_slb(const RunCtx& c, const SubView& v, const BoundArgs& x, hipStream_t st) {
+    constexpr int per_group = 4 * (64 / SLB_GROUP);
     return launch_method(c.method, [&](auto m) {
-        hipLaunchKernelGGL(slb_kernel<decltype(m)::value>, dim3((unsigned)((v.sb.pairs + 3) / 4)), dim3(256), 0, st, x); });
+        if (slb_by_wave(c.b->slb)) hipLaunchKernelGGL(slb_wave_kernel<decltype(m)::value>, dim3((unsigned)((v.sb.pairs + 3) / 4)), dim3(256), 0, st, x);
+        else hipLaunchKernelGGL(slb_kernel<decltype(m)::value>, dim3((unsigned)((v.sb.pairs + per_group - 1) / per_group)), dim3(256), 0, st, x); });
 }
 
 static int launch_bound_fault(const RunCtx& c, const SubView& v, hipStream_t st) {
@@ -383,6 +389,7 @@
     };
     if (ba.worst_case) go(std::false_type()); else go(std::true_type());
     if (launch_ok() != SUSHI_HIP_OK || launch_slb(c, v, ba, st) != SUSHI_HIP_OK) return SUSHI_HIP_ELAUNCH;
+    c.b->last_bounds = ba; c.b->last_bounds_method = c.method;
     if (c.b->fault.period > 0) return launch_bound_fault(c, v, st);
     return SUSHI_HIP_OK;
 }
@@ -390,10 +397,12 @@
 static int second_look(const RunCtx& c, const SubView& v, hipStream_t st, BoundArgs& ba) {
     ba.list = ba.slist; ba.list_count = ba.scount;
     ba.list2 = v.slist2; ba.list2_count = v.n_slist2;
-    hipLaunchKernelGGL(bound_low_exact_kernel, dim3(256 * 4), dim3(BLE_T), 0, st, ba);
+    if (second_look_plain(c.b->second_look)) hipLaunchKernelGGL(bound_low_exact_plain_kernel, dim3(256 * 4), dim3(BLE_T), 0, st, ba);
+    else hipLaunchKernelGGL(bound_low_exact_kernel, dim3(256 * 4), dim3(BLE_T), 0, st, ba);
     if (launch_ok() != SUSHI_HIP_OK) return SUSHI_HIP_ELAUNCH;
-    if (launch_method(c.method, [&](auto m) { hipLaunchKernelGGL(slb_list_kernel<decltype(m)::value>, dim3(256 * 2), dim3(256), 0, st, ba); }) !=
-        SUSHI_HIP_OK)
+    if (launch_method(c.method, [&](auto m) {
+            if (slb_by_wave(c.b->slb)) hipLaunchKernelGGL(slb_list_wave_kernel<decltype(m)::value>, dim3(256 * 2), dim3(256), 0, st, ba);
+            else hipLaunchKernelGGL(slb_list_kernel<decltype(m)::value>, dim3(256 * 2), dim3(256), 0, st, ba); }) != SUSHI_HIP_OK)
         return SUSHI_HIP_ELAUNCH;
     if (c.b->fault.period > 0 && launch_bound_fault(c, v, st) != SUSHI_HIP_OK) return SUSHI_HIP_ELAUNCH;
     hipLaunchKernelGGL(survivor2_kernel, dim3(256), dim3(256), 0, st, ba);
@@ -414,7 +423,7 @@
     if (band && by_search && launch_mac_rows(c, v, st, ba, ROWS_FIRST) != SUSHI_HIP_OK) return SUSHI_HIP_ELAUNCH;
     if (band && launch_mac_list(c, v, st, ba.plist, nullptr, v.n_sub, nullptr, by_search ? 1 : 0) != SUSHI_HIP_OK) return SUSHI_HIP_ELAUNCH;
     if (launch_ifft(c, ip, (unsigned)v.n_sub, st) != SUSHI_HIP_OK) return SUSHI_HIP_ELAUNCH;
-    hipLaunchKernelGGL(survivor_kernel, dim3((unsigned)((sb.pairs + 255) / 256)), dim3(256), 0, st, ba);
+    hipLaunchKernelGGL(survivor_kernel, dim3((unsigned)((sb.pairs + SURVIVOR_THREADS - 1) / SURVIVOR_THREADS)), dim3(SURVIVOR_THREADS), 0, st, ba);
     if (launch_ok() != SUSHI_HIP_OK) return SUSHI_HIP_ELAUNCH;
     ip.order = ba.slist; ip.count = ba.scount; ip.audit_mark = ba.audit_mark;
     if (!band) return SUSHI_HIP_OK;
@@ -545,7 +554,7 @@
         int band = 0;
         BoundArgs ba;
         if ((rc = mac_and_bound(c, v, st, &band, ba)) != SUSHI_HIP_OK) return rc;
-        hipLaunchKernelGGL(survivor_kernel, dim3((unsigned)((sb.pairs + 255) / 256)), dim3(256), 0, st, ba);
+        hipLaunchKernelGGL(survivor_kernel, dim3((unsigned)((sb.pairs + SURVIVOR_THREADS - 1) / SURVIVOR_THREADS)), dim3(SURVIVOR_THREADS), 0, st, ba);
         if (launch_ok() != SUSHI_HIP_OK) return SUSHI_HIP_ELAUNCH;
         tp.lp.list = ba.slist; tp.lp.list_count = ba.scount;
         if (band) {
@@ -708,6 +717,7 @@
         return SUSHI_HIP_ELAUNCH;
     std::swap(b->now, b->spare);
     b->forget_learnt();
+    b->last_bounds_method = -1;
     b->planned = hipMemcpyAsync(b->mem + b->now->lay.desc, b->now->upload.data(), b->now->upload.size(), hipMemcpyHostToDevice, st) == hipSuccess &&
                  hipEventRecord(b->uploaded, st) == hipSuccess;
     return b->planned ? SUSHI_HIP_OK : SUSHI_HIP_ELAUNCH;
@@ -732,6 +742,8 @@
     if ((b->pilot_rows = pilot_rows_route(getenv("SUSHI_HIP_PILOT_ROWS"))) < 0) return SUSHI_HIP_EINVAL;
     if ((b->rest_rows = rest_rows_route(getenv("SUSHI_HIP_REST_ROWS"))) < 0) return SUSHI_HIP_EINVAL;
     if ((b->tspec = tspec_route(getenv("SUSHI_HIP_TSPEC"))) < 0) return SUSHI_HIP_EINVAL;
+    if ((b->slb = slb_route(getenv("SUSHI_HIP_SLB"))) < 0) return SUSHI_HIP_EINVAL;
+    if ((b->second_look = second_look_route(getenv("SUSHI_HIP_SECOND_LOOK"))) < 0) return SUSHI_HIP_EINVAL;
     const char* m = getenv("SUSHI_HIP_BOUND_MODEL");
     if (m && !strcmp(m, "statistical")) b->bound_model = SUSHI_HIP_BOUND_STATISTICAL;
     const char* f = getenv("SUSHI_HIP_TEST_BOUND_FAULT");
@@ -908,6 +920,45 @@
     if (cap < v.sb.pairs) return SUSHI_HIP_ENOSPACE;
     if (slb_host && hipMemcpy(slb_host, v.slb, (size_t)v.sb.pairs * sizeof(float), hipMemcpyDeviceToHost) != hipSuccess) return SUSHI_HIP_ELAUNCH;
     if (acc_host && hipMemcpy(acc_host, v.acc, (size_t)v.sb.pairs * 2 * sizeof(float), hipMemcpyDeviceToHost) != hipSuccess) return SUSHI_HIP_ELAUNCH;
+    return SUSHI_HIP_OK;
+}); }
+
+int sushi_hip_batch_bounds_again(SushiHipBatch* b, int by_wave, int pass, float* slb_host, int32_t* votes_host, int64_t* n_pairs) {
+    return c_boundary([&]() -> int {
+    if (!b || !n_pairs || pass < 0 || pass > 2 || (by_wave != 0 && by_wave != 1)) return SUSHI_HIP_EINVAL;
+    if (!b->last.ran || b->path != SUSHI_HIP_PATH_FFT || b->last_bounds_method < 0) { *n_pairs = 0; return SUSHI_HIP_OK; }
+    hipStream_t st = b->last_stream;
+    if (hipStreamSynchronize(st) != hipSuccess) return SUSHI_HIP_ELAUNCH;
+    BoundArgs ba = b->last_bounds;
+    const int64_t cap = *n_pairs;
+    *n_pairs = ba.n_pairs;
+    if (slb_host && cap < ba.n_pairs) return SUSHI_HIP_ENOSPACE;
+    int votes[VOTE_SLOTS * VOTE_STRIDE];
+    if (pass == 2) {
+        ba.band = 2;
+        if (hipMemsetAsync(ba.band_votes, 0, sizeof(votes), st) != hipSuccess) return SUSHI_HIP_ELAUNCH;
+    }
+    if (pass == 1) {
+        if (ba.band != 1) return SUSHI_HIP_EINVAL;
+        const SubView v = last_sub(b);
+        ba.list = v.slist2; ba.list_count = v.n_slist2;
+    }
+    constexpr int per_group = 4 * (64 / SLB_GROUP);
+    const int rc = launch_method(b->last_bounds_method, [&](auto m) {
+        constexpr int M = decltype(m)::value;
+        if (pass == 1 && by_wave) hipLaunchKernelGGL(slb_list_wave_kernel<M>, dim3(256 * 2), dim3(256), 0, st, ba);
+        else if (pass == 1) hipLaunchKernelGGL(slb_list_kernel<M>, dim3(256 * 2), dim3(256), 0, st, ba);
+        else if (by_wave) hipLaunchKernelGGL(slb_wave_kernel<M>, dim3((unsigned)((ba.n_pairs + 3) / 4)), dim3(256), 0, st, ba);
+        else hipLaunchKernelGGL(slb_kernel<M>, dim3((unsigned)((ba.n_pairs + per_group - 1) / per_group)), dim3(256), 0, st, ba); });
+    if (rc != SUSHI_HIP_OK) return rc;
+    if (pass == 2 && hipMemcpyAsync(votes, ba.band_votes, sizeof(votes), hipMemcpyDeviceToHost, st) != hipSuccess) return SUSHI_HIP_ELAUNCH;
+    if (slb_host && hipMemcpyAsync(slb_host, ba.slb, (size_t)ba.n_pairs * sizeof(float), hipMemcpyDeviceToHost, st) != hipSuccess)
+        return SUSHI_HIP_ELAUNCH;
+    if (hipStreamSynchronize(st) != hipSuccess) return SUSHI_HIP_ELAUNCH;
+    if (pass == 2 && votes_host) {
+        votes_host[0] = votes_host[1] = 0;
+        for (int k = 0; k < VOTE_SLOTS; ++k) { votes_host[0] += votes[k * VOTE_STRIDE]; votes_host[1] += votes[k * VOTE_STRIDE + 1]; }
+    }
     return SUSHI_HIP_OK;
 }); }
 
@@ -942,6 +993,11 @@
         case SUSHI_HIP_WS_TSPEC_LOW: *ptr_dev = v.tspec_low; *bytes = (size_t)v.sb.segs * LROW_BYTES; break;
         case SUSHI_HIP_WS_Y_LOW: *ptr_dev = v.ylow; *bytes = (size_t)v.sb.pairs * LROW_BYTES; break;
         case SUSHI_HIP_WS_TNORM_REST: *ptr_dev = v.tnorm_rest; *bytes = (size_t)v.sb.segs * sizeof(float); break;
+        case SUSHI_HIP_WS_SLIST: *ptr_dev = v.slist; *bytes = (size_t)v.sb.pairs * sizeof(int); break;
+        case SUSHI_HIP_WS_SLIST2: *ptr_dev = v.slist2; *bytes = (size_t)v.sb.pairs * sizeof(int); break;
+        case SUSHI_HIP_WS_SCOUNT: *ptr_dev = v.n_slist; *bytes = (size_t)SC_WORDS * sizeof(int); break;
+        case SUSHI_HIP_WS_MARKS: *ptr_dev = v.audit_mark; *bytes = (size_t)v.sb.pairs; break;
+        case SUSHI_HIP_WS_PAIR_LB: *ptr_dev = v.pair_lb; *bytes = (size_t)v.sb.pairs * sizeof(float); break;
         default: return SUSHI_HIP_EINVAL;
     }
     return SUSHI_HIP_OK;
diff --git a/sushi_amd/csrc/sushi_fft_bound.inc b/sushi_amd/csrc/sushi_fft_bound.inc
--- a/sushi_amd/csrc/sushi_fft_bound.inc
+++ b/sushi_amd/csrc/sushi_fft_bound.inc
@@ -154,11 +154,11 @@
     }
 }
 
-template <int METHOD>
-__device__ __forceinline__ void slb_one(const BoundArgs& a, const int pr, const int lane) {
+constexpr int SLB_GROUP = 16;
+template <int METHOD, int GROUP>
+__device__ __forceinline__ void slb_body(const BoundArgs& a, const int pr, const int lane, const bool live, const int k, const SearchDesc sd) {
     constexpr bool CC = METHOD == SUSHI_HIP_METHOD_CCOEFF_NORMED;
-    const int k = __builtin_amdgcn_readfirstlane(a.pairmap[pr]);
-    const SearchDesc sd = a.searches[k];
+    static_assert(GROUP == 64 || GROUP == SLB_GROUP, "a wave or a row of sixteen lanes");
     const FftLayout lay = fft_layout(sd.win_start, sd.n_pos, sd.tmpl_len);
     const int64_t pairI = absolute_pair(lay, a.sub_first_pair, pr, sd);
     const int64_t qbase = pairI * FFT_STEP * (int64_t)FFT_SEG;
@@ -177,16 +177,18 @@
     const float zn0 = a.znorm_rest[jl], an0 = a.znorm_rest[a.norm_stride + jl], bn0 = a.znorm_rest[2 * a.norm_stride + jl];
     constexpr int NSB = 2 * FH / COARSE_G;
     static_assert(NSB <= 128 && (FFT_STEP * FFT_SEG) % COARSE_G == 0, "a lane looks up two stretches");
+    constexpr int NSL = slb_stretches_a_lane(GROUP);
+    static_assert(NSL * GROUP >= NSB && (GROUP == 64 ? NSL == 2 : NSL * GROUP == NSB), "the group's lanes cover the stretches");
     const int64_t plo = sd.win_start - qbase, phi = (int64_t)sd.n_pos + (sd.win_start - qbase);
     const double* __restrict__ c2 = a.coarse;
     const double* __restrict__ c1 = a.coarse + a.nc;
     auto clampi = [&](int64_t x) { return x < a.nc - 1 ? x : a.nc - 1; };
-    bool use[2];
-    int64_t js[2], je[2], jo0[2], jo1[2];
-    double c2e[2], c2s[2], c1e[2], c1s[2], c2o1[2], c2o0[2], c1o1[2], c1o0[2];
-#pragma unroll
-    for (int t = 0; t < 2; ++t) {
-        const int sb = lane + 64 * t;
+    bool use[NSL];
+    int64_t js[NSL], je[NSL], jo0[NSL], jo1[NSL];
+    double c2e[NSL], c2s[NSL], c1e[NSL], c1s[NSL], c2o1[NSL], c2o0[NSL], c1o1[NSL], c1o0[NSL];
+#pragma unroll
+    for (int t = 0; t < NSL; ++t) {
+        const int sb = slb_stretch(lane, t, GROUP);
         const int64_t p0 = (int64_t)sb * COARSE_G;
         use[t] = sb < NSB && p0 + COARSE_G > plo && p0 < phi;
         const int64_t j = qbase / COARSE_G + sb;
@@ -201,7 +203,7 @@
     __builtin_amdgcn_sched_barrier(0);
     float wl = __builtin_inff();
 #pragma unroll
-    for (int t = 0; t < 2; ++t) {
+    for (int t = 0; t < NSL; ++t) {
         if (use[t]) {
             double e = 0.0;
             if (je[t] > js[t]) {
@@ -222,21 +224,32 @@
             wl = fminf(wl, fmaxf((float)e * 0.9999995f, 0.f));
         }
     }
-    const float wlb = wave_min_f32(wl);
+    auto group_min = [](float v) {
+        if constexpr (GROUP == 64) return wave_min_f32(v);
+        else return row_reduce_f32(v, [](float x, float y) { return fminf(x, y); });
+    };
+    auto group_sum = [](float v) {
+        if constexpr (GROUP == 64) return wave_sum_f32(v);
+        else return row_reduce_f32(v, [](float x, float y) { return x + y; });
+    };
+    const float wlb = group_min(wl);
     float b_rest = 0.f;
     if (a.band) {
         const float t0n = lane < n_seg ? sqrtf(tn0) * 1.000002f : 0.f;
         float pz = t0n * zn0, pa = t0n * an0, pb = t0n * bn0;
-        for (int s = lane + 64; s < n_seg; s += 64) {
-            const int64_t jj = kA + s < a.nb ? kA + s : a.nb;
-            const float t = sqrtf(a.tnorm_rest[(sd.first_seg - a.sub_first_seg) + s]) * 1.000002f;
-            pz += t * a.znorm_rest[jj]; pa += t * a.znorm_rest[a.norm_stride + jj]; pb += t * a.znorm_rest[2 * a.norm_stride + jj];
-        }
-        pz = wave_sum_f32(pz); pa = wave_sum_f32(pa); pb = wave_sum_f32(pb);
+        if constexpr (GROUP != 64) asm volatile("" : "+v"(pz), "+v"(pa), "+v"(pb));
+        if constexpr (GROUP == 64) {
+            for (int s = lane + 64; s < n_seg; s += 64) {
+                const int64_t jj = kA + s < a.nb ? kA + s : a.nb;
+                const float t = sqrtf(a.tnorm_rest[(sd.first_seg - a.sub_first_seg) + s]) * 1.000002f;
+                pz += t * a.znorm_rest[jj]; pa += t * a.znorm_rest[a.norm_stride + jj]; pb += t * a.znorm_rest[2 * a.norm_stride + jj];
+            }
+        }
+        pz = group_sum(pz); pa = group_sum(pa); pb = group_sum(pb);
         const int passes = (n_seg + MAC_SMAX_LONG - 1) / MAC_SMAX_LONG;
         b_rest = (fmaxf(pa, pb) + 1.5e-3f * pz) * tc.mac_scale * (1.0006f + 0.0005f * (float)passes) + 1e-3f;
     }
-    if (lane == 0) {
+    if (lane == 0 && live) {
         float B = acc0, qmax = acc1;
         if (a.band) {
             B = (a.band == 2 ? 0.f : B) + b_rest;
@@ -284,15 +297,51 @@
     }
 }
 template <int METHOD>
+__device__ __forceinline__ void slb_one(const BoundArgs& a, const int pr, const int lane) {
+    const int k = __builtin_amdgcn_readfirstlane(a.pairmap[pr]);
+    const SearchDesc sd = a.searches[k];
+    slb_body<METHOD, 64>(a, pr, lane, true, k, sd);
+}
+template <int METHOD, class PairAt>
+__device__ __forceinline__ void slb_four(const BoundArgs& a, const int first, const int count, const PairAt pair_at, const int lane) {
+    const int entry = first + lane / SLB_GROUP;
+    const bool live = entry < count;
+    const int pr = pair_at(live ? entry : first);
+    const int k = a.pairmap[pr];
+    const SearchDesc sd = a.searches[k];
+    if (__all(fft_layout(sd.win_start, sd.n_pos, sd.tmpl_len).n_seg <= SLB_GROUP)) {
+        slb_body<METHOD, SLB_GROUP>(a, pr, lane % SLB_GROUP, live, k, sd);
+        return;
+    }
+    for (int e = first; e < first + 64 / SLB_GROUP && e < count; ++e)
+        slb_one<METHOD>(a, __builtin_amdgcn_readfirstlane(pair_at(e)), lane);
+}
+template <int METHOD>
 __global__ __launch_bounds__(256)
 void slb_kernel(BoundArgs a) {
+    const int first = __builtin_amdgcn_readfirstlane((blockIdx.x * 4 + (threadIdx.x >> 6)) * (64 / SLB_GROUP));
+    if (first >= a.n_pairs) return;
+    slb_four<METHOD>(a, first, a.n_pairs, [](const int e) { return e; }, threadIdx.x & 63);
+}
+template <int METHOD>
+__global__ __launch_bounds__(256)
+void slb_list_kernel(BoundArgs a) {
+    const int n = *a.list_count;
+    if (n > a.n_pairs / 5) return;
+    const int step = gridDim.x * 4 * (64 / SLB_GROUP);
+    for (int first = (blockIdx.x * 4 + (threadIdx.x >> 6)) * (64 / SLB_GROUP); first < n; first += step)
+        slb_four<METHOD>(a, first, n, [&](const int e) { return a.list[e]; }, threadIdx.x & 63);
+}
+template <int METHOD>
+__global__ __launch_bounds__(256)
+void slb_wave_kernel(BoundArgs a) {
     const int pr = __builtin_amdgcn_readfirstlane(blockIdx.x * 4 + (threadIdx.x >> 6));
     if (pr >= a.n_pairs) return;
     slb_one<METHOD>(a, pr, threadIdx.x & 63);
 }
 template <int METHOD>
 __global__ __launch_bounds__(256)
-void slb_list_kernel(BoundArgs a) {
+void slb_list_wave_kernel(BoundArgs a) {
     const int n = *a.list_count;
     if (n > a.n_pairs / 5) return;
     const int waves = gridDim.x * 4;
@@ -370,10 +419,36 @@
     base = __shfl(base, 0, 64);
     if (add) list[base + __popcll(m & ((1ull << lane) - 1ull))] = pr;
 }
-
-__global__ __launch_bounds__(256)
+template <int WAVES>
+__device__ __forceinline__ int reserve_pairs_block(int* count, RunCounters* counters, const int n_wave, const int delta_wave) {
+    __shared__ int s_n[WAVES], s_delta[WAVES];
+    const int lane = threadIdx.x & 63, w = threadIdx.x >> 6;
+    if (lane == 0) { s_n[w] = n_wave; s_delta[w] = delta_wave; }
+    __syncthreads();
+    if (threadIdx.x == 0) {
+        int before[WAVES], total = 0, delta = 0;
+#pragma unroll
+        for (int i = 0; i < WAVES; ++i) { before[i] = total; total += s_n[i]; delta += s_delta[i]; }
+        const int base = total ? atomicAdd(count, total) : 0;
+        if (delta) atomicAdd(&counters->pairs_transformed, (unsigned long long)(long long)delta);
+#pragma unroll
+        for (int i = 0; i < WAVES; ++i) s_n[i] = base + before[i];
+    }
+    __syncthreads();
+    return s_n[w];
+}
+template <int WAVES>
+__device__ __forceinline__ void append_pairs_block(int* list, int* count, RunCounters* counters, const bool add, const int pr) {
+    const unsigned long long m = __ballot(add);
+    const int lane = threadIdx.x & 63;
+    const int base = reserve_pairs_block<WAVES>(count, counters, __popcll(m), __popcll(m));
+    if (add) list[base + __popcll(m & ((1ull << lane) - 1ull))] = pr;
+}
+
+constexpr int SURVIVOR_THREADS = 1024;
+__global__ __launch_bounds__(SURVIVOR_THREADS)
 void survivor_kernel(BoundArgs a) {
-    const int b = blockIdx.x * 256 + threadIdx.x;
+    const int b = blockIdx.x * SURVIVOR_THREADS + threadIdx.x;
     bool keep = false;
     int pr = 0;
     if (b < a.n_pairs) {
@@ -391,7 +466,7 @@
         }
         if (a.audit_mark) a.audit_mark[pr] = (audit ? MARK_AUDITED : 0) | (keep ? MARK_LISTED : 0);
     }
-    append_pairs(a.slist, a.scount, a.counters, keep, pr);
+    append_pairs_block<SURVIVOR_THREADS / 64>(a.slist, a.scount, a.counters, keep, pr);
 }
 
 enum { ROWS_MARKED = 0, ROWS_FIRST = 1, ROWS_REST = 2, ROWS_ITEMS = 3 };
@@ -584,8 +659,67 @@
 constexpr int BLE_LOGN = 13;
 constexpr int BLE_N = sushi_fft::Plan<BLE_LOGN>::N, BLE_T = sushi_fft::Plan<BLE_LOGN>::NT;
 static_assert(BLE_N == FN / 2, "the low band sampled at every second position");
+__device__ __forceinline__ float second_look_bound(const unsigned mm, const float dc_re, const float dc_im) {
+    const float bw = 1.4142137f * sqrtf(__uint_as_float(mm)) * 1.0007f + fmaxf(dc_re, dc_im);
+    return mm >= 0x7f800000u ? __builtin_inff() : bw;
+}
+__global__ __launch_bounds__(BLE_T, 8)
+void bound_low_exact_kernel(BoundArgs a) {
+    __shared__ __attribute__((aligned(16))) float lds[sushi_fft::lds_floats<BLE_LOGN>()];
+    __shared__ unsigned red[2];
+    typedef _Float16 h2 __attribute__((ext_vector_type(2)));
+    const int n = *a.list_count;
+    if (n > a.n_pairs / 5) return;
+    int slot = blockIdx.x;
+    if (slot >= n) return;
+    if (threadIdx.x == 0) { red[0] = 0u; red[1] = 0u; }
+    const sushi_fft::uint4v* __restrict__ rows = reinterpret_cast<const sushi_fft::uint4v*>(a.y);
+    int pr = a.list[slot];
+    sushi_fft::uint4v w0, w1;
+    {
+        const int t0 = threadIdx.x;
+        w0 = rows[(size_t)pr * LROWE + sushi_fft::sl_entry(t0, 0)]; w1 = rows[(size_t)pr * LROWE + sushi_fft::sl_entry(t0, 1)];
+    }
+    int slot_n = slot + gridDim.x;
+    int pr_n = slot_n < n ? a.list[slot_n] : pr;
+    for (int turn = 0;; turn ^= 1) {
+        int tid = threadIdx.x;
+        asm volatile("" : "+v"(tid));
+        const sushi_fft::uint4v n0 = rows[(size_t)pr_n * LROWE + sushi_fft::sl_entry(tid, 0)];
+        const sushi_fft::uint4v n1 = rows[(size_t)pr_n * LROWE + sushi_fft::sl_entry(tid, 1)];
+        const int slot_nn = slot_n + gridDim.x;
+        const int pr_nn = slot_nn < n ? a.list[slot_nn] : pr_n;
+        const float first_look = tid == 0 ? a.acc[2 * (size_t)pr] : 0.f;
+        const sushi_fft::Twiddles tw = sushi_fft::load_twiddles<BLE_LOGN, 1>(tid, twiddles());
+        __builtin_amdgcn_sched_barrier(0);
+        cpx v[sushi_fft::PER];
+#pragma unroll
+        for (int r = 0; r < sushi_fft::PER; ++r) {
+            if (sushi_fft::sl_in_band(r)) {
+                const h2 h = __builtin_bit_cast(h2, r < 8 ? w0[sushi_fft::sl_sub(r)] : w1[sushi_fft::sl_sub(r)]);
+                v[r] = cpx{(float)h.x, (float)h.y};
+            } else {
+                v[r] = cpx{0.f, 0.f};
+            }
+        }
+        float dc_re = 0.f, dc_im = 0.f;
+        if (tid == 0) { dc_re = v[0].x; dc_im = v[0].y; v[0] = cpx{0.f, 0.f}; }
+        sushi_fft::fft_split<BLE_LOGN, 1>(v, tid, lds, tw);
+        float m2 = 0.f;
+#pragma unroll
+        for (int r = 0; r < sushi_fft::PER; ++r) m2 = fmaxf(m2, v[r].x * v[r].x + v[r].y * v[r].y);
+        const unsigned wm = wave_max_u32(__float_as_uint(m2));
+        if ((tid & 63) == 0) atomicMax(&red[turn], wm);
+        if (tid == 0) red[turn ^ 1] = 0u;
+        __syncthreads();
+        if (tid == 0) a.acc[2 * (size_t)pr] = fminf(first_look, second_look_bound(red[turn], dc_re, dc_im));
+        slot = slot_n;
+        if (slot >= n) break;
+        pr = pr_n; w0 = n0; w1 = n1; slot_n = slot_nn; pr_n = pr_nn;
+    }
+}
 __global__ __launch_bounds__(BLE_T)
-void bound_low_exact_kernel(BoundArgs a) {
+void bound_low_exact_plain_kernel(BoundArgs a) {
     __shared__ __attribute__((aligned(16))) float lds[sushi_fft::lds_floats<BLE_LOGN>()];
     __shared__ unsigned red[BLE_T / 64];
     typedef _Float16 h2 __attribute__((ext_vector_type(2)));
@@ -655,12 +789,9 @@
         const unsigned long long m = __ballot(keep), act = __ballot(slot < n);
         const int lane = threadIdx.x & 63;
         const int dropped = __popcll(act) - __popcll(m);
-        int b0 = 0;
-        if (lane == 0 && m) b0 = atomicAdd(a.list2_count, __popcll(m));
-        if (lane == 0 && dropped > 0)
-            atomicAdd(&a.counters->pairs_transformed, (unsigned long long)0 - (unsigned long long)dropped);
-        b0 = __shfl(b0, 0, 64);
+        const int b0 = reserve_pairs_block<4>(a.list2_count, a.counters, __popcll(m), -dropped);
         if (keep) a.list2[b0 + __popcll(m & ((1ull << lane) - 1ull))] = pr;
+        __syncthreads();
     }
 }
 
diff --git a/sushi_amd/csrc/sushi_geometry.hpp b/sushi_amd/csrc/sushi_geometry.hpp
--- a/sushi_amd/csrc/sushi_geometry.hpp
+++ b/sushi_amd/csrc/sushi_geometry.hpp
@@ -29,6 +29,9 @@
 constexpr int TILE = 1024;
 constexpr int TILES_PER_PAIR = 2 * FFT_H / TILE;
 constexpr int COARSE_G = 256;
+constexpr int SLB_STRETCHES = 2 * FFT_H / COARSE_G;
+SUSHI_GEOM_HD constexpr int slb_stretches_a_lane(int group) { return (SLB_STRETCHES + group - 1) / group; }
+SUSHI_GEOM_HD constexpr int slb_stretch(int lane, int t, int group) { return lane + group * t; }
 
 struct FftLayout { int64_t pair0; int n_pairs; int n_seg; };
 SUSHI_GEOM_HD inline FftLayout fft_layout(int64_t win_start, int n_pos, int tmpl_len) {
diff --git a/sushi_amd/device.py b/sushi_amd/device.py
--- a/sushi_amd/device.py
+++ b/sushi_amd/device.py
@@ -486,6 +486,26 @@
         with torch.cuda.device(self._mem.device):
             return torch.as_tensor(_Foreign(), device=self._mem.device).clone().view(torch.float16)
 
+    def bounds_again(self, by_wave, which=0):
+        n = ctypes.c_int64(int(self.fft_pairs))
+        slb = np.empty(int(self.fft_pairs), np.float32)
+        votes = np.zeros(2, np.int32)
+        _native.check(_native.lib().sushi_hip_batch_bounds_again(self._handle, int(bool(by_wave)), int(which), slb.ctypes.data,
+                                                                 votes.ctypes.data, ctypes.byref(n)), "sushi_hip_batch_bounds_again")
+        return slb[:n.value], ([int(votes[0]), int(votes[1])] if which == 2 else None)
+
+    def exclusion_state(self):
+        def raw(which, dtype):
+            ptr, nbytes = ctypes.c_void_p(), ctypes.c_size_t(0)
+            _native.check(_native.lib().sushi_hip_batch_workspace_view(self._handle, int(which), ctypes.byref(ptr), ctypes.byref(nbytes)),
+                          "sushi_hip_batch_workspace_view")
+            off = ptr.value - self._mem.data_ptr()
+            assert ptr.value and 0 <= off and off + nbytes.value <= self._mem.numel()
+            return self._mem[off:off + nbytes.value].cpu().numpy().view(dtype).copy()
+        counts = raw(_native.WS_SCOUNT, np.int32)
+        return {"slist": raw(_native.WS_SLIST, np.int32), "slist2": raw(_native.WS_SLIST2, np.int32), "n_slist": int(counts[0]),
+                "n_slist2": int(counts[5]), "marks": raw(_native.WS_MARKS, np.uint8), "pair_lb": raw(_native.WS_PAIR_LB, np.float32)}
+
     def ranking_errors(self):
         return self.diagnostics(per_search=True)["ranking_err"]
 
```
